# daniestevez/ldpc-toolbox

Hardware: AMD Instinct MI355X
Metric: codewords/s + info-bits/s, DVB-S2 n=64800 r=1/2 min-sum 50 iters (higher is better)
Workload: dtype f32

## Files before the change

### ldpc_toolbox_amd/csrc/c_api.cpp

```cpp
#include "../../include/ldpc_toolbox.h"

#include <algorithm>
#include <cerrno>
#include <cstdio>
#include <cstdlib>
#include <cstring>
#include <fstream>
#include <memory>
#include <sstream>
#include <string>
#include <vector>

#include "codes.h"
#include "demodulator.h"
#include "device_bch.h"
#include "device_decoder.h"
#include "device_encoder.h"
#include "device_nr_rm.h"
#include "encoder.h"
#include "implementation.h"
#include "simulator.h"
#include "sparse.h"

namespace {
// ... 585 lines not shown
  }
  if (!make_device_encoder(h.get(), device)) return nullptr;
  return h.release();
}

int32_t ldpc_toolbox_encoder_encode_batch(void *encoder, uint8_t *output, size_t output_len, const uint8_t *input,
                                          size_t input_len, size_t batch) {
  return encode_batch(encoder, output, output_len, input, input_len, batch, false, nullptr);
}

int32_t ldpc_toolbox_encoder_encode_batch_device(void *encoder, uint8_t *output, size_t output_len, const uint8_t *input,
                                                 size_t input_len, size_t batch, void *hip_stream) {
  return encode_batch(encoder, output, output_len, input, input_len, batch, true, hip_stream);
}

int32_t ldpc_toolbox_encoder_get(void *encoder, const char *key, int64_t *value) {
  auto *h = static_cast<EncoderHandle *>(encoder);
  if (!h || !key || !value) return -1;
  const std::string k = key;
  if (k == "k")
    *value = static_cast<int64_t>(h->enc.k());
  else if (k == "n")
    *value = static_cast<int64_t>(h->enc.n());
  else if (k == "output_len")
    *value = h->out_len == SIZE_MAX ? -1 : static_cast<int64_t>(h->out_len);
  else if (k == "staircase")
    *value = h->enc.staircase() ? 1 : 0;
  else if (k == "staircase_form")
    *value = h->enc.staircase() ? ldpc::staircase_form(h->enc.k()) : -1;
  else if (k == "device")
    *value = h->dev ? h->dev->device() : -1;
  else
    return -1;
  return 0;
}

int32_t ldpc_toolbox_decoder_decode_batch_f32(void *decoder, uint8_t *output, size_t output_len,
                                              const float *llrs, size_t llrs_len, size_t batch,
                                              uint32_t max_iterations, int32_t *iterations, float *posterior) {
  return decode_batch<float>(decoder, output, output_len, llrs, llrs_len, batch, max_iterations, iterations,
                             posterior, false, nullptr);
}

int32_t ldpc_toolbox_decoder_decode_batch_f64(void *decoder, uint8_t *output, size_t output_len,
                                              const double *llrs, size_t llrs_len, size_t batch,
                                              uint32_t max_iterations, int32_t *iterations, double *posterior) {
  return decode_batch<double>(decoder, output, output_len, llrs, llrs_len, batch, max_iterations, iterations,
                              posterior, false, nullptr);
}

int32_t ldpc_toolbox_decoder_decode_batch_f32_device(void *decoder, uint8_t *output, size_t output_len,
                                                     const float *llrs, size_t llrs_len, size_t batch,
                                                     uint32_t max_iterations, int32_t *iterations,
                                                     float *posterior, void *hip_stream) {
  return decode_batch<float>(decoder, output, output_len, llrs, llrs_len, batch, max_iterations, iterations,
                             posterior, true, hip_stream);
}

int32_t ldpc_toolbox_decoder_decode_batch_f64_device(void *decoder, uint8_t *output, size_t output_len,
                                                     const double *llrs, size_t llrs_len, size_t batch,
                                                     uint32_t max_iterations, int32_t *iterations,
                                                     double *posterior, void *hip_stream) {
  return decode_batch<double>(decoder, output, output_len, llrs, llrs_len, batch, max_iterations, iterations,
                              posterior, true, hip_stream);
}

int32_t ldpc_toolbox_decoder_syndrome(void *decoder, const uint8_t *bits, size_t bits_len, size_t batch,
                                      uint8_t *syndrome, uint32_t *weight) {
  g_last_error.clear();
  auto *h = static_cast<DecoderHandle *>(decoder);
  if (!h || !h->dec) {
    set_error("null decoder handle");
    return LDPC_TOOLBOX_ERR_ARGUMENT;
  }
  if (bits_len != h->dec->n() || (!bits && batch)) {
    set_error("hard decisions must cover the whole codeword (bits_len == n)");
    return LDPC_TOOLBOX_ERR_ARGUMENT;
  }
  const int rc = h->dec->syndrome_host(bits, batch, syndrome, weight);
  if (rc == 0) return 0;
  set_error(h->dec->last_error());
  return rc == -1 ? LDPC_TOOLBOX_ERR_ARGUMENT : LDPC_TOOLBOX_ERR_DEVICE;
}

int32_t ldpc_toolbox_decoder_syndrome_device(void *decoder, const uint8_t *bits, size_t bits_len, size_t batch,
                                             uint8_t *syndrome, uint32_t *weight, void *hip_stream) {
  g_last_error.clear();
  auto *h = static_cast<DecoderHandle *>(decoder);
  if (!h || !h->dec) {
    set_error("null decoder handle");
    return LDPC_TOOLBOX_ERR_ARGUMENT;
  }
  if (bits_len != h->dec->n() || (!bits && batch)) {
    set_error("hard decisions must cover the whole codeword (bits_len == n)");
    return LDPC_TOOLBOX_ERR_ARGUMENT;
  }
  const int rc = h->dec->syndrome_device(bits, batch, syndrome, weight, static_cast<hipStream_t>(hip_stream));
  if (rc == 0) return 0;
  set_error(h->dec->last_error());
  return rc == -1 ? LDPC_TOOLBOX_ERR_ARGUMENT : LDPC_TOOLBOX_ERR_DEVICE;
}

int32_t ldpc_toolbox_decoder_get(void *decoder, const char *key, int64_t *value) {
  auto *h = static_cast<DecoderHandle *>(decoder);
  if (!h || !h->dec || !key || !value) return -1;
  const std::string k = key;
  const ldpc::DeviceDecoder &d = *h->dec;
  if (k == "n")
    *value = static_cast<int64_t>(d.n());
  else if (k == "m")
    *value = static_cast<int64_t>(d.m());
  else if (k == "k")
    *value = static_cast<int64_t>(d.n()) - static_cast<int64_t>(d.m());
  else if (k == "edges")
    *value = static_cast<int64_t>(d.edges());
  else if (k == "input_len")
    *value = static_cast<int64_t>(d.input_len());
  else if (k == "device")
    *value = d.device();
  else if (k == "group_size")
    *value = static_cast<int64_t>(d.group_size());
  else if (k == "max_check_degree")
    *value = d.max_check_degree();
  else if (k == "max_variable_degree")
    *value = d.max_variable_degree();
  else if (k == "layers")
    *value = static_cast<int64_t>(d.layers());
  else if (k == "last_lanes")
    *value = d.last_lanes();
  else if (k == "last_pooled")
    *value = static_cast<int64_t>(d.last_pooled());
  else if (k == "last_group")
    *value = static_cast<int64_t>(d.last_group());
  else if (k == "preferred_group")
    *value = static_cast<int64_t>(d.preferred_group(size_t(1) << 20));
  else if (k == "row_records")
    *value = d.row_records();
  else if (k == "record_flag_bits")
    *value = d.record_flag_bits();
  else if (k == "last_vn_records")
    *value = d.last_vn_records();
  else if (k == "last_vn_bundles")
    *value = d.last_vn_bundles();
  else if (k == "vn_bundle_saved_permille")
    *value = d.vn_bundle_saved_permille();
  else if (k == "last_vn_chains")
    *value = d.last_vn_chains();
  else if (k == "vn_chain_saved_permille")
    *value = d.vn_chain_saved_permille();
  else if (k == "flags8")
    *value = d.flags8();
  else if (k == "last_record_flag_bytes")
    *value = d.last_record_flag_bytes();
  else if (k == "minsum_correction")
    *value = static_cast<int64_t>(d.implementation().correction);
  else if (k == "minsum_correction_int")
    *value = d.implementation().correction_int;
  else if (k == "last_persist" || k == "experiments")
    *value = 0;
  else
    return -1;
  return 0;
}

int32_t ldpc_toolbox_decoder_set(void *decoder, const char *key, int64_t value) {
  auto *h = static_cast<DecoderHandle *>(decoder);
  if (!h || !h->dec || !key) return -1;
  const std::string k = key;
  if (k == "group_size" && value >= 0)
    h->dec->set_group_size(static_cast<size_t>(value));
  else if (k == "profiling")
    h->dec->set_profiling(value != 0);
  else if (!h->dec->set_option(k, value))
    return -1;
  return 0;
}

int32_t ldpc_toolbox_decoder_kernel_stats(void *decoder, int32_t kind, uint64_t *launches, double *total_ms,
                                          int32_t reset) {
  auto *h = static_cast<DecoderHandle *>(decoder);
  if (!h || !h->dec || kind < 0 || kind >= ldpc::kKernelKinds) return -1;
  const ldpc::KernelStat s = h->dec->kernel_stat(kind);
  if (launches) *launches = s.launches;
  if (total_ms) *total_ms = s.total_ms;
  if (reset) h->dec->reset_kernel_stats();
  return 0;
}


void *ldpc_toolbox_sim_ctor(const char *alist, const char *implementation, const char *puncturing, int32_t device,
                            uint32_t pool_size, uint64_t pool_seed) {
  g_last_error.clear();
  if (!alist || !implementation) {
    set_error("null argument");
    return nullptr;
  }
  std::string err;
  ldpc::Simulator *s = ldpc::Simulator::create(alist, implementation, puncturing ? puncturing : "", device,
                                               pool_size, pool_seed, &err);
  if (!s) set_error(err);
  return s;
}

void ldpc_toolbox_sim_dtor(void *sim) { delete static_cast<ldpc::Simulator *>(sim); }

int32_t ldpc_toolbox_sim_run(void *sim, double ebn0_db, uint64_t seed, uint64_t first_frame, size_t frames,
                             uint32_t max_iterations, uint64_t *counters) {
  g_last_error.clear();
  auto *s = static_cast<ldpc::Simulator *>(sim);
  if (!s || !counters) {
    set_error("null argument");
    return -1;
  }
  const int rc = s->run(ebn0_db, seed, first_frame, frames, max_iterations, counters);
  if (rc) set_error(s->last_error());
  return rc;
}

int32_t ldpc_toolbox_sim_run_bch(void *sim, double ebn0_db, uint64_t seed, uint64_t first_frame, size_t frames,
                                 uint32_t max_iterations, uint64_t bch_max_errors, uint64_t *counters) {
  g_last_error.clear();
  auto *s = static_cast<ldpc::Simulator *>(sim);
  if (!s || !counters) {
    set_error("null argument");
    return -1;
  }
  const int rc = s->run_bch(ebn0_db, seed, first_frame, frames, max_iterations, bch_max_errors, counters);
  if (rc) set_error(s->last_error());
  return rc;
}

int32_t ldpc_toolbox_sim_generate(void *sim, double ebn0_db, uint64_t seed, uint64_t first_frame, size_t frames,
                                  float *llrs, uint32_t *pool_index) {
  g_last_error.clear();
  auto *s = static_cast<ldpc::Simulator *>(sim);
  if (!s || !llrs) {
    set_error("null argument");
    return -1;
  }
  const int rc = s->generate(ebn0_db, seed, first_frame, frames, llrs, pool_index);
  if (rc) set_error(s->last_error());
  return rc;
}

int32_t ldpc_toolbox_sim_pool(void *sim, uint8_t *messages, uint8_t *tx_bits) {
  auto *s = static_cast<ldpc::Simulator *>(sim);
  if (!s) return -1;
  if (messages) std::memcpy(messages, s->messages().data(), s->messages().size());
  if (tx_bits) std::memcpy(tx_bits, s->tx_bits().data(), s->tx_bits().size());
  return 0;
}

int32_t ldpc_toolbox_sim_get(void *sim, const char *key, int64_t *value) {
  auto *s = static_cast<ldpc::Simulator *>(sim);
  if (!s || !key || !value) return -1;
  const std::string k = key;
  if (k == "k")
    *value = static_cast<int64_t>(s->k());
  else if (k == "n")
    *value = static_cast<int64_t>(s->n());
  else if (k == "n_tx")
    *value = static_cast<int64_t>(s->n_tx());
  else if (k == "pool")
    *value = s->pool();
  else if (k == "modulation")
    *value = s->modulation();
  else if (k == "interleaving")
    *value = s->interleaving();
  else if (k == "constellation")
    *value = s->has_constellation() ? 1 : 0;
  else if (k == "max_log")
    *value = s->max_log() ? 1 : 0;
  else if (k == "bch")
    *value = s->has_bch() ? 1 : 0;
  else if (k == "rate_match")
    *value = s->has_rate_match() ? 1 : 0;
  else if (k == "streamed_frames" || k == "stream_iterations")
    *value = 0;
  else if (k == "pooled_frames")
    *value = static_cast<int64_t>(s->pooled_frames());
  else if (k == "preferred_batch")
    *value = static_cast<int64_t>(s->decoder()->preferred_group(size_t(1) << 20));
  else
    return -1;
  return 0;
}

int32_t ldpc_toolbox_sim_set(void *sim, const char *key, int64_t value) {
  auto *s = static_cast<ldpc::Simulator *>(sim);
  if (!s || !key) return -1;
  const std::string k = key;
  if (k == "group_size" && value >= 0) {
    s->decoder()->set_group_size(static_cast<size_t>(value));
    return 0;
  }
  if (k == "pooling") {
    s->set_pooling(value != 0);
    return 0;
  }
  if (k == "streaming") return 0;
  if (k == "modulation" || k == "interleaving") {
    g_last_error.clear();
    const bool ok = k == "modulation" ? s->set_modulation(static_cast<int>(value)) : s->set_interleaving(value);
    if (!ok) set_error(s->last_error());
    return ok ? 0 : -1;
  }
// ... 329 lines not shown
```

### ldpc_toolbox_amd/csrc/device_decoder.h

```cpp
#pragma once
#include <hip/hip_runtime_api.h>

#include <algorithm>
#include <atomic>
#include <cstddef>
#include <cstdint>
#include <memory>
#include <string>
#include <vector>

#include "hip_owned.h"
#include "implementation.h"
#include "sparse.h"

namespace ldpc {

struct GroupCall;

struct KernelStat {
  uint64_t launches = 0;
  double total_ms = 0.0;
};

enum KernelKind { kKernelCheck = 0, kKernelVar = 1, kKernelLayer = 2, kKernelOther = 3, kKernelKinds = 4 };

class DeviceDecoder {
 public:
  static DeviceDecoder *create(const SparseMatrix &h, const Implementation &impl,
                               const std::vector<uint8_t> &puncturing, int device, std::string *err);
  ~DeviceDecoder();

  size_t n() const { return n_; }
  size_t m() const { return m_; }
  size_t edges() const { return e_; }
  size_t input_len() const { return input_len_; }
  const Implementation &implementation() const { return impl_; }
  int device() const { return device_; }
  uint32_t max_check_degree() const { return max_row_weight_; }
  uint32_t max_variable_degree() const { return max_col_weight_; }
  size_t layers() const { return level_ptr_.empty() ? 0 : level_ptr_.size() - 1; }
  uint32_t last_lanes() const { return last_lanes_; }
  uint64_t last_pooled() const { return last_pooled_; }
  size_t last_group() const { return last_group_; }
  uint32_t row_records() const { return (rec_ready_ && records_wanted() && opt_lfree_ && !opt_staged_minsum_) ? rec_w_ : 0; }
  uint32_t record_flag_bits() const { return row_records() ? rec_flag_bits_ : 0; }
  uint32_t last_vn_records() const { return last_vn_records_.load(std::memory_order_relaxed) ? 1 : 0; }
  uint32_t flags8() const { return opt_flags8_ ? 1 : 0; }
  uint32_t last_record_flag_bytes() const { return last_record_flag_bytes_.load(std::memory_order_relaxed); }
  uint32_t last_vn_bundles() const { return last_vn_bundles_.load(std::memory_order_relaxed) ? 1 : 0; }
  uint32_t vn_bundle_saved_permille() const { return last_vn_bundle_saved_.load(std::memory_order_relaxed); }
  uint32_t last_vn_chains() const { return last_vn_chains_.load(std::memory_order_relaxed) ? 1 : 0; }
  uint32_t vn_chain_saved_permille() const { return last_vn_chain_saved_.load(std::memory_order_relaxed); }

  void set_group_size(size_t g) { group_pref_ = g; }
  size_t group_size() const { return group_pref_; }
  void set_min_group(size_t g) { min_group_ = g; }
  size_t preferred_group(size_t batch) const { return pick_group(batch); }
  bool set_option(const std::string &key, int64_t value);
  void set_profiling(bool on);
  KernelStat kernel_stat(int kind);
  void reset_kernel_stats();

  int decode_device(const void *llrs, bool llrs_f64, size_t batch, uint32_t max_iterations,
                    uint8_t *bits, size_t out_len, int32_t *iterations, void *posterior,
                    hipStream_t stream);

  int decode_host(const void *llrs, bool llrs_f64, size_t batch, uint32_t max_iterations,
                  uint8_t *bits, size_t out_len, int32_t *iterations, void *posterior);

  int syndrome_device(const uint8_t *bits, size_t batch, uint8_t *syndrome, uint32_t *weight, hipStream_t stream);
  int syndrome_host(const uint8_t *bits, size_t batch, uint8_t *syndrome, uint32_t *weight);

  const std::string &last_error() const { return error_; }

 private:
  DeviceDecoder() = default;
  struct Workspace;
  struct GroupFrame;
  int run_group_i8(Workspace &w, const GroupCall &call);
  template <typename T>
  int run_group(Workspace &w, const GroupCall &call);
  int run_any(Workspace &w, const GroupCall &call);
  int ensure_workspace(Workspace &w, size_t group, void *place = nullptr, size_t *need = nullptr);
  int ensure_lanes(uint32_t lanes, size_t group);
  void release_joint();
  int ensure_host_staging(Workspace &w, size_t G, size_t in_elem);
  int ensure_row_scratch(Workspace &w, size_t bytes);
  struct HostPipe;
  int ensure_pipe(size_t group, size_t out_len, size_t in_elem, bool posterior);
  int stage_in(const char *src, char *dst, size_t bytes);
  int drain_out(char *dst, const char *src, size_t bytes);
  struct LatencyPath;
  struct SmallBatchCall;
  struct EdgeLatencyPath;
  size_t edge_latency_limit() const;
  uint32_t opt_latency_edge_ = 256;
  size_t edge_lanes_ = 0;
  int decode_latency_edge(const void *llrs, bool llrs_f64, bool host_pointers, size_t batch, uint32_t max_iterations,
                             uint8_t *bits, size_t out_len, int32_t *iterations, void *posterior, hipStream_t stream);
  uint32_t opt_latency_ = 32;
  static constexpr int kLatencyRetry = -100;
  static constexpr uint32_t opt_serial_levels_default() { return 512; }
  int decode_latency(const void *llrs, bool llrs_f64, bool host_pointers, size_t batch, uint32_t max_iterations,
                     uint8_t *bits, size_t out_len, int32_t *iterations, void *posterior, hipStream_t stream);
  uint32_t lane_count() const;
  bool split_pays(size_t batch) const;
  size_t pick_group(size_t batch) const;
  bool fail(const std::string &msg, hipError_t e = hipSuccess);
  void timed_begin(int kind, hipStream_t s);
  void timed_end(int kind, hipStream_t s);
  void drain_events();

  Implementation impl_;
  int device_ = 0;
  size_t n_ = 0, m_ = 0, e_ = 0, input_len_ = 0;
  uint32_t max_row_weight_ = 0, max_col_weight_ = 0;
  size_t group_pref_ = 0, min_group_ = 0;
  uint32_t opt_tile_ = 0;
  uint32_t opt_waves_ = 0, opt_vec_ = 4;
  bool opt_staged_minsum_ = false;
  static constexpr uint32_t kStreamBlock = 256;
  static constexpr uint32_t kVnWaves = 128 * 1024;
  static constexpr uint32_t kPackWaves = 16 * 1024;
  static constexpr uint32_t kSyndThreads = 512 * 1024, kMoveWaves = 64 * 1024, kRetireBlocks = 256;
  static constexpr uint32_t kCompactHorizon = 8, kCompactCostLive = 9, kCompactCostSlots = 0, kCompactMinFreedQ = 2;
  std::string error_;

  uint32_t n_keep_ = 0, n_free_ = 0;
  uint32_t post_rows_keep_ = 0;
  bool opt_rec_long_ = false;
  bool opt_rec_quiet_ = true;
  bool opt_vn_event_ = true;
  bool opt_vn_records_ = false;
  bool opt_flags8_ = false;
  bool opt_vn_bundles_ = false;
  static constexpr uint32_t kVnBundleW = kStreamBlock / 64;
  uint32_t vn_bundle_saved_[kVnBundleW + 1] = {};
  std::atomic<bool> last_vn_bundles_{false};
  std::atomic<uint32_t> last_vn_bundle_saved_{0};
  bool opt_vn_chains_ = false;
  uint32_t opt_vn_chain_len_ = 8;
  static constexpr uint32_t kVnChainLens[3] = {4, 8, 16};
  struct VnChainAt {
    uint32_t rs_at = 0, var_at = 0, ptr_at = 0, n_blocks = 0;
    uint32_t saved = 0, saved_alone = 0;
  } vn_chain_at_[3];
  std::atomic<bool> last_vn_chains_{false};
  std::atomic<uint32_t> last_vn_chain_saved_{0};
  std::atomic<uint32_t> last_record_flag_bytes_{0};
  std::atomic<bool> last_vn_records_{false};
  uint32_t rec_w_ = 0;
  uint32_t rec_flag_bits_ = 0;
  bool rec_ready_ = false, rec_prefers_ = false;
  uint32_t opt_records_ = 1;
  bool records_wanted() const { return opt_records_ >= 2 || (opt_records_ == 1 && rec_prefers_); }
  uint32_t opt_rec_run_ = 8;
  bool opt_compact_ = true;
  uint32_t opt_compact_first_ = 0, opt_compact_every_ = 0;
  uint32_t opt_serial_levels_ = 512;
  uint32_t opt_cn_reg_ = 1;
  uint32_t opt_hl_reg_ = 1;
  bool opt_lane_threads_ = true, opt_throttle_ = false;
  uint32_t opt_lead_ = 0;
  bool opt_lane_pace_ = true;
  bool opt_hl_records_ = true;
  std::vector<uint32_t> level_maxdeg_;
  std::vector<uint32_t> level_rec_ptr_;
  bool lfree_ready_ = false, opt_lfree_ = true;
  std::vector<uint32_t> level_ptr_;
  uint32_t pattern_len_ = 0;

  size_t joint_stride_ = 0, joint_second_ = 0;
  int order_after_default_stream(hipStream_t s);
  uint32_t last_lanes_ = 0;
  size_t last_group_ = 0;
  bool opt_pooling_ = false;
  uint64_t last_pooled_ = 0;
  uint32_t pool_budget_ = 0, pool_budget_max_it_ = 0;
  struct StragglerPool;
  int ensure_pool(size_t batch, size_t rows, size_t out_len, size_t in_elem, bool posterior, bool own_iterations);
  static uint32_t next_pool_budget(double ok, double sum_its_ok, double stragglers, double straggler_its, double failed_full,
                                   uint32_t max_it);
  int decode_device_plain(const void *llrs, bool llrs_f64, size_t batch, uint32_t max_iterations, uint8_t *bits, size_t out_len,
                          int32_t *iterations, void *posterior, hipStream_t stream);
  int decode_device_pooled(const void *llrs, bool llrs_f64, size_t batch, uint32_t max_iterations, uint8_t *bits, size_t out_len,
                           int32_t *iterations, void *posterior, hipStream_t stream);
  int decode_host_plain(const void *llrs, bool llrs_f64, size_t batch, uint32_t max_iterations, uint8_t *bits, size_t out_len,
                        int32_t *iterations, void *posterior);
  int decode_host_pooled(const void *llrs, bool llrs_f64, size_t batch, uint32_t max_iterations, uint8_t *bits, size_t out_len,
                         int32_t *iterations, void *posterior);
  size_t pool_chunk(size_t batch) const;
  uint32_t opt_lanes_ = 0;
  bool opt_poll_ = true;

  bool profiling_ = false;
  struct PendingEvent {
    int kind;
    Event a, b;
  };
  KernelStat stats_[kKernelKinds];

  Stream stream_, stream2_;
  Event ev_fork_, ev_join_, ev_default_;
  DeviceBuffer d_row_ptr_, d_edge_col_, d_col_ptr_, d_col_edge_;
  DeviceBuffer d_level_rows_;
  DeviceBuffer d_level_recs_;
  DeviceBuffer d_row_recs_;
  DeviceBuffer d_serial_recs_;
  DeviceBuffer d_src_block_;
  DeviceBuffer d_edge_aux_, d_keep_var_, d_keep_ptr_, d_keep_edge_, d_free_var_, d_free_ptr_, d_free_edge_;
  DeviceBuffer d_edge_peer_, d_free_rs_, d_keep_pos_;
  DeviceBuffer d_keep_rs_;
  uint32_t bundle_rs_at_ = 0, bundle_var_at_ = 0, bundle_ptr_at_ = 0;
  DeviceBuffer joint_slab_;
  std::unique_ptr<Workspace> ws_[2];
  std::unique_ptr<StragglerPool> pool_;
  std::unique_ptr<EdgeLatencyPath> lat_edge_;
  std::unique_ptr<LatencyPath> lat_;
  std::unique_ptr<HostPipe> pipe_;
  std::vector<Event> event_pool_;
  std::vector<PendingEvent> pending_;
};

}
```

### ldpc_toolbox_amd/csrc/device_decoder.hip

```cpp
#define LDPC_GROUP_KERNELS_TU 1
#include "codes.h"
#include "device_decoder_internal.h"

namespace ldpc {

static bool is_dvbs2_half_rate_normal(const SparseMatrix::Csr &g) {
  if (g.n_cols != 64800 || g.n_rows != 32400) return false;
  SparseMatrix ref;
  if (!codes::dvbs2("R1_2", &ref)) return false;
  const SparseMatrix::Csr r = ref.csr();
  if (r.n_edges != g.n_edges || r.row_ptr != g.row_ptr) return false;
  std::vector<uint32_t> a, b;
  for (uint32_t row = 0; row < g.n_rows; row++) {
    a.assign(g.edge_col.begin() + g.row_ptr[row], g.edge_col.begin() + g.row_ptr[row + 1]);
    b.assign(r.edge_col.begin() + r.row_ptr[row], r.edge_col.begin() + r.row_ptr[row + 1]);
    std::sort(a.begin(), a.end());
    std::sort(b.begin(), b.end());
    if (a != b) return false;
  }
  return true;
}

bool DeviceDecoder::fail(const std::string &msg, hipError_t e) {
  static std::mutex m;
// ... 73 lines not shown
  };
  g.edge_col.resize(g.edge_col.size() + kTablePad, 0);
  bool ok = up(g.row_ptr, &d->d_row_ptr_) && up(g.edge_col, &d->d_edge_col_) && up(g.col_ptr, &d->d_col_ptr_) &&
            up(g.col_edge, &d->d_col_edge_);
  const bool flooding_minsum = impl.schedule == Schedule::Flooding && impl.rule == Rule::Minsum && !impl.i8;
  if (ok && flooding_minsum) {
    const LfreeTables lf = build_lfree_tables(g);
    if (lf.ready) {
      d->n_keep_ = lf.n_keep;
      d->n_free_ = lf.n_free;
      d->post_rows_keep_ = lf.post_rows_keep;
      ok = up(lf.aux, &d->d_edge_aux_) && up(lf.keep_var, &d->d_keep_var_) && up(lf.keep_ptr, &d->d_keep_ptr_) &&
           up(lf.keep_edge, &d->d_keep_edge_) && up(lf.free_var, &d->d_free_var_) && up(lf.free_ptr, &d->d_free_ptr_) &&
           up(lf.free_edge, &d->d_free_edge_);
      d->lfree_ready_ = ok;
    }
    const RowRecordTables rr = d->lfree_ready_ ? build_row_record_tables(g, lf, impl.f64) : RowRecordTables();
    if (rr.ready) {
      d->rec_prefers_ = rr.rec_prefers;
      d->rec_w_ = rr.rec_w;
      d->rec_flag_bits_ = rr.flag_bits;
      ok = up(rr.keep_pos, &d->d_keep_pos_) && up(rr.peer, &d->d_edge_peer_) && up(rr.free_rs, &d->d_free_rs_);
      d->rec_ready_ = ok;
      const KeepRsTable kr = (ok && rr.flag_bits == 16) ? build_keep_rs(g, lf) : KeepRsTable();
      if (kr.ready) {
        const VnBundleTables vb = build_vn_bundles(lf.n_keep, lf.keep_ptr, lf.keep_var, kr.rs, kVnBundleW);
        std::vector<uint32_t> words = kr.rs;
        auto append = [&](const std::vector<uint32_t> &v) {
          const uint32_t at = static_cast<uint32_t>(words.size());
          words.insert(words.end(), v.begin(), v.end());
          return at;
        };
        d->bundle_rs_at_ = append(vb.keep_rs);
        d->bundle_var_at_ = append(vb.list_var);
        d->bundle_ptr_at_ = append(vb.list_ptr);
        for (uint32_t c = 0; c < 3; c++) {
          const VnChainTables vc = build_vn_chains(lf.n_keep, lf.keep_ptr, lf.keep_var, kr.rs, kVnBundleW, kVnChainLens[c]);
          VnChainAt &at = d->vn_chain_at_[c];
          at.rs_at = append(vc.keep_rs);
          at.var_at = append(vc.list_var);
          at.ptr_at = append(vc.list_ptr);
          at.n_blocks = vc.n_blocks;
          at.saved = vc.fetches ? static_cast<uint32_t>((vc.fetches - vc.issued) * 1000 / vc.fetches) : 0;
          at.saved_alone = vc.fetches ? static_cast<uint32_t>(vc.carried * 1000 / vc.fetches) : 0;
        }
        ok = up(words, &d->d_keep_rs_);
        for (uint32_t w = 2; w <= kVnBundleW; w++) {
          uint64_t fetches = 0, distinct = 0;
          count_vn_bundle_fetches(lf.n_keep, vb.list_ptr, vb.keep_rs, w, &fetches, &distinct);
          d->vn_bundle_saved_[w] = fetches ? static_cast<uint32_t>((fetches - distinct) * 1000 / fetches) : 0;
        }
      }
      d->opt_vn_records_ = kr.ready && ok && !impl.f64 && impl.correction == Correction::None && is_dvbs2_half_rate_normal(g);
      d->opt_flags8_ = d->opt_vn_records_;
      d->opt_vn_bundles_ = d->opt_vn_records_ && d->bundle_rs_at_ != 0;
      d->opt_vn_chains_ = d->opt_vn_bundles_ && d->vn_chain_at_[0].rs_at != 0;
    }
  }
  if (ok && flooding_minsum && !impl.f64) {
    SlicedTables st = build_sliced_tables(g);
    if (st.ready) {
      d->lat_ = std::make_unique<LatencyPath>();
      d->lat_->tables = std::move(st);
    }
  }
  if (ok && impl.schedule == Schedule::Flooding && impl.rule == Rule::Tanh && !impl.i8 && d->max_row_weight_ <= kLevelRecShort) {
    LevelTables all;
    all.level_ptr = {0u, g.n_rows};
    all.rows.resize(g.n_rows);
    for (uint32_t r = 0; r < g.n_rows; r++) all.rows[r] = r;
    all.maxdeg = {d->max_row_weight_};
    ok = up(build_level_recs(all, g.row_ptr, g.edge_col).words, &d->d_row_recs_);
  }
  LevelTables lt;
  if (ok && impl.schedule == Schedule::Layered) {
    lt = build_levels(g.row_ptr, g.edge_col, g.n_rows, g.n_cols);
    d->level_ptr_ = lt.level_ptr;
    d->level_maxdeg_ = lt.maxdeg;
    const LevelRecs lr = build_level_recs(lt, g.row_ptr, g.edge_col);
    d->level_rec_ptr_ = lr.rec_ptr;
    LevelTables all;
    all.level_ptr = {0u, g.n_rows};
    all.rows = lt.rows;
    all.maxdeg = {lt.maxdeg.empty() ? 0u : *std::max_element(lt.maxdeg.begin(), lt.maxdeg.end())};
    ok = up(lt.rows, &d->d_level_rows_) && up(lr.words, &d->d_level_recs_) &&
         up(build_level_recs(all, g.row_ptr, g.edge_col).words, &d->d_serial_recs_);
  }
  if (ok && !impl.fast && !(impl.i8 && impl.rule == Rule::Minsum) && d->lat_ == nullptr &&
      (impl.schedule == Schedule::Flooding || d->level_ptr_.size() <= size_t(opt_serial_levels_default()) + 1)) {
    EdgeLaneTables et = build_edge_lane_tables(g, impl.schedule == Schedule::Layered ? &lt : nullptr);
    if (et.ready) {
      d->edge_lanes_ = et.lane_var.size();
      d->lat_edge_ = std::make_unique<EdgeLatencyPath>();
      d->lat_edge_->tables = std::move(et);
    }
  }
  if (ok && !puncturing.empty()) {
    const DepunctureMap dm = build_depuncture_map(puncturing, g.n_cols);
    if (!dm.ready) return bail("codeword size not divisible by puncturing pattern length");
    d->pattern_len_ = static_cast<uint32_t>(puncturing.size());
    d->input_len_ = dm.input_len;
    ok = up(dm.src_block, &d->d_src_block_);
  }
  ok = ok && d->stream_.create() == hipSuccess && d->stream2_.create() == hipSuccess && d->ev_fork_.create() == hipSuccess &&
       d->ev_join_.create() == hipSuccess && d->ev_default_.create() == hipSuccess;
  if (!ok) return bail("device allocation / upload of the graph tables failed");
  d->ws_[0] = std::make_unique<Workspace>();
  d->ws_[1] = std::make_unique<Workspace>();
  return d.release();
}

DeviceDecoder::~DeviceDecoder() {
  (void)hipSetDevice(device_);
  if (stream_) (void)hipStreamSynchronize(stream_);
  if (stream2_) (void)hipStreamSynchronize(stream2_);
}


void DeviceDecoder::set_profiling(bool on) { profiling_ = on; }

bool DeviceDecoder::set_option(const std::string &key, int64_t value) {
  if (value < 0) return false;
  const uint32_t v = static_cast<uint32_t>(value);
  if (key == "waves")
    opt_waves_ = v;
  else if (key == "vec")
    opt_vec_ = v;
  else if (key == "tile")
    opt_tile_ = v;
  else if (key == "lfree")
    opt_lfree_ = v != 0;
  else if (key == "records")
    opt_records_ = v != 0 ? (v >= 2 ? 2 : 1) : 0;
  else if (key == "rec_run")
    opt_rec_run_ = std::max<uint32_t>(v, 1);
  else if (key == "rec_quiet")
    opt_rec_quiet_ = v != 0;
  else if (key == "vn_event")
    opt_vn_event_ = v != 0;
  else if (key == "vn_records")
    opt_vn_records_ = v != 0;
  else if (key == "flags8")
    opt_flags8_ = v != 0;
  else if (key == "vn_bundles")
    opt_vn_bundles_ = v != 0;
  else if (key == "vn_chains")
    opt_vn_chains_ = v != 0;
  else if (key == "vn_chain_len") {
    if (v != kVnChainLens[0] && v != kVnChainLens[1] && v != kVnChainLens[2]) return false;
    opt_vn_chain_len_ = v;
  }
  else if (key == "rec_long")
    opt_rec_long_ = v != 0;
  else if (key == "compact")
    opt_compact_ = v != 0;
  else if (key == "staged_minsum")
    opt_staged_minsum_ = v != 0;
  else if (key == "hl_reg")
    opt_hl_reg_ = v;
  else if (key == "cn_reg")
    opt_cn_reg_ = v;
  else if (key == "hl_records")
    opt_hl_records_ = v != 0;
  else if (key == "lane_threads")
    opt_lane_threads_ = v != 0;
  else if (key == "throttle")
    opt_throttle_ = v != 0;
  else if (key == "pooling")
    opt_pooling_ = v != 0;
  else if (key == "lead")
    opt_lead_ = v;
  else if (key == "lane_pace")
    opt_lane_pace_ = v != 0;
  else if (key == "lanes")
    opt_lanes_ = std::min<uint32_t>(v, 2);
  else if (key == "poll")
    opt_poll_ = v != 0;
  else if (key == "latency") {
    opt_latency_ = v;
    opt_latency_edge_ = v == 0 ? 0 : std::max<uint32_t>(v, 64);
  } else if (key == "latency_edge")
    opt_latency_edge_ = v;
  else if (key == "compact_first")
    opt_compact_first_ = v;
  else if (key == "serial_levels")
    opt_serial_levels_ = v;
  else if (key == "compact_every")
    opt_compact_every_ = v;
  else
    return false;
  return true;
}

void DeviceDecoder::timed_begin(int kind, hipStream_t s) {
  if (!profiling_) return;
  PendingEvent p;
  p.kind = kind;
  auto get = [&]() {
    Event e;
    if (!event_pool_.empty()) {
      e = std::move(event_pool_.back());
      event_pool_.pop_back();
    } else {
      (void)e.create(hipEventDefault);
    }
    return e;
  };
  p.a = get();
  p.b = get();
  (void)hipEventRecord(p.a, s);
  pending_.push_back(std::move(p));
}

void DeviceDecoder::timed_end(int, hipStream_t s) {
  if (!profiling_) return;
  (void)hipEventRecord(pending_.back().b, s);
}

void DeviceDecoder::drain_events() {
  for (auto &p : pending_) {
    (void)hipEventSynchronize(p.b);
    float ms = 0.f;
    if (hipEventElapsedTime(&ms, p.a, p.b) == hipSuccess) {
      stats_[p.kind].launches++;
      stats_[p.kind].total_ms += ms;
    }
    event_pool_.push_back(std::move(p.a));
    event_pool_.push_back(std::move(p.b));
  }
  pending_.clear();
}

KernelStat DeviceDecoder::kernel_stat(int kind) {
  drain_events();
  return (kind >= 0 && kind < kKernelKinds) ? stats_[kind] : KernelStat();
}

void DeviceDecoder::reset_kernel_stats() {
  drain_events();
  for (auto &s : stats_) s = KernelStat();
}


size_t DeviceDecoder::pick_group(size_t batch) const {
  const bool serial = impl_.schedule == Schedule::Layered && level_ptr_.size() > size_t(opt_serial_levels_) + 1;
  size_t by_size = 4096;
  while (by_size < 65536 && e_ * by_size * 2 <= size_t(226799) * 4096) by_size *= 2;
  size_t g = group_pref_ ? group_pref_ : std::max<size_t>(serial ? 16384 : 4096, by_size);
  g = std::min(g, std::max(round_up(batch, 64), std::min(min_group_, g)));
  g = round_up(g, 64);
  if (impl_.i8) return round_up(g, 256);
  if (g >= 256) g = g / 256 * 256;
  return g;
}

uint32_t DeviceDecoder::lane_count() const {
  if (opt_lanes_) return opt_lanes_;
  if (impl_.schedule == Schedule::Layered) return 2u;
  if (impl_.f64 || impl_.i8) return 1u;
  if (impl_.rule == Rule::Tanh) return 2u;
  if (impl_.rule == Rule::Minsum && max_row_weight_ > 8 && !profiling_) return 2u;
  return 1u;
}

bool DeviceDecoder::split_pays(size_t batch) const {
  return opt_lanes_ == 2 || (batch >= 2048 && n_ * (batch / 2) >= size_t(50) * 1000 * 1000);
}

int DeviceDecoder::ensure_workspace(Workspace &w, size_t G, void *place, size_t *need) {
  const size_t elem = impl_.i8 ? 2 : (impl_.f64 ? 8 : 4);
  const bool records = lfree_ready_ && rec_ready_ && records_wanted() && opt_lfree_;
  if (!need) {
    if (w.G == G && w.elem == elem && w.chan && w.records == records && (!place || w.slab == place))
      return 0;
    w = Workspace();
  }
  const size_t W = G / 64;
  const size_t align = size_t(2) << 20;
  size_t off = 0;
  auto carve = [&](size_t bytes) {
    const size_t at = off;
    off = round_up(off + std::max<size_t>(bytes, 256), align);
    return at;
  };
  const size_t o_msg = carve(std::max<size_t>(e_, 1) * G * elem);
  const size_t o_msg2 = (lfree_ready_ && !records) ? carve(std::max<size_t>(e_, 1) * G * elem) : 0;
  const bool flags16 = records && rec_flag_bits_ == 16;
  const size_t rec_bytes = records ? std::max<size_t>(m_, 1) * (flags16 ? 2 : rec_w_) * G * elem : 0;
  const size_t o_rec0 = records ? carve(rec_bytes) : 0, o_rec1 = records ? carve(rec_bytes) : 0;
  const size_t flag_bytes = flags16 ? std::max<size_t>(m_, 1) * G * sizeof(uint16_t) : 0;
  const size_t o_flag0 = flags16 ? carve(flag_bytes) : 0, o_flag1 = flags16 ? carve(flag_bytes) : 0;
  const size_t o_post = carve(n_ * G * elem);
  const size_t o_chan = carve(n_ * G * elem);
  const size_t o_perm = carve(4 * G * sizeof(uint32_t) + 1024);
  const size_t o_raw = carve(n_ * W * sizeof(uint64_t));
  const size_t o_hard = carve(n_ * W * sizeof(uint64_t));
  const size_t o_flags = carve(9 * G * sizeof(uint32_t) + 1024);
  if (need) {
    *need = off;
    return 0;
  }
  w.records = records;
  if (w.flag.ensure(64, 64, 64, hipHostMallocMapped) == hipSuccess) {
    w.h_flag = w.flag.get<uint64_t>();
    *w.h_flag = 0;
    if (hipHostGetDevicePointer(reinterpret_cast<void **>(&w.d_flag), w.h_flag, 0) != hipSuccess) w.d_flag = nullptr;
  } else {
    w.h_flag = nullptr;
  }
  w.G = G;
  w.elem = elem;
  if (place) {
    w.slab = place;
    w.borrowed = true;
  } else {
    HIP_TRY(w.own_slab.ensure(off));
    w.slab = w.own_slab.get();
  }
  w.slab_bytes = off;
  char *base = static_cast<char *>(w.slab);
  w.msg = base + o_msg;
  w.msg2 = (lfree_ready_ && !records) ? base + o_msg2 : nullptr;
  w.rec[0] = records ? base + o_rec0 : nullptr;
  w.rec[1] = records ? base + o_rec1 : nullptr;
  w.rec_flags[0] = flags16 ? reinterpret_cast<uint16_t *>(base + o_flag0) : nullptr;
  w.rec_flags[1] = flags16 ? reinterpret_cast<uint16_t *>(base + o_flag1) : nullptr;
  w.post = base + o_post;
  w.chan = base + o_chan;
  w.perm = reinterpret_cast<uint32_t *>(base + o_perm);
  w.slot_cw = w.perm + G;
  w.slot_tmp = w.perm + 2 * G;
  w.fill_cw = w.perm + 3 * G;
  w.n_slots = w.perm + 4 * G;
  w.plan = reinterpret_cast<dev::CompactPlan *>(w.perm + 4 * G + 16);
  w.rawbits = reinterpret_cast<uint64_t *>(base + o_raw);
  w.hardbits = reinterpret_cast<uint64_t *>(base + o_hard);
  uint32_t *flags = reinterpret_cast<uint32_t *>(base + o_flags);
  w.done = flags;
  w.unsat0 = flags + G;
  w.unsat1 = flags + 2 * G;
  w.iters = reinterpret_cast<int32_t *>(flags + 3 * G);
  w.n_active = flags + 4 * G;
  w.scratch_flags = flags + 4 * G + 64;
  w.slice_state = flags + 6 * G;
  if (std::getenv("LDPC_TOOLBOX_DEBUG"))
    std::fprintf(stderr, "ldpc_toolbox (hip): workspace G=%zu slab=%p bytes=%zu msg=+%zx post=+%zx chan=+%zx\n", G,
                 w.slab, off, o_msg, o_post, o_chan);
  return 0;
}

int DeviceDecoder::ensure_lanes(uint32_t lanes, size_t G) {
  if (lanes < 2) {
    Workspace &w = *ws_[0];
    if (w.borrowed && w.G != G) release_joint();
    return ensure_workspace(w, G);
  }
  size_t bytes = 0;
  if (int rc = ensure_workspace(*ws_[0], G, nullptr, &bytes)) return rc;
  const size_t lane_align = size_t(2) << 20;
  const size_t stride = round_up(bytes, lane_align);
  const size_t elem = impl_.i8 ? 2 : (impl_.f64 ? 8 : 4);
  const bool records = lfree_ready_ && rec_ready_ && records_wanted() && opt_lfree_;
  auto current = [&](const Workspace &w, const char *at) {
    return w.borrowed && w.slab == at && w.G == G && w.elem == elem && w.records == records;
  };
  char *base = joint_slab_ ? reinterpret_cast<char *>(round_up(reinterpret_cast<size_t>(joint_slab_.get()), lane_align)) : nullptr;
  if (base && joint_stride_ == stride && current(*ws_[0], base) && current(*ws_[1], base + joint_second_)) return 0;
  release_joint();
  HIP_TRY(joint_slab_.ensure(stride + bytes + lane_align));
  base = reinterpret_cast<char *>(round_up(reinterpret_cast<size_t>(joint_slab_.get()), lane_align));
  joint_stride_ = stride;
  joint_second_ = stride;
  if (int rc = ensure_workspace(*ws_[0], G, base)) return rc;
  return ensure_workspace(*ws_[1], G, base + joint_second_);
}

void DeviceDecoder::release_joint() {
  for (auto &w : ws_)
    if (w && w->borrowed) *w = Workspace();
  joint_slab_ = DeviceBuffer();
  joint_stride_ = 0;
  joint_second_ = 0;
}

int DeviceDecoder::run_any(Workspace &w, const GroupCall &call) {
  GroupCall c = call;
  const bool own_thread = c.own_thread;
  const bool may_wait = c.may_block;
  c.may_block = may_wait && opt_poll_ && impl_.schedule == Schedule::Layered && (own_thread || c.nb * n_ <= size_t(8) * 1000 * 1000);
  c.pace_lead = opt_lead_;
  if (own_thread && may_wait && opt_poll_ && impl_.schedule == Schedule::Layered && opt_lane_pace_) {
    c.may_block = true;
    if (!opt_lead_) c.pace_lead = 1;
  }
  if (impl_.schedule == Schedule::Flooding && !impl_.i8 && opt_poll_ && may_wait && !profiling_ && (c.flood_pace || own_thread)) {
    c.may_block = true;
    if (!opt_lead_) c.pace_lead = 2;
  }
  return impl_.i8 ? run_group_i8(w, c) : impl_.f64 ? run_group<double>(w, c) : run_group<float>(w, c);
}

int DeviceDecoder::order_after_default_stream(hipStream_t s) {
  HIP_TRY(hipEventRecord(ev_default_, nullptr));
  HIP_TRY(hipStreamWaitEvent(s, ev_default_, 0));
  return 0;
}


int DeviceDecoder::ensure_pool(size_t batch, size_t rows, size_t out_len, size_t in_elem, bool posterior, bool own_iterations) {
  if (!pool_) pool_ = std::make_unique<StragglerPool>();
  StragglerPool &p = *pool_;
  constexpr size_t kFloor = 256;
  HIP_TRY(p.d_idx.ensure(batch * sizeof(uint32_t), kFloor));
  HIP_TRY(p.d_stats.ensure(64));
  HIP_TRY(p.d_llrs.ensure(rows * input_len_ * in_elem, kFloor));
  HIP_TRY(p.d_bits.ensure(rows * std::max<size_t>(out_len, 1), kFloor));
  HIP_TRY(p.d_its.ensure(rows * sizeof(int32_t), kFloor));
  if (posterior) HIP_TRY(p.d_post.ensure(rows * n_ * in_elem, kFloor));
  if (own_iterations) HIP_TRY(p.d_its_all.ensure(batch * sizeof(int32_t), kFloor));
  return 0;
}

uint32_t DeviceDecoder::next_pool_budget(double ok, double sum_its_ok, double stragglers, double straggler_its,
                                         double failed_full, uint32_t max_it) {
  const double ok_frames = ok + stragglers, ok_its = sum_its_ok + straggler_its;
  const double avg_ok = ok_frames > 0 ? ok_its / ok_frames : static_cast<double>(max_it);
  uint32_t next = static_cast<uint32_t>(std::min<double>(max_it, std::ceil(2.0 * avg_ok) + 8.0));
  next = std::max<uint32_t>(next, 16);
  if (stragglers + failed_full > 0.25 * (ok + stragglers + failed_full) || uint64_t(next) * 10 >= uint64_t(max_it) * 7) next = max_it;
  return next;
}

size_t DeviceDecoder::pool_chunk(size_t batch) const { return pick_group(batch) * std::max<uint32_t>(lane_count(), 1); }

int DeviceDecoder::decode_device(const void *llrs, bool llrs_f64, size_t batch, uint32_t max_iterations, uint8_t *bits,
                                 size_t out_len, int32_t *iterations, void *posterior, hipStream_t stream) {
  last_pooled_ = 0;
  if (opt_pooling_ && max_iterations >= 24 && batch >= 2 * pool_chunk(batch) && (stream == nullptr || opt_throttle_) && out_len <= n_)
    return decode_device_pooled(llrs, llrs_f64, batch, max_iterations, bits, out_len, iterations, posterior, stream);
  return decode_device_plain(llrs, llrs_f64, batch, max_iterations, bits, out_len, iterations, posterior, stream);
}

int DeviceDecoder::decode_device_pooled(const void *llrs, bool llrs_f64, size_t batch, uint32_t max_iterations, uint8_t *bits,
                                        size_t out_len, int32_t *iterations, void *posterior, hipStream_t stream) {
  HIP_TRY(hipSetDevice(device_));
  const size_t in_elem = llrs_f64 ? 8 : 4, G = pick_group(batch), chunk = pool_chunk(batch);
  hipStream_t s = stream ? stream : stream_;
  if (int rc = ensure_pool(batch, chunk, out_len, in_elem, posterior != nullptr, iterations == nullptr)) return rc;
  StragglerPool &p = *pool_;
  uint32_t *const d_idx = p.d_idx.get<uint32_t>(), *const d_stats = p.d_stats.get<uint32_t>();
  int32_t *its = iterations ? iterations : p.d_its_all.get<int32_t>();
  unsigned long long *d_sum = reinterpret_cast<unsigned long long *>(d_stats + 4);
  HIP_TRY(hipMemsetAsync(d_stats, 0, 64, s));
  uint32_t budget = (pool_budget_ && pool_budget_max_it_ == max_iterations) ? std::min(pool_budget_, max_iterations) : max_iterations;
  double straggler_its = 0.0;
  uint32_t seen_stragglers = 0;
  const size_t llr_row = input_len_ * in_elem, post_row = n_ * in_elem;
  for (size_t b0 = 0; b0 < batch; b0 += chunk) {
    const size_t nf = std::min(chunk, batch - b0);
    if (int rc = decode_device_plain(static_cast<const char *>(llrs) + b0 * llr_row, llrs_f64, nf, budget, bits + b0 * out_len, out_len,
                                     its + b0, posterior ? static_cast<char *>(posterior) + b0 * post_row : nullptr, stream))
      return rc;
    dev::pool_select_kernel<<<static_cast<uint32_t>((nf + 255) / 256), 256, 0, s>>>(
        its + b0, static_cast<uint32_t>(nf), static_cast<uint32_t>(b0), budget < max_iterations ? 1 : 0, d_idx, d_stats, d_sum);
    uint32_t h[6];
    HIP_TRY(hipMemcpyAsync(h, d_stats, sizeof(h), hipMemcpyDeviceToHost, s));
    HIP_TRY(hipStreamSynchronize(s));
    unsigned long long sum_ok;
    std::memcpy(&sum_ok, &h[4], sizeof(sum_ok));
    straggler_its += double(h[2] - seen_stragglers) * budget;
    seen_stragglers = h[2];
    budget = next_pool_budget(h[0], static_cast<double>(sum_ok), h[2], straggler_its, h[1], max_iterations);
  }
  pool_budget_ = budget;
  pool_budget_max_it_ = max_iterations;
  const size_t keep_min = min_group_;
  for (size_t p0 = 0; p0 < seen_stragglers; p0 += chunk) {
    const uint32_t np = static_cast<uint32_t>(std::min<size_t>(chunk, seen_stragglers - p0));
    const uint32_t blocks = (np * 64 + 255) / 256;
    dev::pool_gather_kernel<<<blocks, 256, 0, s>>>(d_idx + p0, np, static_cast<const uint32_t *>(llrs), llr_row / 4,
                                                   p.d_llrs.get<uint32_t>());
    min_group_ = G;
    const int rc = decode_device_plain(p.d_llrs.get(), llrs_f64, np, max_iterations, p.d_bits.get<uint8_t>(), out_len, p.d_its.get<int32_t>(),
                                       posterior ? p.d_post.get() : nullptr, stream);
    min_group_ = keep_min;
    if (rc) return rc;
    dev::pool_scatter_kernel<<<blocks, 256, 0, s>>>(d_idx + p0, np, p.d_bits.get<uint8_t>(), static_cast<uint32_t>(out_len), p.d_its.get<int32_t>(),
                                                    p.d_post.get<const uint32_t>(), posterior ? post_row / 4 : 0, bits,
                                                    iterations, static_cast<uint32_t *>(posterior));
  }
  last_pooled_ = seen_stragglers;
  HIP_TRY(hipGetLastError());
  if (stream == nullptr) HIP_TRY(hipStreamSynchronize(s));
  return 0;
}

int DeviceDecoder::decode_device_plain(const void *llrs, bool llrs_f64, size_t batch, uint32_t max_iterations,
                                       uint8_t *bits, size_t out_len, int32_t *iterations, void *posterior,
                                       hipStream_t stream) {
  if (batch == 0) return 0;
  if (out_len > n_) {
    fail("output_len larger than the codeword length");
    return -1;
  }
  HIP_TRY(hipSetDevice(device_));
  const bool own_stream = stream == nullptr;
  hipStream_t s = own_stream ? stream_ : stream;
  if (own_stream)
    if (int rc = order_after_default_stream(s)) return rc;
  if (lat_ && batch <= opt_latency_ && own_stream) {
    const int rc = decode_latency(llrs, llrs_f64, false, batch, max_iterations, bits, out_len, iterations, posterior, s);
    if (rc != kLatencyRetry) return rc;
  }
  if (lat_edge_ && batch <= edge_latency_limit() && own_stream) {
    const int rc = decode_latency_edge(llrs, llrs_f64, false, batch, max_iterations, bits, out_len, iterations, posterior, s);
    if (rc != kLatencyRetry) return rc;
  }
  size_t G = pick_group(batch);
  uint32_t lanes = lane_count();
  if (lanes == 2 && batch <= G && split_pays(batch)) G = round_up((batch + 1) / 2, 256);
  if (batch <= G) lanes = 1;
  last_lanes_ = lanes;
  last_group_ = G;
  if (int rc = ensure_lanes(lanes, G)) return rc;
  if (lanes == 2) {
    HIP_TRY(hipEventRecord(ev_fork_, s));
    HIP_TRY(hipStreamWaitEvent(stream2_, ev_fork_, 0));
  }
  const size_t in_elem = llrs_f64 ? 8 : 4;
  const bool threaded = lanes == 2 && opt_lane_threads_ && !profiling_ && max_iterations > 0 &&
                        (impl_.schedule == Schedule::Layered ||
                         (impl_.schedule == Schedule::Flooding && !impl_.i8 && (opt_throttle_ || own_stream) && opt_poll_));
  const bool may_block = own_stream || opt_throttle_;
  auto run_groups = [&](uint32_t only_lane) -> int {
    uint32_t gi = 0;
    for (size_t b0 = 0; b0 < batch; b0 += G, gi++) {
      const uint32_t lane = lanes == 2 ? (gi & 1u) : 0u;
      if (only_lane != 2 && lane != only_lane) continue;
      const size_t nb = std::min(G, batch - b0);
      const char *src = static_cast<const char *>(llrs) + b0 * input_len_ * in_elem;
      uint8_t *dst_bits = bits + b0 * out_len;
      int32_t *dst_it = iterations ? iterations + b0 : nullptr;
      void *dst_post = posterior ? static_cast<char *>(posterior) + b0 * n_ * in_elem : nullptr;
      if (int rc = run_any(*ws_[lane], GroupCall{src, llrs_f64, nb, max_iterations, dst_bits, out_len, dst_it, dst_post,
                                                 lane ? stream2_ : s, may_block, threaded, lanes == 1}))
        return rc;
    }
    return 0;
  };
  if (threaded) {
    int rc1 = 0;
    std::thread second([&] {
      rc1 = hipSetDevice(device_) == hipSuccess ? run_groups(1) : -2;
    });
    const int rc0 = run_groups(0);
    second.join();
    if (rc0 || rc1) return rc0 ? rc0 : rc1;
  } else if (int rc = run_groups(2)) {
    return rc;
  }
  if (lanes == 2) {
    HIP_TRY(hipEventRecord(ev_join_, stream2_));
    HIP_TRY(hipStreamWaitEvent(s, ev_join_, 0));
  }
  if (own_stream) HIP_TRY(hipStreamSynchronize(s));
  return 0;
}

int DeviceDecoder::ensure_row_scratch(Workspace &w, size_t bytes) {
  HIP_TRY(w.row_scratch.ensure(bytes));
  return 0;
}

int DeviceDecoder::ensure_host_staging(Workspace &w, size_t G, size_t in_elem) {
  HIP_TRY(w.in.ensure(G * input_len_ * in_elem));
  return 0;
}

namespace {

void par_memcpy(char *dst, const char *src, size_t bytes, unsigned threads) {
  if (threads <= 1 || bytes < (size_t(4) << 20)) {
    std::memcpy(dst, src, bytes);
    return;
  }
  const size_t per = round_up((bytes + threads - 1) / threads, 4096);
  std::vector<std::thread> th;
  for (size_t off = per; off < bytes; off += per)
    th.emplace_back([=] { std::memcpy(dst + off, src + off, std::min(per, bytes - off)); });
  std::memcpy(dst, src, std::min(per, bytes));
  for (auto &t : th) t.join();
}

}

int DeviceDecoder::ensure_pipe(size_t group, size_t out_len, size_t in_elem, bool posterior) {
  if (!pipe_) {
    auto p = std::make_unique<HostPipe>();
    const unsigned hw = std::max(1u, std::thread::hardware_concurrency());
    p->copy_threads = std::min(8u, std::max(1u, hw / 2));
    bool ok = p->h2d.create() == hipSuccess && p->d2h.create() == hipSuccess;
    for (int i = 0; ok && i < HostPipe::kSlots; i++) ok = p->in_done[i].create() == hipSuccess && p->out_done[i].create() == hipSuccess;
    for (int l = 0; ok && l < 2; l++) ok = p->in_ready[l].create() == hipSuccess && p->ingested[l].create() == hipSuccess;
    if (!ok) {
      fail("host staging: stream / event creation failed");
      return -2;
    }
    pipe_ = std::move(p);
  }
  HostPipe &p = *pipe_;
  for (int r = 0; r < HostPipe::kOutRing; r++) {
    HIP_TRY(p.d_bits[r].ensure(std::max<size_t>(group * out_len, 1)));
    HIP_TRY(p.d_iters[r].ensure(group * sizeof(int32_t)));
    if (posterior) HIP_TRY(p.d_post[r].ensure(group * n_ * in_elem));
  }
  return 0;
}

int DeviceDecoder::stage_in(const char *src, char *dst, size_t bytes) {
  HostPipe &p = *pipe_;
  for (size_t off = 0; off < bytes; off += HostPipe::kChunk) {
    const size_t len = std::min(HostPipe::kChunk, bytes - off);
    const int slot = p.next_in;
    p.next_in = (p.next_in + 1) % HostPipe::kSlots;
    HIP_TRY(hipEventSynchronize(p.in_done[slot]));
    if (p.in_slot[slot].ensure(len, HostPipe::kGranule, HostPipe::kChunk) != hipSuccess) {
      fail("host staging: pinned input chunk");
      return -2;
    }
    par_memcpy(p.in_slot[slot].get<char>(), src + off, len, p.copy_threads);
    HIP_TRY(hipMemcpyAsync(dst + off, p.in_slot[slot].get(), len, hipMemcpyHostToDevice, p.h2d));
    HIP_TRY(hipEventRecord(p.in_done[slot], p.h2d));
  }
  return 0;
}

int DeviceDecoder::drain_out(char *dst, const char *src, size_t bytes) {
  HostPipe &p = *pipe_;
  const size_t chunks = (bytes + HostPipe::kChunk - 1) / HostPipe::kChunk;
  auto issue = [&](size_t c) -> int {
    const size_t off = c * HostPipe::kChunk, len = std::min(HostPipe::kChunk, bytes - off);
    const int slot = static_cast<int>(c % HostPipe::kSlots);
    if (p.out_slot[slot].ensure(len, HostPipe::kGranule, HostPipe::kChunk) != hipSuccess) {
      fail("host staging: pinned output chunk");
      return -2;
    }
    HIP_TRY(hipMemcpyAsync(p.out_slot[slot].get(), src + off, len, hipMemcpyDeviceToHost, p.d2h));
    HIP_TRY(hipEventRecord(p.out_done[slot], p.d2h));
    return 0;
  };
  for (size_t c = 0; c < std::min<size_t>(chunks, HostPipe::kSlots); c++)
    if (int rc = issue(c)) return rc;
  for (size_t c = 0; c < chunks; c++) {
    const size_t off = c * HostPipe::kChunk, len = std::min(HostPipe::kChunk, bytes - off);
    const int slot = static_cast<int>(c % HostPipe::kSlots);
    HIP_TRY(hipEventSynchronize(p.out_done[slot]));
    par_memcpy(dst + off, p.out_slot[slot].get<char>(), len, p.copy_threads);
    if (c + HostPipe::kSlots < chunks)
      if (int rc = issue(c + HostPipe::kSlots)) return rc;
  }
  return 0;
}

int DeviceDecoder::decode_host(const void *llrs, bool llrs_f64, size_t batch, uint32_t max_iterations, uint8_t *bits,
                               size_t out_len, int32_t *iterations, void *posterior) {
  last_pooled_ = 0;
  if (opt_pooling_ && max_iterations >= 24 && batch >= 2 * 4 * pool_chunk(batch) && out_len <= n_)
    return decode_host_pooled(llrs, llrs_f64, batch, max_iterations, bits, out_len, iterations, posterior);
  return decode_host_plain(llrs, llrs_f64, batch, max_iterations, bits, out_len, iterations, posterior);
}

int DeviceDecoder::decode_host_pooled(const void *llrs, bool llrs_f64, size_t batch, uint32_t max_iterations, uint8_t *bits,
                                      size_t out_len, int32_t *iterations, void *posterior) {
  const size_t in_elem = llrs_f64 ? 8 : 4, chunk = 4 * pool_chunk(batch);
  const size_t llr_row = input_len_ * in_elem, post_row = n_ * in_elem;
  std::vector<int32_t> own_its;
  if (!iterations) own_its.resize(batch);
  int32_t *its = iterations ? iterations : own_its.data();
  std::vector<size_t> stragglers;
  uint32_t budget = (pool_budget_ && pool_budget_max_it_ == max_iterations) ? std::min(pool_budget_, max_iterations) : max_iterations;
  double ok = 0, sum_ok = 0, straggler_its = 0, failed_full = 0;
  for (size_t b0 = 0; b0 < batch; b0 += chunk) {
    const size_t nf = std::min(chunk, batch - b0);
    if (int rc = decode_host_plain(static_cast<const char *>(llrs) + b0 * llr_row, llrs_f64, nf, budget, bits + b0 * out_len, out_len,
                                   its + b0, posterior ? static_cast<char *>(posterior) + b0 * post_row : nullptr))
      return rc;
    const bool reduced = budget < max_iterations;
    for (size_t i = 0; i < nf; i++) {
      const int32_t it = its[b0 + i];
      if (it >= 0) {
        ok += 1;
        sum_ok += it;
      } else if (reduced) {
        stragglers.push_back(b0 + i);
        straggler_its += budget;
      } else {
        failed_full += 1;
      }
    }
    budget = next_pool_budget(ok, sum_ok, static_cast<double>(stragglers.size()), straggler_its, failed_full, max_iterations);
  }
  pool_budget_ = budget;
  pool_budget_max_it_ = max_iterations;
  if (!stragglers.empty()) {
    const size_t np = stragglers.size();
    std::vector<char> rows(np * llr_row), pbits(np * std::max<size_t>(out_len, 1)), ppost(posterior ? np * post_row : 0);
    std::vector<int32_t> pits(np);
    for (size_t i = 0; i < np; i++) std::memcpy(&rows[i * llr_row], static_cast<const char *>(llrs) + stragglers[i] * llr_row, llr_row);
    const size_t keep_min = min_group_;
    min_group_ = pick_group(batch);
    const int rc = decode_host_plain(rows.data(), llrs_f64, np, max_iterations, reinterpret_cast<uint8_t *>(pbits.data()), out_len,
                                     pits.data(), posterior ? ppost.data() : nullptr);
    min_group_ = keep_min;
    if (rc) return rc;
    for (size_t i = 0; i < np; i++) {
      const size_t f = stragglers[i];
      std::memcpy(bits + f * out_len, &pbits[i * out_len], out_len);
      its[f] = pits[i];
      if (posterior) std::memcpy(static_cast<char *>(posterior) + f * post_row, &ppost[i * post_row], post_row);
    }
  }
  last_pooled_ = stragglers.size();
  return 0;
}

int DeviceDecoder::decode_host_plain(const void *llrs, bool llrs_f64, size_t batch, uint32_t max_iterations,
                                     uint8_t *bits, size_t out_len, int32_t *iterations, void *posterior) {
  if (batch == 0) return 0;
  if (out_len > n_) {
    fail("output_len larger than the codeword length");
    return -1;
  }
  HIP_TRY(hipSetDevice(device_));
  if (lat_ && batch <= opt_latency_) {
    const int rc = decode_latency(llrs, llrs_f64, true, batch, max_iterations, bits, out_len, iterations, posterior, stream_);
    if (rc != kLatencyRetry) return rc;
  }
  if (lat_edge_ && batch <= edge_latency_limit()) {
    const int rc = decode_latency_edge(llrs, llrs_f64, true, batch, max_iterations, bits, out_len, iterations, posterior, stream_);
    if (rc != kLatencyRetry) return rc;
  }
  size_t G = pick_group(batch);
  while (!group_pref_ && G > 4096 && G * input_len_ * (llrs_f64 ? 8 : 4) > (size_t(256) << 20)) G /= 2;
  if (lane_count() == 2 && batch <= G && split_pays(batch)) G = round_up((batch + 1) / 2, 256);
  const uint32_t lanes = (batch > G && opt_lanes_ != 1) ? 2u : 1u;
  last_lanes_ = lanes;
  last_group_ = G;
  const size_t in_elem = llrs_f64 ? 8 : 4;
  if (int rc = ensure_lanes(lanes, G)) return rc;
  for (uint32_t l = 0; l < lanes; l++)
    if (int rc = ensure_host_staging(*ws_[l], G, in_elem)) return rc;
  if (int rc = ensure_pipe(std::min(G, batch), out_len, in_elem, posterior != nullptr)) return rc;
  HostPipe &p = *pipe_;
  std::vector<size_t> starts;
  {
    size_t b0 = 0;
    if (batch >= 2 * G && G >= 1024 && (G / 4) % 256 == 0) {
      starts.push_back(0);
      starts.push_back(G / 4);
      b0 = G;
    }
    for (; b0 < batch; b0 += G) starts.push_back(b0);
    const size_t last0 = starts.back(), last_n = batch - last0;
    if (starts.size() >= 3 && last_n >= 1024) {
      const size_t tail = std::max<size_t>(256, last_n / 4 / 256 * 256);
      starts.push_back(batch - tail);
    }
    starts.push_back(batch);
  }
  const size_t n_groups = starts.size() - 1;
  while (p.group_done.size() < n_groups) {
    Event e;
    HIP_TRY(e.create());
    p.group_done.push_back(std::move(e));
  }
  hipStream_t streams[2] = {stream_, stream2_};
  const size_t row_in = input_len_ * in_elem;
  constexpr size_t R = HostPipe::kOutRing;
  int rc = 0;
  auto drain_group = [&](size_t gi) -> int {
    const size_t b0 = starts[gi], nb = starts[gi + 1] - b0, r = gi % R;
    HIP_TRY(hipStreamWaitEvent(p.d2h, p.group_done[gi], 0));
    int drc = 0;
    if (out_len) drc = drain_out(reinterpret_cast<char *>(bits + b0 * out_len), p.d_bits[r].get<const char>(), nb * out_len);
    if (drc == 0 && iterations)
      drc = drain_out(reinterpret_cast<char *>(iterations + b0), p.d_iters[r].get<const char>(), nb * sizeof(int32_t));
    if (drc == 0 && posterior)
      drc = drain_out(static_cast<char *>(posterior) + b0 * n_ * in_elem, p.d_post[r].get<const char>(), nb * n_ * in_elem);
    return drc;
  };
  const bool threaded = lanes == 2 && n_groups >= 2 && impl_.schedule == Schedule::Layered && opt_lane_threads_ && !profiling_ &&
                        max_iterations > 0;
  struct LaneQueue {
    std::thread th;
    std::mutex m;
    std::condition_variable cv;
    std::deque<std::function<int()>> tasks;
    bool closing = false;
    std::atomic<uint32_t> ingest_recorded{0}, enqueued{0};
    std::atomic<int> rc{0};
  };
  LaneQueue lq[2];
  auto wait_for = [&](std::atomic<uint32_t> &counter, uint32_t at_least, LaneQueue &q) {
    while (counter.load(std::memory_order_acquire) < at_least && q.rc.load() == 0) std::this_thread::yield();
  };
  if (threaded) {
    for (uint32_t l = 0; l < 2; l++) {
      lq[l].th = std::thread([this, l, &lq] {
        LaneQueue &q = lq[l];
        if (hipSetDevice(device_) != hipSuccess) q.rc = -2;
        for (;;) {
          std::function<int()> task;
          {
            std::unique_lock<std::mutex> lock(q.m);
            q.cv.wait(lock, [&] { return q.closing || !q.tasks.empty(); });
            if (q.tasks.empty()) return;
            task = std::move(q.tasks.front());
            q.tasks.pop_front();
          }
// ... 161 lines not shown
```

### ldpc_toolbox_amd/csrc/device_decoder_internal.h

```cpp
#pragma once
#include "device_decoder.h"

#include <algorithm>
#include <atomic>
#include <chrono>
#include <condition_variable>
#include <cstdio>
#include <cstdlib>
#include <cstring>
#include <deque>
#include <functional>
#include <mutex>
#include <thread>
#include <type_traits>

#include "graph_tables.h"
#include "hip_owned.h"
#include "kernels.hip.h"
#include "slice_tasks.h"
#include "latency.hip.h"
#include "latency_edge.hip.h"

namespace ldpc {

inline uint32_t env_u32(const char *name, uint32_t dflt) {
  const char *s = std::getenv(name);
  if (!s || !*s) return dflt;
  return static_cast<uint32_t>(std::strtoul(s, nullptr, 10));
}

inline size_t round_up(size_t x, size_t m) { return (x + m - 1) / m * m; }

struct DeviceDecoder::Workspace {
  size_t G = 0;
  size_t elem = 4;
  void *slab = nullptr;
  DeviceBuffer own_slab;
  bool borrowed = false;
  size_t slab_bytes = 0;
  void *chan = nullptr, *post = nullptr, *msg = nullptr, *msg2 = nullptr;
  void *rec[2] = {nullptr, nullptr};
  uint16_t *rec_flags[2] = {nullptr, nullptr};
  bool records = false;
  uint64_t *rawbits = nullptr, *hardbits = nullptr;
  uint32_t *perm = nullptr, *slot_cw = nullptr, *slot_tmp = nullptr, *fill_cw = nullptr, *n_slots = nullptr;
  dev::CompactPlan *plan = nullptr;
  uint32_t *done = nullptr, *unsat0 = nullptr, *unsat1 = nullptr, *n_active = nullptr, *scratch_flags = nullptr,
           *slice_state = nullptr;
  int32_t *iters = nullptr;
  PinnedBuffer flag;
  uint64_t *h_flag = nullptr, *d_flag = nullptr;
  uint32_t epoch = 0;
  DeviceBuffer in;
  hipEvent_t after_ingest = nullptr;
  std::atomic<uint32_t> *ingest_seq = nullptr;
  DeviceBuffer row_scratch;
};

struct DeviceDecoder::HostPipe {
  static constexpr size_t kChunk = size_t(32) << 20;
  static constexpr size_t kGranule = size_t(64) << 10;
  static constexpr int kSlots = 4;
  static constexpr int kOutRing = 4;
  Stream h2d, d2h;
  PinnedBuffer in_slot[kSlots], out_slot[kSlots];
  Event in_done[kSlots], out_done[kSlots];
  int next_in = 0;
  Event in_ready[2], ingested[2];
  std::vector<Event> group_done;
  DeviceBuffer d_bits[kOutRing], d_iters[kOutRing], d_post[kOutRing];
  unsigned copy_threads = 1;
};

struct SmallBatchStaging {
  PinnedBuffer h_in, h_out;
  uint32_t grid = 0;
};

struct DeviceDecoder::LatencyPath {
  SlicedTables tables;
  bool uploaded = false;
  DeviceBuffer d_rslice_ptr, d_rdeg, d_col, d_vslice_ptr, d_vdeg, d_vedge, d_perm, d_inv;
  DeviceBuffer slot_mem, sync;
  dev::LatencyState slots{};
  SmallBatchStaging staging;
  static constexpr size_t kPinnedGranule = size_t(1) << 20;
};

struct DeviceDecoder::EdgeLatencyPath {
  EdgeLaneTables tables;
  bool uploaded = false;
  DeviceBuffer d_level_chunk, d_lane_var, d_lane_info, d_var_ptr, d_var_lane;
  DeviceBuffer slot_mem, flag_mem, sync;
  dev::EdgeLatState slots{};
  SmallBatchStaging staging;
  static constexpr size_t kPinnedGranule = size_t(1) << 16;
};

#define HIP_TRY(expr)                                  \
  do {                                                 \
    hipError_t _e = (expr);                            \
    if (_e != hipSuccess) {                            \
      fail(#expr, _e);                                 \
      return -2;                                       \
    }                                                  \
  } while (0)

struct DeviceDecoder::StragglerPool {
  DeviceBuffer d_idx, d_stats, d_llrs, d_post, d_bits, d_its, d_its_all;
};


struct Tiling {
  uint32_t blocks, threads;
  dev::Sched sched;
};

inline Tiling make_tiling(uint32_t G, uint32_t tile, uint32_t slice, uint32_t nodes, uint32_t threads,
                   uint32_t target_waves) {
  Tiling t;
  t.threads = threads;
  t.sched.tile = tile;
  t.sched.nchunks = G / slice;
  const uint32_t wpb = threads / 64;
  uint32_t wpc = std::max<uint32_t>(1, target_waves / t.sched.nchunks);
  wpc = std::min<uint32_t>(wpc, std::max<uint32_t>(nodes, 1));
  t.sched.slices_per_tile = std::max<uint32_t>(1, tile / slice);
  while ((uint64_t(wpc) * t.sched.slices_per_tile) % wpb != 0) wpc++;
  t.sched.waves_per_chunk = wpc;
  t.sched.reverse = 0;
  t.sched.per_tile_div = dev::fast_div(wpc * t.sched.slices_per_tile);
  t.sched.spt_div = dev::fast_div(t.sched.slices_per_tile);
  t.sched.tile_div = dev::fast_div(tile);
  t.sched.n_tiles = (t.sched.nchunks + t.sched.slices_per_tile - 1) / t.sched.slices_per_tile;
  t.blocks = static_cast<uint32_t>(uint64_t(wpc) * t.sched.nchunks / wpb);
  return t;
}

struct GroupCall {
  const void *llrs;
  bool llrs_f64;
  size_t nb;
  uint32_t max_iterations;
  uint8_t *bits;
  size_t out_len;
  int32_t *iterations;
  void *posterior;
  hipStream_t stream;
  bool may_block;
  bool own_thread;
  bool flood_pace;
  uint32_t pace_lead = 0;
};

template <int V>
using int_c = std::integral_constant<int, V>;
template <typename F>
auto with_bool(bool b, F &&f) {
  if (b) return f(std::true_type{});
  return f(std::false_type{});
}
template <typename T, typename F>
auto with_vec(uint32_t vec, F &&f) {
  if constexpr (sizeof(T) == 4)
    if (vec == 4) return f(int_c<4>{});
  if (vec >= 2) return f(int_c<2>{});
  return f(int_c<1>{});
}

inline bool staged_block(uint32_t arrays, uint32_t dmax, size_t elem, uint32_t *threads, size_t *lds) {
  for (uint32_t t : {256u, 128u, 64u}) {
    const size_t bytes = size_t(arrays) * std::max<uint32_t>(dmax, 1) * t * elem;
    if (bytes <= 64 * 1024 || (t == 64 && bytes <= 160 * 1024)) {
      *threads = t;
      *lds = bytes;
      return true;
    }
  }
  return false;
}


constexpr uint32_t kScratchWaves = 2048, kScratchThreads = 256;
inline size_t scratch_bytes_for(const Tiling &t, uint32_t dmax, size_t elem) {
  return size_t(t.blocks) * (t.threads / 64) * 2 * dmax * 64 * elem;
}


struct ProgressPoll {
  const uint64_t *flag;
  uint32_t epoch;
  bool throttle;
  uint32_t lead;
  hipStream_t stream;
  static constexpr int64_t kStallNs = 200 * 1000 * 1000;
  mutable bool gave_up = false;

  static uint64_t load(const uint64_t *p) { return __atomic_load_n(p, __ATOMIC_ACQUIRE); }
  uint32_t running(uint32_t all) const {
    if (!flag) return all;
    const uint64_t f = load(flag);
    return (f >> 40) == uint64_t(epoch & 0xFFFFFFu) ? static_cast<uint32_t>(f & 0xFFFFFu) : all;
  }
  bool finished(uint32_t it) const {
    if (!flag) return false;
    const uint64_t mine = uint64_t(epoch & 0xFFFFFFu);
    uint64_t f = load(flag);
    if (throttle && !gave_up && it > lead) {
      uint64_t last = f;
      auto since = std::chrono::steady_clock::now();
      for (uint32_t spins = 1;; spins++) {
        if ((f >> 40) == mine && ((f & 0xFFFFFu) == 0 || ((f >> 20) & 0xFFFFFu) + lead >= it)) break;
        if ((spins & 0x3FFu) == 0) {
          if (hipStreamQuery(stream) != hipErrorNotReady) {
            f = load(flag);
            break;
          }
          const auto now = std::chrono::steady_clock::now();
          if (f != last) {
            last = f;
            since = now;
          } else if (std::chrono::duration_cast<std::chrono::nanoseconds>(now - since).count() > kStallNs) {
            gave_up = true;
            break;
          }
        }
        f = load(flag);
      }
    }
    return (f >> 40) == mine && (f & 0xFFFFFu) == 0;
  }
};


inline uint32_t pick_vec_for(uint32_t tile, uint32_t max_vec, uint32_t wanted) {
  uint32_t vec = std::min<uint32_t>(std::min(max_vec, std::max<uint32_t>(wanted, 1)), 4);
  if (vec == 3) vec = 2;
  while (vec > 1 && tile % (64 * vec) != 0) vec /= 2;
  return vec;
}

namespace grp {
void init_group(hipStream_t s, uint32_t *done, int32_t *iters, uint32_t *unsat0, uint32_t *unsat1, uint32_t *n_active,
                uint32_t *n_slots, uint32_t *slot_cw, uint32_t nb, uint32_t G);
void latch(hipStream_t s, uint32_t *done, int32_t *iters, uint32_t *unsat, uint32_t *n_active, int32_t iteration, uint32_t G);
void syndrome_bits(hipStream_t s, uint32_t threads, const uint32_t *row_ptr, const uint32_t *edge_col, uint32_t n_rows,
                   const uint64_t *bits, uint32_t *unsat, const uint32_t *n_active, const uint32_t *n_slots, uint32_t W,
                   uint32_t rows_per_thread);
void compact_plan(hipStream_t s, dev::State st, dev::CompactPlan *plan, uint32_t *movers, uint32_t *holes, uint32_t *fill_cw,
                  uint32_t remaining_iterations, dev::CompactRule rule);
void compact_commit(hipStream_t s, dev::State st, const dev::CompactPlan *plan, uint32_t *unsat0, uint32_t *unsat1,
                    uint32_t *n_slots, const uint32_t *fill_cw, uint32_t G);
}

struct DeviceDecoder::GroupFrame {
  DeviceDecoder &d;
  Workspace &w;
  const GroupCall &c;
  const hipStream_t s;
  const uint32_t G, W, n, m, tile;
  const uint32_t *const row_ptr = d.d_row_ptr_.get<uint32_t>(), *const edge_col = d.d_edge_col_.get<uint32_t>();
  dev::State st;
  const ProgressPoll poll;
  const uint32_t synd_chunks = (W + 63) / 64;
  const uint32_t synd_rows =
      std::max<uint32_t>(1, std::min<uint32_t>(64, uint32_t(uint64_t(m) * synd_chunks * 64 / kSyndThreads)));
  const uint32_t synd_threads = 64 * synd_chunks * ((m + synd_rows - 1) / synd_rows);

  GroupFrame(DeviceDecoder &dec, Workspace &ws, const GroupCall &call, uint32_t tile_)
      : d(dec), w(ws), c(call), s(call.stream), G(static_cast<uint32_t>(ws.G)), W(G / 64), n(static_cast<uint32_t>(dec.n_)),
        m(static_cast<uint32_t>(dec.m_)), tile(tile_),
        st{ws.done, ws.iters, ws.n_active, ws.n_slots, ws.slot_cw, nullptr, 0, 0, nullptr, nullptr, 0},
        poll{(dec.opt_poll_ && ws.d_flag) ? ws.h_flag : nullptr, ws.epoch = (ws.epoch % 0xFFFFFFu) + 1, call.may_block,
             call.pace_lead ? call.pace_lead : (dec.impl_.schedule == Schedule::Layered ? 2u : 8u), call.stream} {}

  dev::Graph graph(const uint32_t *edge_aux, const uint32_t *edge_peer) const {
    return dev::Graph{row_ptr, edge_col, d.d_col_ptr_.get<uint32_t>(), d.d_col_edge_.get<uint32_t>(), m, n, static_cast<uint32_t>(d.e_),
                      nullptr, nullptr,  nullptr,                      0,                              edge_aux, edge_peer};
  }
  dev::State ticked(uint32_t it) const {
    dev::State t = st;
    t.publish = d.opt_poll_ ? w.d_flag : nullptr;
    t.epoch = w.epoch;
    t.tick = it;
    return t;
  }
  void syndrome_of(const uint64_t *hard, uint32_t *unsat) const {
    if (m == 0) return;
    grp::syndrome_bits(s, synd_threads, row_ptr, edge_col, m, hard, unsat, w.n_active, w.n_slots, W, synd_rows);
  }
  void latch(uint32_t *unsat, int32_t it) const { grp::latch(s, w.done, w.iters, unsat, w.n_active, it, G); }
  template <typename K32, typename K64, typename C, typename P>
  int begin(K32 ingest_f32, K64 ingest_f64, C *chan, P *post) const {
    grp::init_group(s, w.done, w.iters, w.unsat0, w.unsat1, w.n_active, w.n_slots, w.slot_cw, static_cast<uint32_t>(c.nb), G);
    const dim3 grid((n + 63) / 64, W);
    const uint32_t block_size = d.pattern_len_ ? n / d.pattern_len_ : 0;
    auto ingest = [&](auto kernel, auto *src) {
      kernel<<<grid, 256, 0, s>>>(src, d.input_len_, static_cast<uint32_t>(c.nb), n, G, tile, chan, post, w.rawbits,
                                  d.d_src_block_.get<int32_t>(), block_size);
    };
    if (c.llrs_f64)
      ingest(ingest_f64, static_cast<const double *>(c.llrs));
    else
      ingest(ingest_f32, static_cast<const float *>(c.llrs));
    if (w.after_ingest) {
      if (const hipError_t e = hipEventRecord(w.after_ingest, s); e != hipSuccess) {
        d.fail("hipEventRecord(w.after_ingest, s)", e);
        return -2;
      }
      if (w.ingest_seq) w.ingest_seq->fetch_add(1, std::memory_order_release);
    }
    syndrome_of(w.rawbits, w.unsat0);
    latch(w.unsat0, 0);
    return 0;
  }
  template <typename P>
  void emit(const P *post, const uint32_t *do_compact, int zero_fill, int retire_only) const {
    const dim3 grid(std::min<uint32_t>((n + 63) / 64, retire_only ? kRetireBlocks : 4096), W);
    auto go = [&](auto kernel, auto *out) {
      kernel<<<grid, 256, 0, s>>>(post, w.rawbits, st, do_compact, n, G, tile, static_cast<uint32_t>(c.out_len), c.bits,
                                  c.iterations, out, zero_fill, retire_only);
    };
    if (c.llrs_f64)
      go(dev::emit_kernel<P, double>, static_cast<double *>(c.posterior));
    else
      go(dev::emit_kernel<P, float>, static_cast<float *>(c.posterior));
  }
};

}
```

### ldpc_toolbox_amd/csrc/kernels_flooding.hip.h

```cpp
#pragma once
namespace ldpc {
namespace dev {



template <typename T>
struct RecWord {
  typedef uint32_t type;
  static constexpr int kArgShift = 26;
};
template <>
struct RecWord<double> {
  typedef uint64_t type;
  static constexpr int kArgShift = 58;
};

typedef uint32_t store_u32x4 __attribute__((ext_vector_type(4)));
__device__ __forceinline__ void store_data_pad(const store_u32x4 &data) { asm volatile("s_nop 0" ::"v"(data)); }

template <typename T, int VEC, bool NT>
__device__ __forceinline__ Pack<T, VEC> buf_load(const RowBuf &b, uint32_t lane_off, uint32_t row_off) {
  constexpr int kBytes = sizeof(T) * VEC;
  static_assert(kBytes == 4 || kBytes == 8 || kBytes == 16, "pack size");
  if constexpr (kBytes == 4)
// ... 116 lines not shown
  template <bool NT>
  __device__ __forceinline__ void store(const RowBuf &b, uint32_t lane_off, uint32_t row_off, uint32_t row_bytes) const {
    buf_store<T, VEC, NT>(b, lane_off, row_off, min1);
    buf_store<T, VEC, NT>(b, lane_off, row_off + row_bytes, min2);
    buf_store<T, VEC, NT>(b, lane_off, row_off + 2 * row_bytes, __builtin_bit_cast(Pack<T, VEC>, flip));
    if constexpr (RECW == 4) buf_store<T, VEC, NT>(b, lane_off, row_off + 3 * row_bytes, __builtin_bit_cast(Pack<T, VEC>, arg));
  }
  __device__ __forceinline__ T value(uint32_t slot, int k) const {
    const W a = RECW == 4 ? arg.v[k] : (flip.v[k] >> RecWord<T>::kArgShift);
    const T mag = (a == W(slot)) ? min2.v[k] : min1.v[k];
    const W sign = (flip.v[k] >> slot) << (8 * sizeof(W) - 1);
    return __builtin_bit_cast(T, __builtin_bit_cast(W, mag) | sign);
  }
};
template <typename T, int VEC>
struct RowRec<T, VEC, 3, uint16_t> {
  typedef typename RecWord<T>::type W;
  static __device__ __forceinline__ uint16_t pack_flags(W fl, uint32_t arg) {
    return uint16_t((uint32_t(fl) & ((1u << kArgShift16) - 1)) | (arg << kArgShift16));
  }
  typedef RowRec New;
  static constexpr uint32_t kRows = 2;
  Pack<T, VEC> min1, min2;
  Pack<uint16_t, VEC> flip;
  __device__ __forceinline__ void load(const RecBuf<true> &b, uint32_t lane_off, uint32_t row_off, uint32_t row_bytes) {
    min1 = buf_load<T, VEC, false>(b.b, lane_off, row_off);
    min2 = buf_load<T, VEC, false>(b.b, lane_off, row_off + row_bytes);
    flip = flags_load<uint16_t, VEC, false>(b.f, lane_off / uint32_t(sizeof(T) / sizeof(uint16_t)), row_off / uint32_t(sizeof(T)));
  }
  template <bool NT>
  __device__ __forceinline__ void store(const RecBuf<true> &b, uint32_t lane_off, uint32_t row_off, uint32_t row_bytes) const {
    buf_store<T, VEC, NT>(b.b, lane_off, row_off, min1);
    buf_store<T, VEC, NT>(b.b, lane_off, row_off + row_bytes, min2);
    flags_store<uint16_t, VEC, NT>(b.f, lane_off / uint32_t(sizeof(T) / sizeof(uint16_t)), row_off / uint32_t(sizeof(T)), flip);
  }
  __device__ __forceinline__ T value(uint32_t slot, int k) const {
    const uint32_t f = flip.v[k];
    const T mag = ((f >> kArgShift16) == slot) ? min2.v[k] : min1.v[k];
    const W sign = W(f >> slot) << (8 * sizeof(W) - 1);
    return __builtin_bit_cast(T, __builtin_bit_cast(W, mag) | sign);
  }
};
template <typename T, int VEC>
struct RowRec8New : RowRec<T, VEC, 3, uint16_t> {
  typedef typename RecWord<T>::type W;
  template <bool NT>
  __device__ __forceinline__ void store(const RecBuf<true> &b, uint32_t lane_off, uint32_t row_off, uint32_t row_bytes) const {
    Pack<T, VEC> m1, m2;
    Pack<uint8_t, VEC> fl;
#pragma unroll
    for (int k = 0; k < VEC; k++) {
      const RecFlags8Stored<W> r = record_flags8_encode<W>(__builtin_bit_cast(W, this->min1.v[k]),
                                                           __builtin_bit_cast(W, this->min2.v[k]), this->flip.v[k]);
      m1.v[k] = __builtin_bit_cast(T, r.min1);
      m2.v[k] = __builtin_bit_cast(T, r.min2);
      fl.v[k] = r.byte;
    }
    buf_store<T, VEC, NT>(b.b, lane_off, row_off, m1);
    buf_store<T, VEC, NT>(b.b, lane_off, row_off + row_bytes, m2);
    flags_store<uint8_t, VEC, NT>(b.f, lane_off / uint32_t(sizeof(T)), row_off / uint32_t(2 * sizeof(T)), fl);
  }
};
template <typename T, int VEC>
struct RowRec<T, VEC, 3, uint8_t> {
  typedef typename RecWord<T>::type W;
  typedef RowRec8New<T, VEC> New;
  static __device__ __forceinline__ uint16_t pack_flags(W fl, uint32_t arg) { return New::pack_flags(fl, arg); }
  static constexpr uint32_t kRows = 2;
  Pack<T, VEC> min1, min2;
  Pack<uint8_t, VEC> fl;
  __device__ __forceinline__ void load(const RecBuf<true> &b, uint32_t lane_off, uint32_t row_off, uint32_t row_bytes) {
    min1 = buf_load<T, VEC, false>(b.b, lane_off, row_off);
    min2 = buf_load<T, VEC, false>(b.b, lane_off, row_off + row_bytes);
    fl = flags_load<uint8_t, VEC, false>(b.f, lane_off / uint32_t(sizeof(T)), row_off / uint32_t(2 * sizeof(T)));
  }
  __device__ __forceinline__ T value(uint32_t slot, int k) const {
    const RecFlags8Loaded<W> r = record_flags8_decode<W>(__builtin_bit_cast(W, min1.v[k]), __builtin_bit_cast(W, min2.v[k]), fl.v[k]);
    const uint32_t f = r.flags;
    const W mag = ((f >> kArgShift16) == slot) ? r.min2 : r.min1;
    const W sign = W(f >> slot) << (8 * sizeof(W) - 1);
    return __builtin_bit_cast(T, mag | sign);
  }
};
template <typename T, int VEC>
struct RowRec8Once {
  typedef typename RecWord<T>::type W;
  typedef RowRec8New<T, VEC> New;
  static constexpr uint32_t kRows = 2;
  Pack<T, VEC> min1, min2;
  uint32_t fl, arg;
  __device__ __forceinline__ void load(const RecBuf<true> &b, uint32_t lane_off, uint32_t row_off, uint32_t row_bytes) {
    min1 = buf_load<T, VEC, false>(b.b, lane_off, row_off);
    min2 = buf_load<T, VEC, false>(b.b, lane_off, row_off + row_bytes);
    const Pack<uint8_t, VEC> bytes = flags_load<uint8_t, VEC, false>(b.f, lane_off / uint32_t(sizeof(T)), row_off / uint32_t(2 * sizeof(T)));
    fl = 0;
#pragma unroll
    for (int k = 0; k < VEC; k++) fl |= uint32_t(bytes.v[k]) << (8 * k);
    uint32_t a = (fl >> 7) & 0x01010101u;
#pragma unroll
    for (int k = 0; k < VEC; k++)
      a |= record_flags8_arg<W>(__builtin_bit_cast(W, min1.v[k]), __builtin_bit_cast(W, min2.v[k]), uint8_t(0)) << (8 * k);
    asm("" : "+v"(fl));
    asm("" : "+v"(a));
    arg = a;
  }
  __device__ __forceinline__ T value(uint32_t slot, int k) const {
    return __builtin_bit_cast(T, record_flags8_value<W>(__builtin_bit_cast(W, min1.v[k]), __builtin_bit_cast(W, min2.v[k]),
                                                        uint8_t(fl >> (8 * k)), (arg >> (8 * k)) & 0xFFu, slot));
  }
};


template <typename T, int VEC, int RECW, bool F16 = false, bool F8 = false>
__global__ __launch_bounds__(256) void vn_free_rec_kernel(Graph g, Sched sc, State st, const uint32_t *__restrict__ free_rs_,
                                                          const T *__restrict__ chan, typename RecRef<T, F16, F8>::in rec,
                                                          T *__restrict__ post, int32_t event_iteration) {
  typedef RowRec<T, VEC, RECW, RecFlagWord<T, F16, F8>> Rec;
  if (event_iteration < 0 && *st.n_active == 0) return;
  const TablePtr free_var = table_ptr(g.list_var), free_rs = table_ptr(free_rs_);
  const uint32_t lane = threadIdx.x & 63u, tile = sc.tile;
  const uint32_t wave = uniform((blockIdx.x * blockDim.x + threadIdx.x) >> 6);
  uint32_t chunk, i0;
  wave_slot(sc, wave, &chunk, &i0);
  if (chunk >= sc.nchunks) return;
  const uint32_t b0 = chunk * (64 * VEC);
  if (b0 >= *st.n_slots) return;
  if (event_iteration >= 0 && st.slice_state[chunk] != 1) return;
  const size_t off = size_t(b0) + lane * VEC;
  const size_t G = tile;
  chan += tile_base(b0, g.n_cols, sc) + lane * VEC;
  post += tile_base(b0, g.n_cols, sc) + lane * VEC;
  const uint32_t row_bytes = tile * uint32_t(sizeof(T)), lane_off = lane * uint32_t(VEC * sizeof(T));
  const RecBuf<F16> b_rec = rec_buf<T, RECW>(rec, b0, g.n_rows, sc, row_bytes);
  bool live[VEC];
  bool any_live = false;
#pragma unroll
  for (int k = 0; k < VEC; k++) {
    live[k] = event_iteration < 0 ? st.done[off + k] == 0 : (st.done[off + k] != 0 && st.iters[off + k] == event_iteration);
    any_live = any_live || live[k];
  }
  if (__builtin_amdgcn_ballot_w64(any_live) == 0) return;
  for (uint32_t i = i0; i < g.n_list; i += sc.waves_per_chunk) {
    const uint32_t v = free_var[i], a = free_rs[2 * i], b = free_rs[2 * i + 1];
    const Pack<T, VEC> ch = load_pack<T, VEC>(chan + size_t(v) * G);
    Rec ra, rb;
    if (a != kAuxNone) ra.load(b_rec, lane_off, (a >> 6) * Rec::kRows * row_bytes, row_bytes);
    if (b != kAuxNone) rb.load(b_rec, lane_off, (b >> 6) * Rec::kRows * row_bytes, row_bytes);
#pragma unroll
    for (int k = 0; k < VEC; k++) {
      T sum = -T(0.0);
      if (a != kAuxNone) sum = sum + ra.value(a & 63u, k);
      if (b != kAuxNone) sum = sum + rb.value(b & 63u, k);
      if (live[k]) post[size_t(v) * G + k] = ch.v[k] + sum;
    }
  }
}


template <typename RecIn>
struct VnEvent {
  const uint32_t *free_var, *free_rs;
  RecIn rec;
  uint32_t n_free;
};
template <typename T, bool EVF16, bool EVF8 = false>
using VnEventOf = VnEvent<typename RecRef<T, EVF16, EVF8>::in>;
__device__ __forceinline__ bool has_records(const void *rec) { return rec != nullptr; }
template <typename T, typename FW>
__device__ __forceinline__ bool has_records(const RecPair<T, FW> &rec) { return rec.mag != nullptr; }
template <typename... SRC>
struct VnSource;
template <typename M>
struct VnSource<M> {
  M msg;
};
template <typename R, typename K>
struct VnSource<R, K> {
  R rec;
  K keep_rs;
};
struct VnChain {
  uint32_t len, width, mates, n_blocks, n_groups;
};
template <typename R, typename K, typename C>
struct VnSource<R, K, C> {
  R rec;
  K keep_rs;
  C chain;
};
template <typename Rec, typename T, int VEC, typename FW>
struct VnCarry {
  static_assert(VEC * sizeof(FW) <= 8, "the flag words of a lane fit two registers");
  Pack<T, VEC> min1, min2;
  uint32_t fl[2];
  static __device__ __forceinline__ Pack<FW, VEC> &flags_of(RowRec<T, VEC, 3, uint16_t> &r) { return r.flip; }
  static __device__ __forceinline__ Pack<FW, VEC> &flags_of(RowRec<T, VEC, 3, uint8_t> &r) { return r.fl; }
  __device__ __forceinline__ void keep(Rec r) {
    min1 = r.min1;
    min2 = r.min2;
    uint64_t bits = 0;
#pragma unroll
    for (int k = 0; k < VEC; k++) bits |= uint64_t(flags_of(r).v[k]) << (8 * sizeof(FW) * k);
    fl[0] = uint32_t(bits);
    fl[1] = uint32_t(bits >> 32);
    asm("" : "+v"(fl[0]));
    if constexpr (VEC * sizeof(FW) > 4) asm("" : "+v"(fl[1]));
  }
  __device__ __forceinline__ T value(uint32_t slot, int k) const {
    Rec r;
    r.min1 = min1;
    r.min2 = min2;
    const uint64_t bits = uint64_t(fl[0]) | (uint64_t(fl[1]) << 32);
    flags_of(r).v[k] = FW(bits >> (8 * sizeof(FW) * k));
    return r.value(slot, k);
  }
};
struct VnChainWalk {
  uint32_t blk, w, t, mate;
  __device__ __forceinline__ uint32_t settle(const VnChain &c, uint32_t n_list) {
    while (blk < c.n_blocks) {
      const uint32_t i = (blk * c.len + t) * c.width + w;
      if (t < c.len && i < n_list) return i;
      t = 0;
      w += c.mates;
      if (w >= c.width) {
        w = mate;
        blk += c.n_groups;
      }
    }
    return n_list;
  }
};
template <typename T, int VEC, int U, bool NT, bool LIST, int EVW = 0, bool EVF16 = false, bool EVF8 = false, typename... SRC>
__global__ __launch_bounds__(256) void vn_kernel(
    Graph g, Sched sc, State st, const T *__restrict__ chan, SRC... src,
    T *__restrict__ post, const uint32_t *__restrict__ unsat_in, uint32_t *__restrict__ unsat_clear,
    int32_t latch_iteration, VnEventOf<T, EVF16, EVF8> ev = {}) {
  constexpr bool REC = sizeof...(SRC) >= 2, CHAIN = sizeof...(SRC) == 3;
  const VnSource<const SRC &...> from{src...};
  static_assert(!REC || (LIST && EVF16 && (EVW == 0 || EVW == 3)), "from records: the kept list, the 16-bit family's records");
  uint32_t *__restrict__ n_active = st.n_active;
  const bool idle = *n_active == 0;
  if (EVW == 0 && idle) return;
  const TablePtr col_ptr = table_ptr(LIST ? g.list_ptr : g.col_ptr);
  TablePtr col_edge = nullptr;
  if constexpr (!REC) col_edge = table_ptr(LIST ? g.list_edge : g.col_edge);
  uint32_t *__restrict__ done = st.done;
  int32_t *__restrict__ iters = st.iters;
  const uint32_t n_cols = LIST ? g.n_list : g.n_cols;
  const uint32_t waves_per_chunk = sc.waves_per_chunk, tile = sc.tile;
  const uint32_t lane = threadIdx.x & 63u;
  const uint32_t wave = uniform((blockIdx.x * blockDim.x + threadIdx.x) >> 6);
  uint32_t chunk, v_first;
  wave_slot(sc, wave, &chunk, &v_first);
  if (chunk >= sc.nchunks) return;
  const uint32_t b0 = chunk * (64 * VEC);
  if (b0 >= *st.n_slots) return;
  if constexpr (EVW != 0) {
    if (idle && (!has_records(ev.rec) || unsat_in == nullptr || st.slice_state == nullptr || st.slice_state[chunk] == 2u)) return;
  }
  const size_t off = size_t(b0) + lane * VEC;
  const size_t G = tile;
  chan += tile_base(b0, g.n_cols, sc) + lane * VEC;
  post += tile_base(b0, g.n_cols, sc) + lane * VEC;
  const T *__restrict__ msg = nullptr;
  if constexpr (!REC) msg = from.msg + tile_base(b0, g.n_edges, sc) + lane * VEC;
  uint32_t row_bytes = 0, lane_off = 0;
  if constexpr (REC) {
    row_bytes = tile * uint32_t(sizeof(T));
    lane_off = lane * uint32_t(VEC * sizeof(T));
  }
  bool skip[VEC];
  bool any_live = false, any_new = false;
#pragma unroll
  for (int k = 0; k < VEC; k++) {
    const bool was_done = done[off + k] != 0;
    const bool converged = !was_done && unsat_in != nullptr && unsat_in[off + k] == 0;
    int32_t own_iterations = latch_iteration;
    bool expired = false;
    if (st.it0 != nullptr) {
      own_iterations = latch_iteration - static_cast<int32_t>(st.it0[off + k]);
      expired = !was_done && !converged && own_iterations >= static_cast<int32_t>(st.max_it);
    }
    skip[k] = was_done || converged || expired;
    any_live = any_live || !skip[k];
    if (v_first == 0 && !idle) {
      if (converged || expired) {
        done[off + k] = 1u;
        iters[off + k] = converged ? own_iterations : -1;
        atomicSub(n_active, 1u);
        any_new = true;
      }
      unsat_clear[off + k] = 0u;
    }
  }
  if constexpr (EVW != 0) {
    if (has_records(ev.rec) && unsat_in != nullptr && st.slice_state != nullptr && st.slice_state[chunk] != 2u) {
      bool fresh[VEC];
      bool any_fresh = false;
#pragma unroll
      for (int k = 0; k < VEC; k++) {
        const int32_t was = iters[off + k];
        fresh[k] = unsat_in[off + k] == 0 && st.slot_cw[off + k] != kNoCodeword && (was < 0 || was == latch_iteration);
        any_fresh = any_fresh || fresh[k];
      }
      if (__builtin_amdgcn_ballot_w64(any_fresh) != 0) {
// ... 848 lines not shown
```

### ldpc_toolbox_amd/csrc/kernels_group.hip.h

```cpp
#pragma once
namespace ldpc {
namespace dev {

#ifdef LDPC_GROUP_KERNELS_TU
__global__ void init_group_kernel(uint32_t *done, int32_t *iters, uint32_t *unsat0, uint32_t *unsat1,
                                  uint32_t *n_active, uint32_t *n_slots, uint32_t *slot_cw, uint32_t nb,
                                  uint32_t G) {
  const uint32_t b = blockIdx.x * blockDim.x + threadIdx.x;
  if (b < G) {
    done[b] = b >= nb ? 1u : 0u;
    iters[b] = -1;
    unsat0[b] = 0;
    unsat1[b] = 0;
    slot_cw[b] = b < nb ? b : kNoCodeword;
  }
  if (b == 0) {
    *n_active = nb;
    *n_slots = min(G, (nb + 255u) / 256u * 256u);
  }
}
#endif

#ifdef LDPC_GROUP_KERNELS_TU
__global__ void latch_kernel(uint32_t *done, int32_t *iters, uint32_t *unsat, uint32_t *n_active,
                             int32_t iteration, uint32_t G) {
  const uint32_t b = blockIdx.x * blockDim.x + threadIdx.x;
  if (b >= G) return;
  if (!done[b] && unsat[b] == 0) {
    done[b] = 1u;
    iters[b] = iteration;
    atomicSub(n_active, 1u);
  }
  unsat[b] = 0;
}
#endif

template <typename T>
__global__ void pack_hard_kernel(const T *__restrict__ soft, uint64_t *__restrict__ bits,
                                 const uint32_t *__restrict__ n_active, const uint32_t *__restrict__ n_slots,
                                 uint32_t n_cols, uint32_t tile, uint32_t W, uint32_t waves_per_word) {
  if (*n_active == 0) return;
  const uint32_t lane = threadIdx.x & 63u;
  const uint32_t wave = uniform((blockIdx.x * blockDim.x + threadIdx.x) >> 6);
  const uint32_t w = wave / waves_per_word;
  if (w >= W || w * 64 >= *n_slots) return;
  soft += tile_base(w * 64, n_cols, tile) + lane;
  constexpr int U = 8;
  for (uint32_t v0 = wave % waves_per_word; v0 < n_cols; v0 += U * waves_per_word) {
    T x[U];
#pragma unroll
    for (int u = 0; u < U; u++) {
      const uint32_t v = v0 + u * waves_per_word;
      if (v < n_cols) x[u] = soft[size_t(v) * tile];
    }
#pragma unroll
    for (int u = 0; u < U; u++) {
      const uint32_t v = v0 + u * waves_per_word;
      if (v < n_cols) {
        const uint64_t b = __builtin_amdgcn_ballot_w64(x[u] <= T(0.0));
        if (lane == 0) bits[size_t(v) * W + w] = b;
      }
    }
  }
}

template <typename T>
__global__ void pack_hard_pair_kernel(const T *__restrict__ soft, uint64_t *__restrict__ bits,
                                      const uint32_t *__restrict__ n_active, const uint32_t *__restrict__ n_slots,
                                      uint32_t n_cols, uint32_t tile, uint32_t W, uint32_t waves_per_pair) {
  if (*n_active == 0) return;
  struct alignas(2 * sizeof(T)) Two {
    T a, b;
  };
  const uint32_t lane = threadIdx.x & 63u;
  const uint32_t wave = uniform((blockIdx.x * blockDim.x + threadIdx.x) >> 6);
  const uint32_t w = (wave / waves_per_pair) * 2;
  if (w >= W || w * 64 >= *n_slots) return;
  const Two *__restrict__ src = reinterpret_cast<const Two *>(soft + tile_base(w * 64, n_cols, tile)) + lane;
  const uint32_t row_pairs = tile / 2;
  const int from0 = static_cast<int>((lane >> 1) * 4), from1 = static_cast<int>((32 + (lane >> 1)) * 4);
  const uint32_t which = lane & 1u;
  constexpr int U = 8;
  for (uint32_t v0 = wave % waves_per_pair; v0 < n_cols; v0 += U * waves_per_pair) {
    Two x[U];
#pragma unroll
    for (int u = 0; u < U; u++) {
      const uint32_t v = v0 + u * waves_per_pair;
      if (v < n_cols) x[u] = src[size_t(v) * row_pairs];
    }
#pragma unroll
    for (int u = 0; u < U; u++) {
      const uint32_t v = v0 + u * waves_per_pair;
      if (v < n_cols) {
        const int two = (x[u].a <= T(0) ? 1 : 0) | (x[u].b <= T(0) ? 2 : 0);
        const uint32_t lo = static_cast<uint32_t>(__builtin_amdgcn_ds_bpermute(from0, two));
        const uint32_t hi = static_cast<uint32_t>(__builtin_amdgcn_ds_bpermute(from1, two));
        const uint64_t b0 = __builtin_amdgcn_ballot_w64(((lo >> which) & 1u) != 0);
        const uint64_t b1 = __builtin_amdgcn_ballot_w64(((hi >> which) & 1u) != 0);
        if (lane == 0) {
          bits[size_t(v) * W + w] = b0;
          if (w + 1 < W) bits[size_t(v) * W + w + 1] = b1;
        }
      }
    }
  }
}

#ifdef LDPC_GROUP_KERNELS_TU
__global__ __launch_bounds__(256) void syndrome_bits_kernel(const uint32_t *__restrict__ row_ptr_,
                                                            const uint32_t *__restrict__ edge_col_, uint32_t n_rows,
                                                            const uint64_t *__restrict__ bits,
                                                            uint32_t *__restrict__ unsat,
                                                            const uint32_t *__restrict__ n_active,
                                                            const uint32_t *__restrict__ n_slots, uint32_t W,
                                                            uint32_t rows_per_wave) {
  if (*n_active == 0) return;
  constexpr int U = 8;
  const TablePtr row_ptr = table_ptr(row_ptr_), edge_col = table_ptr(edge_col_);
  const uint32_t lane = threadIdx.x & 63u;
  const uint32_t wave = uniform((blockIdx.x * blockDim.x + threadIdx.x) >> 6);
  const uint32_t word_chunks = (W + 63) / 64;
  const uint32_t w = (wave % word_chunks) * 64 + lane;
  const uint32_t c0 = (wave / word_chunks) * rows_per_wave;
  if (c0 >= n_rows) return;
  const bool live = w < W && w * 64 < *n_slots;
  if (__builtin_amdgcn_ballot_w64(live) == 0) return;
  const uint32_t c1 = min(c0 + rows_per_wave, n_rows);
  bits += live ? w : 0;
  uint64_t acc = 0;
  for (uint32_t c = c0; c < c1; c++) {
    const uint32_t e0 = row_ptr[c], e1 = row_ptr[c + 1];
    uint64_t x = 0;
    for (uint32_t e = e0; e < e1; e += U) {
      uint64_t y[U];
#pragma unroll
      for (int u = 0; u < U; u++) {
        const uint32_t v = edge_col[min(e + u, e1 - 1)];
        y[u] = bits[size_t(v) * W];
      }
#pragma unroll
      for (int u = 0; u < U; u++) x ^= (e + u < e1) ? y[u] : 0;
    }
    acc |= x;
  }
  if (!live) acc = 0;
  const uint32_t w0 = (wave % word_chunks) * 64;
  for (uint32_t j = 0; j < 64; j++) {
    const uint64_t bitsj = (uint64_t(uint32_t(__builtin_amdgcn_readlane(static_cast<int>(acc >> 32), j))) << 32) |
                           uint64_t(uint32_t(__builtin_amdgcn_readlane(static_cast<int>(acc), j)));
    if (bitsj == 0) continue;
    if ((bitsj >> lane) & 1ull) unsat[size_t(w0 + j) * 64 + lane] = 1u;
  }
}
#endif


template <typename SrcT, typename T>
__global__ __launch_bounds__(256) void ingest_kernel(const SrcT *__restrict__ src, size_t src_stride,
                                                     uint32_t nb, uint32_t n, uint32_t G, uint32_t tile,
                                                     T *__restrict__ chan, T *__restrict__ post,
                                                     uint64_t *__restrict__ rawbits,
                                                     const int32_t *__restrict__ src_block,
                                                     uint32_t block_size) {
  __shared__ SrcT lds[64][65];
  const uint32_t tx = threadIdx.x & 63u, ty = threadIdx.x >> 6;
  const uint32_t v0 = blockIdx.x * 64, b0 = blockIdx.y * 64;
  for (uint32_t r = ty; r < 64; r += 4) {
    const uint32_t b = b0 + r, v = v0 + tx;
    SrcT val = SrcT(1.0);
    if (b < nb && v < n) {
      if (src_block) {
        const int32_t sb = src_block[v / block_size];
        val = sb < 0 ? SrcT(0.0) : src[size_t(b) * src_stride + size_t(sb) * block_size + v % block_size];
      } else {
        val = src[size_t(b) * src_stride + v];
      }
    }
    lds[r][tx] = val;
  }
  __syncthreads();
  const uint32_t W = G / 64;
  const size_t base = tile_base(b0, n, tile) + tx;
  for (uint32_t r = ty; r < 64; r += 4) {
    const uint32_t v = v0 + r;
    if (v < n) {
      const SrcT val = lds[tx][r];
      const T q = static_cast<T>(val);
      chan[base + size_t(v) * tile] = q;
      post[base + size_t(v) * tile] = q;
      const uint64_t bal = __builtin_amdgcn_ballot_w64(val <= SrcT(0.0));
      if (tx == 0) rawbits[size_t(v) * W + blockIdx.y] = bal;
    }
  }
}

template <typename T, typename OutT>
__global__ __launch_bounds__(256) void emit_kernel(const T *__restrict__ post,
                                                   const uint64_t *__restrict__ rawbits, State st,
                                                   const uint32_t *__restrict__ do_compact, uint32_t n,
                                                   uint32_t G, uint32_t tile, uint32_t out_len,
                                                   uint8_t *__restrict__ bits, int32_t *__restrict__ iterations,
                                                   OutT *__restrict__ posterior, int zero_fill,
                                                   int retire_only) {
  __shared__ T lds[64][65];
  const uint32_t tx = threadIdx.x & 63u, ty = threadIdx.x >> 6;
  const uint32_t b0 = blockIdx.y * 64;
  if (b0 >= *st.n_slots) return;
  if (retire_only && *do_compact == 0) return;
  if (retire_only) {
    const uint32_t slot = b0 + tx;
    if (__builtin_amdgcn_ballot_w64(st.done[slot] != 0 && st.slot_cw[slot] != kNoCodeword) == 0) return;
  }
  const size_t base = tile_base(b0, n, tile) + tx;
  const uint32_t W = G / 64;
  const uint32_t n_emit = posterior ? n : min(n, out_len);
  for (uint32_t v0 = blockIdx.x * 64; v0 < max(n_emit, 1u); v0 += gridDim.x * 64) {
  __syncthreads();
  for (uint32_t r = ty; r < 64; r += 4) {
    const uint32_t v = v0 + r;
    lds[r][tx] = (v < n) ? post[base + size_t(v) * tile] : T(0.0);
  }
  __syncthreads();
  for (uint32_t r = ty; r < 64; r += 4) {
    const uint32_t slot = b0 + r, v = v0 + tx;
    const uint32_t cw = st.slot_cw[slot];
    if (cw == kNoCodeword) continue;
    if (retire_only && st.done[slot] == 0) continue;
    const int32_t it = st.iters[slot];
    if (v < n) {
      T val = lds[tx][r];
      uint8_t bit;
      if (it == 0 && rawbits != nullptr)
        bit = uint8_t((rawbits[size_t(v) * W + (cw >> 6)] >> (cw & 63u)) & 1u);
      else if (zero_fill && it < 0) {
        bit = 1;
        val = T(0.0);
      } else
        bit = uint8_t(val <= T(0.0));
      if (v < out_len) bits[size_t(cw) * out_len + v] = bit;
      if constexpr (sizeof(T) == 2) {
        const int c = val >= 127 ? 127 : (val <= -127 ? -127 : int(val));
        if (posterior) posterior[size_t(cw) * n + v] = static_cast<OutT>(c);
      } else {
        if (posterior) posterior[size_t(cw) * n + v] = static_cast<OutT>(val);
      }
    }
    if (iterations && v0 == 0 && tx == 0) iterations[cw] = it;
  }
  }
}

#ifdef LDPC_GROUP_KERNELS_TU
__global__ __launch_bounds__(256) void syndrome_of_bits_kernel(const uint32_t *__restrict__ row_ptr,
                                                               const uint32_t *__restrict__ edge_col,
                                                               uint32_t m, uint32_t n, uint32_t batch,
                                                               const uint8_t *__restrict__ bits,
                                                               uint8_t *__restrict__ syndrome,
                                                               uint32_t *__restrict__ weight) {
  const uint32_t c = blockIdx.x * blockDim.x + threadIdx.x;
  const uint32_t b = blockIdx.y;
  if (b >= batch) return;
  uint32_t parity = 0;
  if (c < m) {
    const uint8_t *row = bits + size_t(b) * n;
    for (uint32_t e = row_ptr[c]; e < row_ptr[c + 1]; e++) parity ^= row[edge_col[e]] & 1u;
    if (syndrome) syndrome[size_t(b) * m + c] = static_cast<uint8_t>(parity);
  }
  if (weight) {
    const uint64_t odd = __builtin_amdgcn_ballot_w64(parity != 0);
    if ((threadIdx.x & 63u) == 0 && odd != 0) atomicAdd(weight + b, static_cast<uint32_t>(__popcll(odd)));
  }
}
#endif

struct CompactPlan {
  uint32_t do_compact;
  uint32_t n_live;
  uint32_t new_slots;
  uint32_t n_move;
};

struct CompactRule {
  uint32_t horizon;
  uint32_t cost_live;
  uint32_t cost_slots;
  uint32_t min_freed_q;
};

#ifdef LDPC_GROUP_KERNELS_TU
__global__ __launch_bounds__(1024) void compact_plan_kernel(State st, CompactPlan *plan, uint32_t *movers,
                                                           uint32_t *holes, uint32_t *fill_cw,
                                                           uint32_t remaining_iterations, CompactRule rule) {
  __shared__ uint32_t wave_tot[2][16];
  __shared__ uint32_t base[2];
  __shared__ uint32_t s_new_slots, s_go;
  if (threadIdx.x == 0 && st.publish != nullptr)
    __hip_atomic_store(st.publish, progress_word(st.epoch, st.tick, min(*st.n_active, 0xFFFFFu)), __ATOMIC_RELAXED,
                       __HIP_MEMORY_SCOPE_SYSTEM);
  const uint32_t n_slots = *st.n_slots;
  const uint32_t lane = threadIdx.x & 63u, wid = threadIdx.x >> 6;
  if (threadIdx.x == 0) base[0] = base[1] = 0;
  __syncthreads();
  uint32_t mine = 0;
  for (uint32_t s = threadIdx.x; s < n_slots; s += 1024) mine += st.done[s] == 0 ? 1u : 0u;
  for (int o = 32; o > 0; o >>= 1) mine += __shfl_down(mine, o, 64);
  if (lane == 0) wave_tot[0][wid] = mine;
  __syncthreads();
  if (threadIdx.x == 0) {
    uint32_t n_live = 0;
    for (uint32_t i = 0; i < 16; i++) n_live += wave_tot[0][i];
    const uint32_t new_slots = (n_live + 255u) / 256u * 256u;
    plan->n_live = n_live;
    plan->new_slots = new_slots;
    plan->n_move = 0;
    const uint32_t freed = n_slots - min(new_slots, n_slots);
    const uint64_t gain = uint64_t(freed) * min(remaining_iterations, rule.horizon) * 4;
    const uint64_t cost = uint64_t(n_live) * rule.cost_live + uint64_t(n_slots) * rule.cost_slots;
    const uint32_t go =
        (n_live > 0 && uint64_t(freed) * 4 >= uint64_t(n_slots) * rule.min_freed_q && freed > 0 && gain > cost) ? 1u : 0u;
    plan->do_compact = go;
    s_go = go;
    s_new_slots = new_slots;
  }
  __syncthreads();
  if (!s_go) return;
  const uint32_t new_slots = s_new_slots;
  for (uint32_t s0 = 0; s0 < n_slots; s0 += 1024) {
    const uint32_t s = s0 + threadIdx.x;
    const bool in = s < n_slots;
    const bool live = in && st.done[s] == 0;
    const bool cls[2] = {live && s >= new_slots, in && !live && s < new_slots};
    uint32_t before[2];
#pragma unroll
    for (int q = 0; q < 2; q++) {
      const uint64_t m = __builtin_amdgcn_ballot_w64(cls[q]);
      before[q] = __popcll(m & ((1ull << lane) - 1ull));
      if (lane == 0) wave_tot[q][wid] = __popcll(m);
    }
    if (in) fill_cw[s] = kNoCodeword;
    __syncthreads();
#pragma unroll
    for (int q = 0; q < 2; q++) {
      uint32_t off = base[q];
      for (uint32_t i = 0; i < wid; i++) off += wave_tot[q][i];
      if (cls[q]) (q == 0 ? movers : holes)[off + before[q]] = s;
    }
    __syncthreads();
    if (threadIdx.x < 2) {
      uint32_t t = 0;
      for (uint32_t i = 0; i < 16; i++) t += wave_tot[threadIdx.x][i];
      base[threadIdx.x] += t;
    }
    __syncthreads();
  }
  const uint32_t n_move = base[0];
  for (uint32_t i = threadIdx.x; i < n_move; i += 1024) fill_cw[holes[i]] = st.slot_cw[movers[i]];
  if (threadIdx.x == 0) plan->n_move = n_move;
}
#endif

template <typename T>
struct MoveList {
  T *arr[3];
  uint32_t rows[3];
  uint32_t moved[3];
  uint32_t count;
};

template <typename T>
__global__ __launch_bounds__(256) void compact_move_kernel(const CompactPlan *plan,
                                                           const uint32_t *__restrict__ movers,
                                                           const uint32_t *__restrict__ holes, MoveList<T> ml,
                                                           uint32_t tile, uint32_t nchunks, uint32_t waves_per_chunk) {
  if (plan->do_compact == 0) return;
  constexpr int U = 8;
  const uint32_t lane = threadIdx.x & 63u;
  const uint32_t wave = uniform((blockIdx.x * blockDim.x + threadIdx.x) >> 6);
  const uint32_t chunk = wave / waves_per_chunk;
  if (chunk >= nchunks || chunk * 64 >= plan->n_move) return;
  const uint32_t i = chunk * 64 + lane;
  const bool valid = i < plan->n_move;
  const uint32_t from = valid ? movers[i] : 0, to = valid ? holes[i] : 0;
  const uint32_t r0 = wave % waves_per_chunk;
  for (uint32_t a = 0; a < ml.count; a++) {
    const uint32_t rows = ml.rows[a];
    const T *__restrict__ src = ml.arr[a] + tile_base(from, rows, tile);
    T *__restrict__ dst = ml.arr[a] + tile_base(to, rows, tile);
    const uint32_t moved = ml.moved[a];
    for (uint32_t r = r0; r < moved; r += U * waves_per_chunk) {
      T x[U];
#pragma unroll
      for (int u = 0; u < U; u++) {
        const uint32_t ru = r + u * waves_per_chunk;
        if (valid && ru < moved) x[u] = src[size_t(ru) * tile];
      }
#pragma unroll
      for (int u = 0; u < U; u++) {
        const uint32_t ru = r + u * waves_per_chunk;
        if (valid && ru < moved) dst[size_t(ru) * tile] = x[u];
      }
    }
  }
}

#ifdef LDPC_GROUP_KERNELS_TU
__global__ void compact_commit_kernel(State st, const CompactPlan *plan, uint32_t *unsat0, uint32_t *unsat1,
                                      uint32_t *n_slots_w, const uint32_t *__restrict__ fill_cw, uint32_t G) {
  if (plan->do_compact == 0) return;
  const uint32_t b = blockIdx.x * blockDim.x + threadIdx.x;
  if (b >= G) return;
  if (st.slice_state != nullptr && b < G / 64) st.slice_state[b] = 2;
  if (b >= plan->new_slots) {
    st.slot_cw[b] = kNoCodeword;
    st.done[b] = 1u;
  } else if (st.done[b] != 0) {
    const uint32_t cw = fill_cw[b];
    st.slot_cw[b] = cw;
    st.done[b] = cw == kNoCodeword ? 1u : 0u;
  }
  st.iters[b] = -1;
  unsat0[b] = 0;
  unsat1[b] = 0;
  if (b == 0) *n_slots_w = plan->new_slots;
}
#endif

#ifdef LDPC_GROUP_KERNELS_TU
__global__ __launch_bounds__(256) void pool_select_kernel(const int32_t *__restrict__ its, uint32_t nf, uint32_t first, int reduced,
                                                          uint32_t *__restrict__ idx, uint32_t *__restrict__ stats,
                                                          unsigned long long *__restrict__ sum_its) {
  const uint32_t i = blockIdx.x * blockDim.x + threadIdx.x;
  const int32_t it = i < nf ? its[i] : 0;
  const bool ok = i < nf && it >= 0, miss = i < nf && it < 0;
  const uint64_t ok_mask = __builtin_amdgcn_ballot_w64(ok), miss_mask = __builtin_amdgcn_ballot_w64(miss);
  const uint32_t lane = threadIdx.x & 63u;
  unsigned long long s = ok ? static_cast<unsigned long long>(it) : 0ull;
  for (int off = 32; off > 0; off >>= 1) s += __shfl_xor(s, off, 64);
  uint32_t base = 0;
  if (lane == 0) {
    if (ok_mask) {
      atomicAdd(&stats[0], static_cast<uint32_t>(__builtin_popcountll(ok_mask)));
      atomicAdd(sum_its, s);
    }
    if (miss_mask) base = atomicAdd(&stats[reduced ? 2 : 1], static_cast<uint32_t>(__builtin_popcountll(miss_mask)));
  }
  base = __shfl(base, 0, 64);
  if (miss && reduced) idx[base + __builtin_popcountll(miss_mask & ((1ull << lane) - 1ull))] = first + i;
}
__global__ __launch_bounds__(256) void pool_gather_kernel(const uint32_t *__restrict__ idx, uint32_t count,
                                                          const uint32_t *__restrict__ src, size_t row_words,
                                                          uint32_t *__restrict__ dst) {
  const uint32_t i = (blockIdx.x * blockDim.x + threadIdx.x) >> 6, lane = threadIdx.x & 63u;
  if (i >= count) return;
  const uint32_t *s = src + size_t(idx[i]) * row_words;
  uint32_t *d = dst + size_t(i) * row_words;
  for (size_t w = lane; w < row_words; w += 64) d[w] = s[w];
}
__global__ __launch_bounds__(256) void pool_scatter_kernel(const uint32_t *__restrict__ idx, uint32_t count,
                                                           const uint8_t *__restrict__ pbits, uint32_t out_len,
                                                           const int32_t *__restrict__ pits, const uint32_t *__restrict__ ppost,
                                                           size_t post_words, uint8_t *__restrict__ bits,
                                                           int32_t *__restrict__ its, uint32_t *__restrict__ post) {
  const uint32_t i = (blockIdx.x * blockDim.x + threadIdx.x) >> 6, lane = threadIdx.x & 63u;
  if (i >= count) return;
  const size_t f = idx[i];
  for (uint32_t b = lane; b < out_len; b += 64) bits[f * out_len + b] = pbits[size_t(i) * out_len + b];
  if (lane == 0 && its != nullptr) its[f] = pits[i];
  if (post != nullptr)
    for (size_t w = lane; w < post_words; w += 64) post[f * post_words + w] = ppost[size_t(i) * post_words + w];
}
#endif

}
}
```

### ldpc_toolbox_amd/csrc/launch.hip.h

```cpp
#pragma once
#include "device_decoder_internal.h"

namespace ldpc {

template <typename T>
struct Launch {
  hipStream_t s;
  bool rec_long;
  bool fast;
  bool corr;
  dev::MinsumCorr<T> minsum_corr;

  template <typename F>
  auto with_corr(F &&launch) const {
    if (corr) return launch(minsum_corr);
    return launch();
  }
  template <typename F>
  auto minsum(uint32_t vec, bool first, F &&f) const {
    return with_vec<T>(vec, [&](auto V) {
      return with_bool(first, [&](auto FIRST) { return with_corr([&](auto... mc) { return f(V, FIRST, mc...); }); });
    });
  }
  template <typename F>
  void with_rule(Rule rule, F &&f) const {
    auto fast_or = [&](auto fast_rule, auto exact_rule) {
      if constexpr (sizeof(T) == 4)
        if (fast) return f(fast_rule);
      f(exact_rule);
    };
    switch (rule) {
      case Rule::Phi: return fast_or(int_c<dev::kRulePhiFast>{}, int_c<dev::kRulePhi>{});
      case Rule::Tanh: return fast_or(int_c<dev::kRuleTanhFast>{}, int_c<dev::kRuleTanh>{});
      case Rule::Minstarapprox: return f(int_c<dev::kRuleMinstarapprox>{});
      case Rule::Aminstar: return f(int_c<dev::kRuleAminstar>{});
      case Rule::Minsum:
        return with_corr([&](auto... mc) { f(int_c<sizeof...(mc) ? dev::kRuleMinsumCorr : dev::kRuleMinsum>{}, mc...); });
    }
  }
  template <typename K, typename... A>
  void go(K kernel, const Tiling &t, size_t lds, const A &...args) const {
    if (lds > 48 * 1024)
      (void)hipFuncSetAttribute(reinterpret_cast<const void *>(kernel), hipFuncAttributeMaxDynamicSharedMemorySize,
                                static_cast<int>(lds));
    kernel<<<t.blocks, t.threads, lds, s>>>(args...);
  }

  void cn_minsum(bool first, uint32_t vec, bool wide_mask, const Tiling &t, const dev::Graph &g, const dev::State &st,
                 const T *L, T *msg, uint32_t *unsat) const {
    minsum(vec, first, [&](auto V, auto FIRST, auto... mc) {
      with_bool(wide_mask, [&](auto wide) {
        using MASK = std::conditional_t<decltype(wide)::value, uint64_t, uint32_t>;
        dev::cn_minsum_kernel<T, decltype(V)::value, MASK, 8, decltype(FIRST)::value, true, decltype(mc)...>
            <<<t.blocks, t.threads, 0, s>>>(g, t.sched, st, L, msg, unsat, mc...);
      });
    });
  }
  void cn_lfree(bool first, uint32_t vec, bool wide_mask, const Tiling &t, const dev::Graph &g, const dev::State &st,
                const T *chan, T *post, const T *msg_in, T *msg_out, uint32_t *unsat) const {
    minsum(vec, first, [&](auto V, auto FIRST, auto... mc) {
      with_bool(wide_mask, [&](auto wide) {
        using MASK = std::conditional_t<decltype(wide)::value, uint64_t, uint32_t>;
        dev::cn_minsum_lfree_kernel<T, decltype(V)::value, MASK, 4, decltype(FIRST)::value, true, false, decltype(mc)...>
            <<<t.blocks, t.threads, 0, s>>>(g, t.sched, st, chan, post, msg_in, msg_out, unsat, mc...);
      });
    });
  }
  struct Records {
    T *mag;
    void *flags;
    uint32_t recw;
    bool flags8 = false;
  };
  template <typename F>
  static void with_rec_form(const Records &r, F &&f) {
    if (r.recw == 3 && r.flags != nullptr && r.flags8) return f(int_c<3>{}, std::true_type{}, std::true_type{});
    if (r.recw == 3 && r.flags != nullptr) return f(int_c<3>{}, std::true_type{}, std::false_type{});
    if (r.recw == 3) return f(int_c<3>{}, std::false_type{}, std::false_type{});
    f(int_c<4>{}, std::false_type{}, std::false_type{});
  }
  template <bool CONST, bool F16, bool F8 = false>
  static auto rec_ref(const Records &r) {
    using TT = std::conditional_t<CONST, const T, T>;
    using FW = dev::RecFlagWord<T, F16, F8>;
    if constexpr (F16)
      return dev::RecPair<TT, FW>{r.mag, static_cast<FW *>(r.flags)};
    else
      return static_cast<TT *>(r.mag);
  }
  void cn_rec(bool first, uint32_t vec, const Tiling &t, const dev::Graph &g, const dev::State &st, const T *chan, T *post,
              const Records &in, const Records &out, T *msg, uint32_t *unsat, uint32_t run, bool send = true) const {
    minsum(vec, first, [&](auto V, auto FIRST, auto... mc) {
      with_rec_form(in, [&](auto W, auto F16, auto F8) {
        with_bool(rec_long, [&](auto long_rows) {
          constexpr bool kF8 = decltype(F8)::value && !decltype(long_rows)::value;
          constexpr int kU = kF8 ? int(kRecFlags8MaxRow) : 8;
          auto go_rec = [&](auto SEND) {
            dev::cn_minsum_rec_kernel<T, decltype(V)::value, decltype(W)::value, decltype(F16)::value, kU, decltype(FIRST)::value,
                                      true, false, decltype(long_rows)::value, decltype(SEND)::value, kF8, decltype(mc)...>
                <<<t.blocks, t.threads, 0, s>>>(g, t.sched, st, chan, post, rec_ref<true, decltype(F16)::value, kF8>(in),
                                                rec_ref<false, decltype(F16)::value, kF8>(out), msg, unsat, run, mc...);
          };
          if constexpr (decltype(F16)::value) {
            if (!send) return go_rec(std::false_type{});
          }
          go_rec(std::true_type{});
        });
      });
    });
  }
  void vn_free_rec(uint32_t vec, const Tiling &t, const dev::Graph &g, const dev::State &st, const uint32_t *free_rs,
                   const T *chan, const Records &rec, T *post, int32_t event_iteration) const {
    with_vec<T>(vec, [&](auto V) {
      with_rec_form(rec, [&](auto W, auto F16, auto F8) {
        dev::vn_free_rec_kernel<T, decltype(V)::value, decltype(W)::value, decltype(F16)::value, decltype(F8)::value>
            <<<t.blocks, t.threads, 0, s>>>(g, t.sched, st, free_rs, chan, rec_ref<true, decltype(F16)::value, decltype(F8)::value>(rec),
                                            post, event_iteration);
      });
    });
  }

  void cn_staged(bool first, Rule rule, uint32_t reg_dmax, const uint32_t *recs, const Tiling &t, size_t lds, T *row_scratch,
                 const dev::Graph &g, const dev::State &st, const T *L, T *msg, uint32_t *unsat, uint32_t dmax) const {
    with_rule(rule, [&](auto rule_c, auto... mc) {
      with_bool(first, [&](auto FIRST) {
        constexpr int RULE = decltype(rule_c)::value;
        if constexpr (RULE == dev::kRuleTanh) {
          if (reg_dmax != 0)
            return with_bool(reg_dmax == 10, [&](auto ten) {
              go(dev::cn_reg_kernel<RULE, T, decltype(ten)::value ? 10 : 12, decltype(FIRST)::value>, t, lds, g, t.sched, st,
                 recs, L, msg, unsat, dmax);
            });
        }
        if (row_scratch)
          go(dev::cn_staged_kernel<RULE, T, decltype(FIRST)::value, true, decltype(mc)...>, t, 0, g, t.sched, st, L, msg,
             unsat, dmax, row_scratch, mc...);
        else
          go(dev::cn_staged_kernel<RULE, T, decltype(FIRST)::value, false, decltype(mc)...>, t, lds, g, t.sched, st, L, msg,
             unsat, dmax, nullptr, mc...);
      });
    });
  }

  template <int VEC, bool NT, bool LIST, int EVW, bool EVF16, bool EVF8, typename... SRC>
  void vn_go(const Tiling &t, const dev::Graph &g, const dev::State &st, const T *chan, T *post, const uint32_t *unsat_in,
             uint32_t *unsat_clear, int32_t latch_it, const uint32_t *free_var, const uint32_t *free_rs, const Records *ev_rec,
             uint32_t n_free, SRC... src) const {
    dev::VnEventOf<T, EVF16, EVF8> ev{};
    if (ev_rec) ev = dev::VnEventOf<T, EVF16, EVF8>{free_var, free_rs, rec_ref<true, EVF16, EVF8>(*ev_rec), n_free};
    dev::vn_kernel<T, VEC, 8, NT, LIST, EVW, EVF16, EVF8, SRC...>
        <<<t.blocks, t.threads, 0, s>>>(g, t.sched, st, chan, src..., post, unsat_in, unsat_clear, latch_it, ev);
  }
  typedef const T *__restrict__ MsgIn;
  typedef const uint32_t *__restrict__ TableIn;
  void vn(bool list, uint32_t vec, const Tiling &t, const dev::Graph &g, const dev::State &st, const T *chan, const T *msg,
          T *post, const uint32_t *unsat_in, uint32_t *unsat_clear, int32_t latch_it) const {
    with_vec<T>(vec, [&](auto V) {
      with_bool(list, [&](auto LIST) {
        vn_go<decltype(V)::value, true, decltype(LIST)::value, 0, false, false, MsgIn>(
            t, g, st, chan, post, unsat_in, unsat_clear, latch_it, nullptr, nullptr, nullptr, 0, msg);
      });
    });
  }
  void vn_event(uint32_t vec, const Tiling &t, const dev::Graph &g, const dev::State &st, const T *chan, const T *msg, T *post,
                const uint32_t *unsat_in, uint32_t *unsat_clear, int32_t latch_it, const uint32_t *free_var,
                const uint32_t *free_rs, const Records &rec, uint32_t n_free) const {
    with_vec<T>(vec, [&](auto V) {
      with_rec_form(rec, [&](auto W, auto F16, auto F8) {
        vn_go<decltype(V)::value, true, true, decltype(W)::value, decltype(F16)::value, decltype(F8)::value, MsgIn>(
            t, g, st, chan, post, unsat_in, unsat_clear, latch_it, free_var, free_rs, &rec, n_free, msg);
      });
    });
  }

  void vn_rec(uint32_t vec, const Tiling &t, const dev::Graph &g, const dev::State &st, const T *chan,
              const Records &rec, const uint32_t *keep_rs, T *post, const uint32_t *unsat_in, uint32_t *unsat_clear,
              int32_t latch_it, const uint32_t *free_var, const uint32_t *free_rs, const Records *ev_rec, uint32_t n_free,
              const dev::VnChain *chain = nullptr) const {
    with_vec<T>(vec, [&](auto V) {
      with_bool(ev_rec != nullptr, [&](auto EV) {
        with_bool(rec.flags8, [&](auto F8) {
          constexpr bool kF8 = decltype(F8)::value;
          using RecIn = typename dev::RecRef<T, true, kF8>::in;
          if (chain)
            return vn_go<decltype(V)::value, true, true, decltype(EV)::value ? 3 : 0, true, kF8, RecIn, TableIn, dev::VnChain>(
                t, g, st, chan, post, unsat_in, unsat_clear, latch_it, free_var, free_rs, ev_rec, n_free,
                rec_ref<true, true, kF8>(rec), keep_rs, *chain);
          vn_go<decltype(V)::value, true, true, decltype(EV)::value ? 3 : 0, true, kF8, RecIn, TableIn>(
              t, g, st, chan, post, unsat_in, unsat_clear, latch_it, free_var, free_rs, ev_rec, n_free,
              rec_ref<true, true, kF8>(rec), keep_rs);
        });
      });
    });
  }
  static Tiling chain_tiling(uint32_t G, uint32_t tile, uint32_t slice, uint32_t threads, uint32_t target_waves,
                             dev::VnChain *chain) {
    const uint32_t wpb = threads / 64, spt = std::max<uint32_t>(1, tile / slice);
    uint32_t mates = (spt <= wpb && wpb % spt == 0) ? wpb / spt : 1;
    mates = std::min(mates, chain->width);
    if (chain->width % mates != 0) mates = 1;
    Tiling t = make_tiling(G, tile, slice, std::max<uint32_t>(chain->n_blocks, 1) * mates, threads, target_waves);
    if (t.sched.waves_per_chunk % mates != 0) mates = 1;
    chain->mates = mates;
    chain->n_groups = t.sched.waves_per_chunk / mates;
    return t;
  }

  void hl(bool first, Rule rule, uint32_t reg_dmax, const Tiling &t, size_t lds, T *row_scratch, const dev::Graph &g,
          const dev::State &st, const uint32_t *level_rows, uint32_t n_level, T *Q, T *R, uint32_t dmax) const {
    with_rule(rule, [&](auto rule_c, auto... mc) {
      with_bool(first, [&](auto FIRST) {
        constexpr int RULE = decltype(rule_c)::value;
        auto reg = [&](auto DMAX) {
          go(dev::hl_level_reg_kernel<RULE, T, decltype(DMAX)::value, decltype(FIRST)::value, decltype(mc)...>, t, lds, g,
             t.sched, st, level_rows, n_level, Q, R, dmax, mc...);
        };
        if (reg_dmax == 10)
          reg(int_c<10>{});
        else if (reg_dmax == 12)
          reg(int_c<12>{});
        else if (reg_dmax == 24)
          reg(int_c<24>{});
        else if (row_scratch)
          go(dev::hl_level_kernel<RULE, T, decltype(FIRST)::value, true, decltype(mc)...>, t, 0, g, t.sched, st, level_rows,
             n_level, Q, R, dmax, row_scratch, mc...);
        else
          go(dev::hl_level_kernel<RULE, T, decltype(FIRST)::value, false, decltype(mc)...>, t, lds, g, t.sched, st,
             level_rows, n_level, Q, R, dmax, nullptr, mc...);
      });
    });
  }

  void hl_minsum(bool first, uint32_t vec, const Tiling &t, const dev::Graph &g, const dev::State &st,
                 const uint32_t *level_rows, uint32_t n_level, T *Q, T *R) const {
    minsum(vec, first, [&](auto V, auto FIRST, auto... mc) {
      dev::hl_minsum_kernel<T, decltype(V)::value, 8, decltype(FIRST)::value, decltype(mc)...>
          <<<t.blocks, t.threads, 0, s>>>(g, t.sched, st, level_rows, n_level, Q, R, mc...);
    });
  }
  static uint32_t hl_reg_bucket(uint32_t maxdeg) {
    const uint32_t dmax = maxdeg <= 8 ? 8 : (maxdeg <= 12 ? 12 : (maxdeg <= 20 ? 20 : (maxdeg <= 32 ? 32 : 0)));
    return 2 * dmax * (sizeof(T) / 4) <= 96 ? dmax : 0;
  }
  static uint32_t hl_reg_vec(uint32_t vec, uint32_t dmax) {
    const uint32_t words = sizeof(T) / 4;
    while (vec > 1 && 2 * dmax * vec * words > 96) vec /= 2;
    return vec;
  }
  template <typename F>
  static bool with_bucket(uint32_t dmax, F &&f) {
    switch (dmax) {
      case 8: return f(int_c<8>{});
      case 12: return f(int_c<12>{});
      case 20: return f(int_c<20>{});
      case 32: return f(int_c<32>{});
      default: return false;
    }
  }
  bool hl_minsum_reg(bool first, uint32_t vec, uint32_t dmax, const Tiling &t, const dev::Graph &g, const dev::State &st,
                     const uint32_t *level_rows, uint32_t n_level, T *Q, T *R) const {
    return minsum(vec, first, [&](auto V, auto FIRST, auto... mc) {
      return with_bucket(dmax, [&](auto D) {
        constexpr int VEC = decltype(V)::value, DMAX = decltype(D)::value;
        if constexpr (DMAX <= 12 || VEC * sizeof(T) <= (DMAX == 20 ? 8u : 4u)) {
          dev::hl_minsum_reg_kernel<T, VEC, DMAX, decltype(FIRST)::value, decltype(mc)...>
              <<<t.blocks, t.threads, 0, s>>>(g, t.sched, st, level_rows, n_level, Q, R, mc...);
          return true;
        } else {
          return false;
        }
// ... 28 lines not shown
```

### ldpc_toolbox_amd/csrc/run_group.hip.h

```cpp
#pragma once
#include "launch.hip.h"

namespace ldpc {


template <typename T>
int DeviceDecoder::run_group(Workspace &w, const GroupCall &call) {
  const uint32_t max_iterations = call.max_iterations;
  const size_t nb = call.nb;
  uint32_t tile = opt_tile_ ? opt_tile_ : (sizeof(T) == 4 ? 256 : 128);
  tile = std::max<uint32_t>(64, tile / 64 * 64);
  while (w.G % tile != 0) tile -= 64;
  GroupFrame f(*this, w, call, tile);
  const uint32_t G = f.G, W = f.W, n = f.n, m = f.m;
  const hipStream_t s = f.s;
  const ProgressPoll &poll = f.poll;
  dev::State &st = f.st;
  auto ticked = [&](uint32_t it) { return f.ticked(it); };
  T *chan = static_cast<T *>(w.chan), *post = static_cast<T *>(w.post), *msg = static_cast<T *>(w.msg);
  const uint32_t target_waves = opt_waves_ ? opt_waves_ : 256 * 1024;
  const uint32_t lds_columns = impl_.rule == Rule::Tanh ? 1u : 2u;
  const Launch<T> launch{s, max_row_weight_ > 8 || opt_rec_long_, impl_.fast, impl_.correction != Correction::None,
                         dev::MinsumCorr<T>{static_cast<T>(impl_.alpha()), static_cast<T>(impl_.beta())}};
  const dev::Graph g = f.graph(d_edge_aux_.get<uint32_t>(), d_edge_peer_.get<uint32_t>());

  if (int rc = f.begin(dev::ingest_kernel<float, T>, dev::ingest_kernel<double, T>, chan, post)) return rc;
  const Tiling pack_t = make_tiling(G, tile, 64, n, 256, std::min<uint32_t>(target_waves, kPackWaves));
  auto pack = [&](const T *soft) {
    dev::pack_hard_kernel<T><<<pack_t.blocks, pack_t.threads, 0, s>>>(soft, w.hardbits, w.n_active, w.n_slots, n, tile,
                                                                      W, pack_t.sched.waves_per_chunk);
  };

  auto emit = [&](int zero_fill, int retire_only) { f.emit(post, &w.plan->do_compact, zero_fill, retire_only); };
  const Tiling mv_t = make_tiling(G, tile, 64, n, 256, kMoveWaves);
  uint32_t post_move_rows = 0;
  auto compact = [&](uint32_t remaining, T *msg_cur, bool with_chan, uint32_t msg_rows, uint16_t *flags = nullptr,
                     uint32_t flag_rows = 0, bool flags8 = false) {
    grp::compact_plan(s, ticked(max_iterations - remaining), w.plan, w.perm, w.slot_tmp, w.fill_cw, remaining,
        dev::CompactRule{kCompactHorizon, kCompactCostLive, kCompactCostSlots, kCompactMinFreedQ});
    emit(0, 1);
    dev::MoveList<T> ml{};
    auto add = [&](T *arr, uint32_t rows, uint32_t moved) {
      ml.arr[ml.count] = arr;
      ml.rows[ml.count] = rows;
      ml.moved[ml.count++] = moved;
    };
    if (with_chan) add(chan, n, n);
    add(post, n, post_move_rows ? post_move_rows : n);
    if (msg_rows) add(msg_cur, msg_rows, msg_rows);
    dev::compact_move_kernel<T><<<mv_t.blocks, mv_t.threads, 0, s>>>(w.plan, w.perm, w.slot_tmp, ml, tile,
                                                                     mv_t.sched.nchunks, mv_t.sched.waves_per_chunk);
    if (flags && flags8) {
      const dev::MoveList<uint8_t> fl{{reinterpret_cast<uint8_t *>(flags)}, {flag_rows}, {flag_rows}, 1};
      dev::compact_move_kernel<uint8_t><<<mv_t.blocks, mv_t.threads, 0, s>>>(w.plan, w.perm, w.slot_tmp, fl, tile,
                                                                           mv_t.sched.nchunks, mv_t.sched.waves_per_chunk);
    } else if (flags) {
      const dev::MoveList<uint16_t> fl{{flags}, {flag_rows}, {flag_rows}, 1};
      dev::compact_move_kernel<uint16_t><<<mv_t.blocks, mv_t.threads, 0, s>>>(w.plan, w.perm, w.slot_tmp, fl, tile,
                                                                            mv_t.sched.nchunks, mv_t.sched.waves_per_chunk);
    }
    grp::compact_commit(s, st, w.plan, w.unsat0, w.unsat1, w.n_slots, w.fill_cw, G);
  };
  auto checkpoint_due = [&](uint32_t it) {
    if (!opt_compact_ || max_iterations < 12 || it + 4 > max_iterations) return false;
    const bool layered = impl_.schedule == Schedule::Layered;
    const uint32_t first = opt_compact_first_ ? opt_compact_first_ : (layered ? 3u : 6u);
    const uint32_t every = opt_compact_every_ ? opt_compact_every_ : (layered ? 1u : 2u);
    if (it < first) return false;
    return it <= 26 ? (it - first) % every == 0 : it % 4 == 0;
  };

  uint32_t *unsat[2] = {w.unsat0, w.unsat1};
  int zero_fill = 0;
  last_record_flag_bytes_.store(0, std::memory_order_relaxed);

  if (impl_.schedule == Schedule::Flooding) {
    const bool streaming = impl_.rule == Rule::Minsum && !opt_staged_minsum_ && max_row_weight_ <= 64;
    const uint32_t vec = pick_vec_for(tile, sizeof(T) == 4 ? 4 : 2, opt_vec_);
    const uint32_t stream_block = kStreamBlock;
    const Tiling vn_t = make_tiling(G, tile, 64 * vec, n, stream_block, opt_waves_ ? opt_waves_ : kVnWaves);
    Tiling cn_t = make_tiling(G, tile, 64 * vec, m, stream_block, target_waves);
    uint32_t st_threads = 256;
    size_t st_lds = 0;
    T *cn_scratch = nullptr;
    if (!streaming) {
      if (staged_block(lds_columns, max_row_weight_, sizeof(T), &st_threads, &st_lds)) {
        cn_t = make_tiling(G, tile, 64, m, st_threads, target_waves);
      } else {
        st_threads = kScratchThreads;
        st_lds = 0;
        cn_t = make_tiling(G, tile, 64, m, st_threads, std::min(target_waves, kScratchWaves));
        if (int rc = ensure_row_scratch(w, scratch_bytes_for(cn_t, max_row_weight_, sizeof(T)))) return rc;
        cn_scratch = w.row_scratch.get<T>();
      }
    }
    const uint32_t cn_reg = (streaming || !opt_cn_reg_ || !d_row_recs_ || impl_.rule != Rule::Tanh || impl_.fast ||
                             uint64_t(std::max(e_, n_)) * tile * sizeof(T) >= (1ull << 32))
                                ? 0u
                                : (max_row_weight_ <= 10 ? 10u : (max_row_weight_ <= 12 ? 12u : 0u));
    const bool wide_mask = max_row_weight_ > 32;
    const bool records = streaming && w.records && w.rec[0] != nullptr &&
                         uint64_t(std::max<size_t>(std::max(e_, n_), m_ * rec_w_)) * tile * sizeof(T) < (1ull << 32);
    const bool lfree = streaming && lfree_ready_ && opt_lfree_ && (w.msg2 != nullptr || records);
    T *mbuf[2] = {msg, (lfree && !records) ? static_cast<T *>(w.msg2) : msg};
    const bool flags8 = records && w.rec_flags[0] != nullptr && opt_flags8_ && !launch.rec_long &&
                        record_flag_bytes(max_row_weight_, sizeof(T) == 8) == 1;
    if (records) last_record_flag_bytes_.store((flags8 ? 1u : (w.rec_flags[0] ? 2u : uint32_t(sizeof(T)))),
                                  std::memory_order_relaxed);
    const typename Launch<T>::Records rbuf[2] = {{static_cast<T *>(w.rec[0]), w.rec_flags[0], rec_w_, flags8},
                                                 {static_cast<T *>(w.rec[1]), w.rec_flags[1], rec_w_, flags8}};
    const uint32_t rec_rows = w.rec_flags[0] ? 2 * m : m * rec_w_;
    if (lfree && post_rows_keep_ > 0 && post_rows_keep_ <= n) post_move_rows = post_rows_keep_;
    const bool vn_records = records && w.rec_flags[0] != nullptr && d_keep_rs_ && opt_vn_records_;
    last_vn_records_.store(vn_records, std::memory_order_relaxed);
    bool vn_bundles = false;
    const bool quiet = records && opt_rec_quiet_;
    if (quiet) {
      st.slice_state = w.slice_state;
      HIP_TRY(hipMemsetAsync(w.slice_state, 0, size_t(G / 64) * sizeof(uint32_t), s));
    }
    const uint32_t rec_run = std::max<uint32_t>(1, std::min<uint32_t>(opt_rec_run_, m));
    const Tiling rec_t = make_tiling(G, tile, 64 * vec, (m + rec_run - 1) / rec_run, stream_block, target_waves);
    dev::Graph g_keep = g, g_free = g;
    Tiling vn_keep_t = vn_t, vn_free_t = vn_t, vn_event_t = vn_t;
    if (lfree) {
      g_keep.list_var = d_keep_var_.get<uint32_t>();
      g_keep.list_ptr = d_keep_ptr_.get<uint32_t>();
      g_keep.list_edge = records ? d_keep_pos_.get<uint32_t>() : d_keep_edge_.get<uint32_t>();
      g_keep.n_list = n_keep_;
      g_free.list_var = d_free_var_.get<uint32_t>();
      g_free.list_ptr = d_free_ptr_.get<uint32_t>();
      g_free.list_edge = d_free_edge_.get<uint32_t>();
      g_free.n_list = n_free_;
      const uint32_t wv = opt_waves_ ? opt_waves_ : kVnWaves;
      vn_keep_t = make_tiling(G, tile, 64 * vec, n_keep_, stream_block, wv);
      vn_keep_t.sched.reverse = 1u;
      vn_free_t = make_tiling(G, tile, 64 * vec, n_free_, stream_block, wv);
      vn_event_t = make_tiling(G, tile, 64 * vec, n_free_, stream_block, 16 * 1024);
    }
    dev::Graph g_bundle = g_keep;
    uint32_t bundle_saved = 0, chain_rs_at = 0;
    if (vn_records && opt_vn_bundles_ && bundle_rs_at_ != 0) {
      vn_bundles = true;
      g_bundle.list_var = d_keep_rs_.get<uint32_t>() + bundle_var_at_;
      g_bundle.list_ptr = d_keep_rs_.get<uint32_t>() + bundle_ptr_at_;
      const uint32_t bundle_w = std::max<uint32_t>(1, (stream_block / 64) / vn_keep_t.sched.slices_per_tile);
      bundle_saved = vn_bundle_saved_[std::min(bundle_w, kVnBundleW)];
    }
    last_vn_bundles_.store(vn_bundles, std::memory_order_relaxed);
    last_vn_bundle_saved_.store(bundle_saved, std::memory_order_relaxed);
    dev::VnChain chain{};
    Tiling vn_chain_t = vn_keep_t;
    uint32_t chain_saved = 0;
    bool vn_chains = false;
    if (vn_bundles && opt_vn_chains_) {
      const VnChainAt &at = vn_chain_at_[opt_vn_chain_len_ == kVnChainLens[0] ? 0 : (opt_vn_chain_len_ == kVnChainLens[1] ? 1 : 2)];
      if (at.rs_at != 0) {
        vn_chains = true;
        chain.len = opt_vn_chain_len_;
        chain.width = kVnBundleW;
        chain.n_blocks = at.n_blocks;
        vn_chain_t = Launch<T>::chain_tiling(G, tile, 64 * vec, stream_block, opt_waves_ ? opt_waves_ : kVnWaves, &chain);
        vn_chain_t.sched.reverse = 1u;
        g_bundle.list_var = d_keep_rs_.get<uint32_t>() + at.var_at;
        g_bundle.list_ptr = d_keep_rs_.get<uint32_t>() + at.ptr_at;
        chain_rs_at = at.rs_at;
        chain_saved = chain.mates == kVnBundleW ? at.saved : at.saved_alone;
      }
    }
    last_vn_chains_.store(vn_chains, std::memory_order_relaxed);
    last_vn_chain_saved_.store(chain_saved, std::memory_order_relaxed);
    const bool adaptive = opt_compact_ && poll.flag != nullptr && poll.throttle && !opt_compact_every_;
    bool seen_drop = false;
    auto tail_checkpoint = [&](uint32_t it) {
      const uint32_t first_ck = opt_compact_first_ ? opt_compact_first_ : 6u;
      return seen_drop && max_iterations >= 12 && it + 4 <= max_iterations && it >= first_ck;
    };
    for (uint32_t it = 1; it <= max_iterations; it++) {
      if (it > 1 && poll.finished(it)) break;
      if (adaptive && !seen_drop && poll.running(static_cast<uint32_t>(nb)) < nb) seen_drop = true;
      const bool first = it == 1;
      uint32_t *unsat_out = unsat[it & 1];
      T *m_out = mbuf[it & 1];
      const T *m_in = mbuf[(it + 1) & 1];
      const dev::State stp = ticked(it);
      timed_begin(kKernelCheck, s);
      if (records)
        launch.cn_rec(first, vec, rec_t, g, stp, chan, post, rbuf[(it + 1) & 1], rbuf[it & 1], msg, unsat_out, rec_run,
                      !vn_records);
      else if (lfree)
        launch.cn_lfree(first, vec, wide_mask, cn_t, g, stp, chan, post, m_in, m_out, unsat_out);
      else if (streaming)
        launch.cn_minsum(first, vec, wide_mask, cn_t, g, stp, first ? chan : post, msg, unsat_out);
      else
        launch.cn_staged(first, impl_.rule, cn_reg, d_row_recs_.get<uint32_t>(), cn_t, st_lds, cn_scratch, g, stp, first ? chan : post, msg,
                         unsat_out, max_row_weight_);
      timed_end(kKernelCheck, s);
      timed_begin(kKernelVar, s);
      if (vn_records) {
        const bool event = quiet && it > 1 && opt_vn_event_;
        launch.vn_rec(vec, vn_chains ? vn_chain_t : vn_keep_t, vn_bundles ? g_bundle : g_keep, st, chan, rbuf[it & 1],
                      d_keep_rs_.get<uint32_t>() + (vn_chains ? chain_rs_at : (vn_bundles ? bundle_rs_at_ : 0u)), post,
                      first ? nullptr : unsat_out, unsat[(it + 1) & 1], static_cast<int32_t>(it) - 1, d_free_var_.get<uint32_t>(),
                      d_free_rs_.get<uint32_t>(), event ? &rbuf[(it - 1) & 1] : nullptr, n_free_, vn_chains ? &chain : nullptr);
        if (quiet && it > 1 && !event)
          launch.vn_free_rec(vec, vn_event_t, g_free, st, d_free_rs_.get<uint32_t>(), chan, rbuf[(it - 1) & 1], post,
                             static_cast<int32_t>(it) - 1);
      } else if (quiet && it > 1 && opt_vn_event_) {
        launch.vn_event(vec, vn_keep_t, g_keep, st, chan, m_out, post, unsat_out, unsat[(it + 1) & 1],
                        static_cast<int32_t>(it) - 1, d_free_var_.get<uint32_t>(), d_free_rs_.get<uint32_t>(), rbuf[(it - 1) & 1],
                        n_free_);
      } else {
        launch.vn(lfree, vec, lfree ? vn_keep_t : vn_t, lfree ? g_keep : g, st, chan, m_out, post,
                  first ? nullptr : unsat_out, unsat[(it + 1) & 1], static_cast<int32_t>(it) - 1);
        if (quiet && it > 1)
          launch.vn_free_rec(vec, vn_event_t, g_free, st, d_free_rs_.get<uint32_t>(), chan, rbuf[(it - 1) & 1], post,
                             static_cast<int32_t>(it) - 1);
      }
      timed_end(kKernelVar, s);
      if (checkpoint_due(it) || tail_checkpoint(it)) {
        if (records)
          compact(max_iterations - it, rbuf[it & 1].mag, true, rec_rows, w.rec_flags[it & 1], m, flags8);
        else
          compact(max_iterations - it, m_out, true, static_cast<uint32_t>(e_));
      }
    }
    if (records && max_iterations > 0) {
      launch.vn_free_rec(vec, vn_free_t, g_free, st, d_free_rs_.get<uint32_t>(), chan, rbuf[max_iterations & 1], post, -1);
    } else if (lfree && max_iterations > 0) {
      dev::State st_nolatch = st;
      launch.vn(true, vec, vn_free_t, g_free, st_nolatch, chan, mbuf[max_iterations & 1], post, nullptr, w.scratch_flags, -1);
    }
    if (max_iterations > 0) {
      pack(post);
      uint32_t *u = unsat[(max_iterations + 1) & 1];
      f.syndrome_of(w.hardbits, u);
      f.latch(u, static_cast<int32_t>(max_iterations));
    } else {
      zero_fill = 1;
    }
  } else {
    uint32_t threads = 64;
    size_t lds = 0;
    const bool streaming = impl_.rule == Rule::Minsum && !opt_staged_minsum_;
    if (!staged_block(lds_columns, max_row_weight_, sizeof(T), &threads, &lds) && !streaming) {
      const size_t waves_bound = size_t(kScratchWaves) + size_t(G / 64) * (kScratchThreads / 64);
      if (int rc = ensure_row_scratch(w, waves_bound * 2 * max_row_weight_ * 64 * sizeof(T))) return rc;
    }
    const uint32_t n_levels = level_ptr_.empty() ? 0 : static_cast<uint32_t>(level_ptr_.size() - 1);
    const dev::State st0 = st;
    const uint32_t vec = pick_vec_for(tile, sizeof(T) == 4 ? 4 : 2, opt_vec_);
    const bool serial = n_levels > opt_serial_levels_;
    const uint32_t n_launch = serial ? std::min<uint32_t>(n_levels, 1) : n_levels;
    const bool hl_rec = streaming && opt_hl_records_ && opt_hl_reg_ && max_row_weight_ <= (sizeof(T) == 4 ? 26u : 58u) &&
                        Launch<T>::hl_reg_bucket(max_row_weight_) != 0 && m_ * 3 <= e_ &&
                        uint64_t(std::max(n_, m_ * 3)) * tile * sizeof(T) < (1ull << 32);
    for (uint32_t it = 1; it <= max_iterations; it++) {
      if (it > 1 && poll.finished(it)) break;
      const dev::State stp = ticked(it);
      for (uint32_t l = 0; l < n_launch; l++) {
        const dev::State &st = l == 0 ? stp : st0;
        const uint32_t r0 = serial ? 0 : level_ptr_[l], cnt = serial ? m : level_ptr_[l + 1] - level_ptr_[l];
        const uint32_t lmaxdeg = serial ? max_row_weight_ : level_maxdeg_[l];
        const uint32_t tnodes = serial ? 1 : cnt;
        const uint32_t sblock = serial ? 64 : 256;
        const uint32_t reg_dmax = opt_hl_reg_ ? Launch<T>::hl_reg_bucket(lmaxdeg) : 0;
        if (hl_rec) {
          const uint32_t rvec = Launch<T>::hl_rec_vec(vec, reg_dmax);
          const Tiling t = make_tiling(G, tile, 64 * rvec, tnodes, sblock, target_waves);
          timed_begin(kKernelLayer, s);
          const bool launched = launch.hl_minsum_rec(it == 1, rvec, reg_dmax, t, g, st, d_level_rows_.get<uint32_t>() + r0, cnt, post, msg);
          timed_end(kKernelLayer, s);
          if (!launched) {
            fail("internal error: no row-record layered kernel for this level");
            return -3;
          }
          continue;
        }
        if (streaming && reg_dmax) {
          const uint32_t rvec = Launch<T>::hl_reg_vec(vec, reg_dmax);
          const Tiling t = make_tiling(G, tile, 64 * rvec, tnodes, sblock, target_waves);
          timed_begin(kKernelLayer, s);
          const bool launched = launch.hl_minsum_reg(it == 1, rvec, reg_dmax, t, g, st, d_level_rows_.get<uint32_t>() + r0, cnt, post, msg);
          timed_end(kKernelLayer, s);
          if (!launched) {
            fail("internal error: no register-resident layered kernel for this level");
            return -3;
          }
          continue;
        }
        if (streaming) {
          const Tiling t = make_tiling(G, tile, 64 * vec, tnodes, sblock, target_waves);
          timed_begin(kKernelLayer, s);
          launch.hl_minsum(it == 1, vec, t, g, st, d_level_rows_.get<uint32_t>() + r0, cnt, post, msg);
          timed_end(kKernelLayer, s);
          continue;
        }
        const uint32_t ldmax = std::max<uint32_t>(lmaxdeg, 1);
        uint32_t lthreads = threads;
        size_t llds = lds;
        const bool lfits = staged_block(lds_columns, ldmax, sizeof(T), &lthreads, &llds);
        if (serial) {
          lthreads = 64;
          llds = size_t(lds_columns) * ldmax * 64 * sizeof(T);
        }
        if (!lfits) {
          lthreads = serial ? 64 : kScratchThreads;
          llds = 0;
        }
        const bool fits32 = uint64_t(std::max(e_, n_)) * tile * sizeof(T) < (1ull << 32);
        const uint32_t lreg = (!opt_hl_reg_ || !fits32) ? 0 : (ldmax <= 10 ? 10 : (ldmax <= 12 ? 12 : (ldmax <= 24 ? 24 : 0)));
        const uint32_t *ltab = !lreg ? d_level_rows_.get<uint32_t>() + r0 : (serial ? d_serial_recs_.get<uint32_t>() : d_level_recs_.get<uint32_t>() + level_rec_ptr_[l]);
        const Tiling t = make_tiling(G, tile, 64, tnodes, lthreads, lfits ? target_waves : std::min(target_waves, kScratchWaves));
        if (!lfits && scratch_bytes_for(t, ldmax, sizeof(T)) > w.row_scratch.capacity()) {
          fail("internal error: row scratch smaller than a level's launch");
          return -3;
        }
        timed_begin(kKernelLayer, s);
        launch.hl(it == 1, impl_.rule, lreg, t, llds, lfits ? nullptr : w.row_scratch.get<T>(), g, st, ltab, cnt, post,
                  msg, ldmax);
        timed_end(kKernelLayer, s);
      }
      pack(post);
      f.syndrome_of(w.hardbits, w.unsat0);
      f.latch(w.unsat0, static_cast<int32_t>(it));
      if (checkpoint_due(it)) compact(max_iterations - it, msg, false, hl_rec ? m * 3 : static_cast<uint32_t>(e_));
    }
  }

  emit(zero_fill, 0);
  HIP_TRY(hipGetLastError());
  return 0;
}

}
```

Before: 50960.

## Trim per-call edge work: skip post at ingest, fuse checkpoint retire/move, emit from hard bits

When posteriors are not requested and the record-based flooding path is used, ingest no longer writes the posterior array, and the first check-node pass reads the channel values in its place. At checkpoints, the separate retire-emit and row-move launches are fused into combined retire+move and post-commit kernels. The final pass now uses a variable-node kernel that writes hard-decision bits directly with ballots, and emit builds output bytes from those packed bits instead of transposing float posteriors. The aim is to cut memory traffic and launch count at call boundaries, at the cost of more code paths and new correctness edge cases such as the partial pack rows and the hard_ok gating.

```diff
diff --git a/ldpc_toolbox_amd/csrc/c_api.cpp b/ldpc_toolbox_amd/csrc/c_api.cpp
--- a/ldpc_toolbox_amd/csrc/c_api.cpp
+++ b/ldpc_toolbox_amd/csrc/c_api.cpp
@@ -761,6 +761,10 @@
     *value = d.flags8();
   else if (k == "last_record_flag_bytes")
     *value = d.last_record_flag_bytes();
+  else if (k == "call_edges")
+    *value = d.call_edges();
+  else if (k == "last_call_edges")
+    *value = d.last_call_edges();
   else if (k == "minsum_correction")
     *value = static_cast<int64_t>(d.implementation().correction);
   else if (k == "minsum_correction_int")
diff --git a/ldpc_toolbox_amd/csrc/device_decoder.h b/ldpc_toolbox_amd/csrc/device_decoder.h
--- a/ldpc_toolbox_amd/csrc/device_decoder.h
+++ b/ldpc_toolbox_amd/csrc/device_decoder.h
@@ -51,6 +51,12 @@
   uint32_t vn_bundle_saved_permille() const { return last_vn_bundle_saved_.load(std::memory_order_relaxed); }
   uint32_t last_vn_chains() const { return last_vn_chains_.load(std::memory_order_relaxed) ? 1 : 0; }
   uint32_t vn_chain_saved_permille() const { return last_vn_chain_saved_.load(std::memory_order_relaxed); }
+  uint32_t call_edges() const { return opt_call_edges_ ? 1 : 0; }
+  uint32_t last_call_edges() const { return last_call_edges_.load(std::memory_order_relaxed); }
+  static constexpr uint32_t kCallEdgeIngest = 1;
+  static constexpr uint32_t kCallEdgeClose = 2;
+  static constexpr uint32_t kCallEdgeEmit = 4;
+  static constexpr uint32_t kCallEdgeCheckpoint = 8;
 
   void set_group_size(size_t g) { group_pref_ = g; }
   size_t group_size() const { return group_pref_; }
@@ -123,6 +129,7 @@
   static constexpr uint32_t kVnWaves = 128 * 1024;
   static constexpr uint32_t kPackWaves = 16 * 1024;
   static constexpr uint32_t kSyndThreads = 512 * 1024, kMoveWaves = 64 * 1024, kRetireBlocks = 256;
+  static constexpr uint32_t kEdgeRetireBlocks = 1024, kEdgeMoveBlocks = 2048;
   static constexpr uint32_t kCompactHorizon = 8, kCompactCostLive = 9, kCompactCostSlots = 0, kCompactMinFreedQ = 2;
   std::string error_;
 
@@ -147,6 +154,8 @@
   } vn_chain_at_[3];
   std::atomic<bool> last_vn_chains_{false};
   std::atomic<uint32_t> last_vn_chain_saved_{0};
+  bool opt_call_edges_ = true;
+  std::atomic<uint32_t> last_call_edges_{0};
   std::atomic<uint32_t> last_record_flag_bytes_{0};
   std::atomic<bool> last_vn_records_{false};
   uint32_t rec_w_ = 0;
diff --git a/ldpc_toolbox_amd/csrc/device_decoder.hip b/ldpc_toolbox_amd/csrc/device_decoder.hip
--- a/ldpc_toolbox_amd/csrc/device_decoder.hip
+++ b/ldpc_toolbox_amd/csrc/device_decoder.hip
@@ -249,6 +249,8 @@
   }
   else if (key == "rec_long")
     opt_rec_long_ = v != 0;
+  else if (key == "call_edges")
+    opt_call_edges_ = v != 0;
   else if (key == "compact")
     opt_compact_ = v != 0;
   else if (key == "staged_minsum")
@@ -430,6 +432,7 @@
   w.fill_cw = w.perm + 3 * G;
   w.n_slots = w.perm + 4 * G;
   w.plan = reinterpret_cast<dev::CompactPlan *>(w.perm + 4 * G + 16);
+  w.hard_ok = w.perm + 4 * G + 32;
   w.rawbits = reinterpret_cast<uint64_t *>(base + o_raw);
   w.hardbits = reinterpret_cast<uint64_t *>(base + o_hard);
   uint32_t *flags = reinterpret_cast<uint32_t *>(base + o_flags);
@@ -533,6 +536,7 @@
 int DeviceDecoder::decode_device(const void *llrs, bool llrs_f64, size_t batch, uint32_t max_iterations, uint8_t *bits,
                                  size_t out_len, int32_t *iterations, void *posterior, hipStream_t stream) {
   last_pooled_ = 0;
+  last_call_edges_.store(0, std::memory_order_relaxed);
   if (opt_pooling_ && max_iterations >= 24 && batch >= 2 * pool_chunk(batch) && (stream == nullptr || opt_throttle_) && out_len <= n_)
     return decode_device_pooled(llrs, llrs_f64, batch, max_iterations, bits, out_len, iterations, posterior, stream);
   return decode_device_plain(llrs, llrs_f64, batch, max_iterations, bits, out_len, iterations, posterior, stream);
@@ -762,6 +766,7 @@
 int DeviceDecoder::decode_host(const void *llrs, bool llrs_f64, size_t batch, uint32_t max_iterations, uint8_t *bits,
                                size_t out_len, int32_t *iterations, void *posterior) {
   last_pooled_ = 0;
+  last_call_edges_.store(0, std::memory_order_relaxed);
   if (opt_pooling_ && max_iterations >= 24 && batch >= 2 * 4 * pool_chunk(batch) && out_len <= n_)
     return decode_host_pooled(llrs, llrs_f64, batch, max_iterations, bits, out_len, iterations, posterior);
   return decode_host_plain(llrs, llrs_f64, batch, max_iterations, bits, out_len, iterations, posterior);
diff --git a/ldpc_toolbox_amd/csrc/device_decoder_internal.h b/ldpc_toolbox_amd/csrc/device_decoder_internal.h
--- a/ldpc_toolbox_amd/csrc/device_decoder_internal.h
+++ b/ldpc_toolbox_amd/csrc/device_decoder_internal.h
@@ -45,6 +45,7 @@
   uint64_t *rawbits = nullptr, *hardbits = nullptr;
   uint32_t *perm = nullptr, *slot_cw = nullptr, *slot_tmp = nullptr, *fill_cw = nullptr, *n_slots = nullptr;
   dev::CompactPlan *plan = nullptr;
+  uint32_t *hard_ok = nullptr;
   uint32_t *done = nullptr, *unsat0 = nullptr, *unsat1 = nullptr, *n_active = nullptr, *scratch_flags = nullptr,
            *slice_state = nullptr;
   int32_t *iters = nullptr;
@@ -315,11 +316,14 @@
     return 0;
   }
   template <typename P>
-  void emit(const P *post, const uint32_t *do_compact, int zero_fill, int retire_only) const {
-    const dim3 grid(std::min<uint32_t>((n + 63) / 64, retire_only ? kRetireBlocks : 4096), W);
+  void emit(const P *post, const uint32_t *do_compact, int zero_fill, int retire_only, const uint64_t *hard = nullptr,
+            const uint32_t *hard_ok = nullptr) const {
+    const bool from_hard = hard != nullptr && c.posterior == nullptr && !zero_fill && !retire_only;
+    const uint32_t blocks_x = from_hard ? (std::min<uint32_t>(n, static_cast<uint32_t>(c.out_len)) + 3) / 4 / 64 + 1 : (n + 63) / 64;
+    const dim3 grid(std::min<uint32_t>(blocks_x, retire_only ? kRetireBlocks : 4096), W);
     auto go = [&](auto kernel, auto *out) {
       kernel<<<grid, 256, 0, s>>>(post, w.rawbits, st, do_compact, n, G, tile, static_cast<uint32_t>(c.out_len), c.bits,
-                                  c.iterations, out, zero_fill, retire_only);
+                                  c.iterations, out, zero_fill, retire_only, from_hard ? hard : nullptr, hard_ok);
     };
     if (c.llrs_f64)
       go(dev::emit_kernel<P, double>, static_cast<double *>(c.posterior));
diff --git a/ldpc_toolbox_amd/csrc/kernels_flooding.hip.h b/ldpc_toolbox_amd/csrc/kernels_flooding.hip.h
--- a/ldpc_toolbox_amd/csrc/kernels_flooding.hip.h
+++ b/ldpc_toolbox_amd/csrc/kernels_flooding.hip.h
@@ -292,6 +292,73 @@
       if (a != kAuxNone) sum = sum + ra.value(a & 63u, k);
       if (b != kAuxNone) sum = sum + rb.value(b & 63u, k);
       if (live[k]) post[size_t(v) * G + k] = ch.v[k] + sum;
+    }
+  }
+}
+
+template <typename T, int VEC, int RECW, bool F16 = false, bool F8 = false>
+__global__ __launch_bounds__(256) void vn_free_hard_kernel(Graph g, Sched sc, State st, const uint32_t *__restrict__ free_rs_,
+                                                           const T *__restrict__ chan, typename RecRef<T, F16, F8>::in rec,
+                                                           const T *__restrict__ post, uint64_t *__restrict__ bits, uint32_t W) {
+  typedef RowRec<T, VEC, RECW, RecFlagWord<T, F16, F8>> Rec;
+  if (*st.n_active == 0) return;
+  const TablePtr free_var = table_ptr(g.list_var), free_rs = table_ptr(free_rs_);
+  const uint32_t lane = threadIdx.x & 63u, tile = sc.tile;
+  const uint32_t wave = uniform((blockIdx.x * blockDim.x + threadIdx.x) >> 6);
+  uint32_t chunk, i0;
+  wave_slot(sc, wave, &chunk, &i0);
+  if (chunk >= sc.nchunks) return;
+  const uint32_t b0 = chunk * (64 * VEC);
+  if (b0 >= *st.n_slots) return;
+  const size_t off = size_t(b0) + lane * VEC;
+  const size_t G = tile;
+  chan += tile_base(b0, g.n_cols, sc) + lane * VEC;
+  post += tile_base(b0, g.n_cols, sc) + lane * VEC;
+  bits += chunk * VEC;
+  const uint32_t row_bytes = tile * uint32_t(sizeof(T)), lane_off = lane * uint32_t(VEC * sizeof(T));
+  const RecBuf<F16> b_rec = rec_buf<T, RECW>(rec, b0, g.n_rows, sc, row_bytes);
+  bool live[VEC];
+  bool any_live = false, all_live = true;
+#pragma unroll
+  for (int k = 0; k < VEC; k++) {
+    live[k] = st.done[off + k] == 0;
+    any_live = any_live || live[k];
+    all_live = all_live && live[k];
+  }
+  any_live = __builtin_amdgcn_ballot_w64(any_live) != 0;
+  all_live = __builtin_amdgcn_ballot_w64(!all_live) == 0;
+  const uint32_t mine = lane % VEC, at = lane / VEC;
+  for (uint32_t i = i0; i < g.n_list; i += sc.waves_per_chunk) {
+    const uint32_t v = free_var[i], a = free_rs[2 * i], b = free_rs[2 * i + 1];
+    Pack<T, VEC> x;
+    if (any_live) {
+      const Pack<T, VEC> ch = load_pack<T, VEC>(chan + size_t(v) * G);
+      Rec ra, rb;
+      if (a != kAuxNone) ra.load(b_rec, lane_off, (a >> 6) * Rec::kRows * row_bytes, row_bytes);
+      if (b != kAuxNone) rb.load(b_rec, lane_off, (b >> 6) * Rec::kRows * row_bytes, row_bytes);
+#pragma unroll
+      for (int k = 0; k < VEC; k++) {
+        T sum = -T(0.0);
+        if (a != kAuxNone) sum = sum + ra.value(a & 63u, k);
+        if (b != kAuxNone) sum = sum + rb.value(b & 63u, k);
+        x.v[k] = ch.v[k] + sum;
+      }
+    }
+    if (!all_live) {
+      const Pack<T, VEC> old = load_pack<T, VEC>(post + size_t(v) * G);
+#pragma unroll
+      for (int k = 0; k < VEC; k++) x.v[k] = (any_live && live[k]) ? x.v[k] : old.v[k];
+    }
+    uint64_t picked = 0;
+#pragma unroll
+    for (int k = 0; k < VEC; k++) {
+      const uint64_t bal = __builtin_amdgcn_ballot_w64(x.v[k] <= T(0.0));
+      picked = (mine == uint32_t(k)) ? bal : picked;
+    }
+#pragma unroll
+    for (int j = 0; j < VEC; j++) {
+      const uint64_t word = __builtin_amdgcn_ballot_w64(((picked >> (uint32_t(j) * (64 / VEC) + at)) & 1ull) != 0);
+      if (lane == 0) bits[size_t(v) * W + j] = word;
     }
   }
 }
diff --git a/ldpc_toolbox_amd/csrc/kernels_group.hip.h b/ldpc_toolbox_amd/csrc/kernels_group.hip.h
--- a/ldpc_toolbox_amd/csrc/kernels_group.hip.h
+++ b/ldpc_toolbox_amd/csrc/kernels_group.hip.h
@@ -38,7 +38,9 @@
 template <typename T>
 __global__ void pack_hard_kernel(const T *__restrict__ soft, uint64_t *__restrict__ bits,
                                  const uint32_t *__restrict__ n_active, const uint32_t *__restrict__ n_slots,
-                                 uint32_t n_cols, uint32_t tile, uint32_t W, uint32_t waves_per_word) {
+                                 uint32_t n_cols, uint32_t tile, uint32_t W, uint32_t waves_per_word, uint32_t n_pack,
+                                 uint32_t *__restrict__ ran) {
+  if (ran != nullptr && blockIdx.x == 0 && threadIdx.x == 0) *ran = *n_active != 0 ? 1u : 0u;
   if (*n_active == 0) return;
   const uint32_t lane = threadIdx.x & 63u;
   const uint32_t wave = uniform((blockIdx.x * blockDim.x + threadIdx.x) >> 6);
@@ -46,17 +48,17 @@
   if (w >= W || w * 64 >= *n_slots) return;
   soft += tile_base(w * 64, n_cols, tile) + lane;
   constexpr int U = 8;
-  for (uint32_t v0 = wave % waves_per_word; v0 < n_cols; v0 += U * waves_per_word) {
+  for (uint32_t v0 = wave % waves_per_word; v0 < n_pack; v0 += U * waves_per_word) {
     T x[U];
 #pragma unroll
     for (int u = 0; u < U; u++) {
       const uint32_t v = v0 + u * waves_per_word;
-      if (v < n_cols) x[u] = soft[size_t(v) * tile];
+      if (v < n_pack) x[u] = soft[size_t(v) * tile];
     }
 #pragma unroll
     for (int u = 0; u < U; u++) {
       const uint32_t v = v0 + u * waves_per_word;
-      if (v < n_cols) {
+      if (v < n_pack) {
         const uint64_t b = __builtin_amdgcn_ballot_w64(x[u] <= T(0.0));
         if (lane == 0) bits[size_t(v) * W + w] = b;
       }
@@ -187,12 +189,19 @@
       const SrcT val = lds[tx][r];
       const T q = static_cast<T>(val);
       chan[base + size_t(v) * tile] = q;
-      post[base + size_t(v) * tile] = q;
+      if (post != nullptr) post[base + size_t(v) * tile] = q;
       const uint64_t bal = __builtin_amdgcn_ballot_w64(val <= SrcT(0.0));
       if (tx == 0) rawbits[size_t(v) * W + blockIdx.y] = bal;
     }
   }
 }
+
+template <typename T, typename OutT>
+__device__ __forceinline__ void emit_rows(T (*lds)[65], uint32_t bx, uint32_t nbx, uint32_t by, const T *__restrict__ post,
+                                          const uint64_t *__restrict__ rawbits, const State &st, uint32_t n, uint32_t G,
+                                          uint32_t tile, uint32_t out_len, uint8_t *__restrict__ bits,
+                                          int32_t *__restrict__ iterations, OutT *__restrict__ posterior, int zero_fill,
+                                          int retire_only);
 
 template <typename T, typename OutT>
 __global__ __launch_bounds__(256) void emit_kernel(const T *__restrict__ post,
@@ -201,20 +210,80 @@
                                                    uint32_t G, uint32_t tile, uint32_t out_len,
                                                    uint8_t *__restrict__ bits, int32_t *__restrict__ iterations,
                                                    OutT *__restrict__ posterior, int zero_fill,
-                                                   int retire_only) {
+                                                   int retire_only, const uint64_t *__restrict__ hard = nullptr,
+                                                   const uint32_t *__restrict__ hard_ok = nullptr) {
   __shared__ T lds[64][65];
+  if (retire_only && *do_compact == 0) return;
+  const uint32_t W = G / 64;
+  if (hard != nullptr && posterior == nullptr && !zero_fill && !retire_only && (hard_ok == nullptr || *hard_ok != 0)) {
+    const uint32_t tx = threadIdx.x & 63u, ty = threadIdx.x >> 6;
+    const uint32_t b0 = blockIdx.y * 64;
+    if (b0 >= *st.n_slots) return;
+    __shared__ uint64_t words[260];
+    const uint32_t n_bits = min(n, out_len);
+    const uint32_t n_groups = (n_bits + 3) / 4 + 1;
+    for (uint32_t g0 = blockIdx.x * 64; g0 < n_groups; g0 += gridDim.x * 64) {
+      __syncthreads();
+      for (uint32_t t = threadIdx.x; t < 260; t += 256) {
+        const int32_t v = int32_t(4 * g0 + t) - 3;
+        words[t] = (v >= 0 && uint32_t(v) < n_bits) ? hard[size_t(v) * W + blockIdx.y] : 0ull;
+      }
+      __syncthreads();
+      for (uint32_t r = ty; r < 64; r += 4) {
+        const uint32_t slot = b0 + r;
+        const uint32_t cw = st.slot_cw[slot];
+        if (cw == kNoCodeword) continue;
+        const int32_t it = st.iters[slot];
+        uint8_t *row = bits + size_t(cw) * out_len;
+        const uint32_t a = uint32_t(reinterpret_cast<uintptr_t>(row)) & 3u;
+        const int32_t vs = int32_t(4 * (g0 + tx)) - int32_t(a);
+        uint32_t four = 0;
+        if (it == 0 && rawbits != nullptr) {
+#pragma unroll
+          for (int j = 0; j < 4; j++) {
+            const int32_t v = vs + j;
+            if (v >= 0 && uint32_t(v) < n_bits)
+              four |= uint32_t((rawbits[size_t(v) * W + (cw >> 6)] >> (cw & 63u)) & 1u) << (8 * j);
+          }
+        } else {
+#pragma unroll
+          for (int j = 0; j < 4; j++) four |= uint32_t((words[4 * tx + 3 - a + j] >> r) & 1u) << (8 * j);
+        }
+        if (vs >= 0 && uint32_t(vs) + 4 <= n_bits) {
+          *reinterpret_cast<uint32_t *>(row + vs) = four;
+        } else {
+#pragma unroll
+          for (int j = 0; j < 4; j++) {
+            const int32_t v = vs + j;
+            if (v >= 0 && uint32_t(v) < n_bits) row[v] = uint8_t(four >> (8 * j));
+          }
+        }
+        if (iterations && g0 == 0 && tx == 0) iterations[cw] = it;
+      }
+    }
+    return;
+  }
+  emit_rows<T, OutT>(lds, blockIdx.x, gridDim.x, blockIdx.y, post, rawbits, st, n, G, tile, out_len, bits, iterations, posterior,
+                     zero_fill, retire_only);
+}
+
+template <typename T, typename OutT>
+__device__ __forceinline__ void emit_rows(T (*lds)[65], uint32_t bx, uint32_t nbx, uint32_t by, const T *__restrict__ post,
+                                          const uint64_t *__restrict__ rawbits, const State &st, uint32_t n, uint32_t G,
+                                          uint32_t tile, uint32_t out_len, uint8_t *__restrict__ bits,
+                                          int32_t *__restrict__ iterations, OutT *__restrict__ posterior, int zero_fill,
+                                          int retire_only) {
   const uint32_t tx = threadIdx.x & 63u, ty = threadIdx.x >> 6;
-  const uint32_t b0 = blockIdx.y * 64;
+  const uint32_t b0 = by * 64;
   if (b0 >= *st.n_slots) return;
-  if (retire_only && *do_compact == 0) return;
   if (retire_only) {
     const uint32_t slot = b0 + tx;
     if (__builtin_amdgcn_ballot_w64(st.done[slot] != 0 && st.slot_cw[slot] != kNoCodeword) == 0) return;
   }
+  const uint32_t W = G / 64;
   const size_t base = tile_base(b0, n, tile) + tx;
-  const uint32_t W = G / 64;
   const uint32_t n_emit = posterior ? n : min(n, out_len);
-  for (uint32_t v0 = blockIdx.x * 64; v0 < max(n_emit, 1u); v0 += gridDim.x * 64) {
+  for (uint32_t v0 = bx * 64; v0 < max(n_emit, 1u); v0 += nbx * 64) {
   __syncthreads();
   for (uint32_t r = ty; r < 64; r += 4) {
     const uint32_t v = v0 + r;
@@ -368,14 +437,23 @@
 };
 
 template <typename T>
+__device__ __forceinline__ void move_rows(const CompactPlan *plan, const uint32_t *__restrict__ movers,
+                                          const uint32_t *__restrict__ holes, const MoveList<T> &ml, uint32_t tile,
+                                          uint32_t nchunks, uint32_t waves_per_chunk, uint32_t wave);
+template <typename T>
 __global__ __launch_bounds__(256) void compact_move_kernel(const CompactPlan *plan,
                                                            const uint32_t *__restrict__ movers,
                                                            const uint32_t *__restrict__ holes, MoveList<T> ml,
                                                            uint32_t tile, uint32_t nchunks, uint32_t waves_per_chunk) {
   if (plan->do_compact == 0) return;
+  move_rows<T>(plan, movers, holes, ml, tile, nchunks, waves_per_chunk, uniform((blockIdx.x * blockDim.x + threadIdx.x) >> 6));
+}
+template <typename T>
+__device__ __forceinline__ void move_rows(const CompactPlan *plan, const uint32_t *__restrict__ movers,
+                                          const uint32_t *__restrict__ holes, const MoveList<T> &ml, uint32_t tile,
+                                          uint32_t nchunks, uint32_t waves_per_chunk, uint32_t wave) {
   constexpr int U = 8;
   const uint32_t lane = threadIdx.x & 63u;
-  const uint32_t wave = uniform((blockIdx.x * blockDim.x + threadIdx.x) >> 6);
   const uint32_t chunk = wave / waves_per_chunk;
   if (chunk >= nchunks || chunk * 64 >= plan->n_move) return;
   const uint32_t i = chunk * 64 + lane;
@@ -403,11 +481,8 @@
   }
 }
 
-#ifdef LDPC_GROUP_KERNELS_TU
-__global__ void compact_commit_kernel(State st, const CompactPlan *plan, uint32_t *unsat0, uint32_t *unsat1,
-                                      uint32_t *n_slots_w, const uint32_t *__restrict__ fill_cw, uint32_t G) {
-  if (plan->do_compact == 0) return;
-  const uint32_t b = blockIdx.x * blockDim.x + threadIdx.x;
+__device__ __forceinline__ void commit_slot(const State &st, const CompactPlan *plan, uint32_t *unsat0, uint32_t *unsat1,
+                                            uint32_t *n_slots_w, const uint32_t *__restrict__ fill_cw, uint32_t G, uint32_t b) {
   if (b >= G) return;
   if (st.slice_state != nullptr && b < G / 64) st.slice_state[b] = 2;
   if (b >= plan->new_slots) {
@@ -423,7 +498,55 @@
   unsat1[b] = 0;
   if (b == 0) *n_slots_w = plan->new_slots;
 }
-#endif
+#ifdef LDPC_GROUP_KERNELS_TU
+__global__ void compact_commit_kernel(State st, const CompactPlan *plan, uint32_t *unsat0, uint32_t *unsat1,
+                                      uint32_t *n_slots_w, const uint32_t *__restrict__ fill_cw, uint32_t G) {
+  if (plan->do_compact == 0) return;
+  commit_slot(st, plan, unsat0, unsat1, n_slots_w, fill_cw, G, blockIdx.x * blockDim.x + threadIdx.x);
+}
+#endif
+
+template <typename T, typename OutT, typename FW>
+__global__ __launch_bounds__(256) void compact_retire_move_kernel(
+    const CompactPlan *plan, const T *__restrict__ post, const uint64_t *__restrict__ rawbits, State st, uint32_t n, uint32_t G,
+    uint32_t tile, uint32_t out_len, uint8_t *__restrict__ bits, int32_t *__restrict__ iterations, OutT *__restrict__ posterior,
+    uint32_t emit_blocks, uint32_t emit_nbx, const uint32_t *__restrict__ movers, const uint32_t *__restrict__ holes,
+    MoveList<T> ml, MoveList<FW> fl, uint32_t nchunks, uint32_t waves_per_chunk) {
+  __shared__ T lds[64][65];
+  if (plan->do_compact == 0) return;
+  if (blockIdx.x < emit_blocks) {
+    const uint32_t W = G / 64;
+    for (uint32_t b = blockIdx.x; b < emit_nbx * W; b += emit_blocks)
+      emit_rows<T, OutT>(lds, b % emit_nbx, emit_nbx, b / emit_nbx, post, rawbits, st, n, G, tile, out_len, bits, iterations,
+                         posterior, 0, 1);
+    return;
+  }
+  const uint32_t n_waves = (gridDim.x - emit_blocks) * (blockDim.x >> 6);
+  const uint32_t wave0 = uniform(((blockIdx.x - emit_blocks) * blockDim.x + threadIdx.x) >> 6);
+  const uint32_t todo = min(nchunks, (plan->n_move + 63u) / 64u) * waves_per_chunk;
+  for (uint32_t wave = wave0; wave < todo; wave += n_waves) {
+    move_rows<T>(plan, movers, holes, ml, tile, nchunks, waves_per_chunk, wave);
+    if (fl.count != 0) move_rows<FW>(plan, movers, holes, fl, tile, nchunks, waves_per_chunk, wave);
+  }
+}
+template <typename T>
+__global__ __launch_bounds__(256) void compact_post_commit_kernel(State st, const CompactPlan *plan, uint32_t *unsat0,
+                                                                  uint32_t *unsat1, uint32_t *n_slots_w,
+                                                                  const uint32_t *__restrict__ fill_cw, uint32_t G,
+                                                                  uint32_t commit_blocks, const uint32_t *__restrict__ movers,
+                                                                  const uint32_t *__restrict__ holes, MoveList<T> ml,
+                                                                  uint32_t tile, uint32_t nchunks, uint32_t waves_per_chunk) {
+  if (plan->do_compact == 0) return;
+  if (blockIdx.x < commit_blocks) {
+    commit_slot(st, plan, unsat0, unsat1, n_slots_w, fill_cw, G, blockIdx.x * blockDim.x + threadIdx.x);
+    return;
+  }
+  const uint32_t n_waves = (gridDim.x - commit_blocks) * (blockDim.x >> 6);
+  const uint32_t wave0 = uniform(((blockIdx.x - commit_blocks) * blockDim.x + threadIdx.x) >> 6);
+  const uint32_t todo = min(nchunks, (plan->n_move + 63u) / 64u) * waves_per_chunk;
+  for (uint32_t wave = wave0; wave < todo; wave += n_waves)
+    move_rows<T>(plan, movers, holes, ml, tile, nchunks, waves_per_chunk, wave);
+}
 
 #ifdef LDPC_GROUP_KERNELS_TU
 __global__ __launch_bounds__(256) void pool_select_kernel(const int32_t *__restrict__ its, uint32_t nf, uint32_t first, int reduced,
diff --git a/ldpc_toolbox_amd/csrc/launch.hip.h b/ldpc_toolbox_amd/csrc/launch.hip.h
--- a/ldpc_toolbox_amd/csrc/launch.hip.h
+++ b/ldpc_toolbox_amd/csrc/launch.hip.h
@@ -116,6 +116,16 @@
         dev::vn_free_rec_kernel<T, decltype(V)::value, decltype(W)::value, decltype(F16)::value, decltype(F8)::value>
             <<<t.blocks, t.threads, 0, s>>>(g, t.sched, st, free_rs, chan, rec_ref<true, decltype(F16)::value, decltype(F8)::value>(rec),
                                             post, event_iteration);
+      });
+    });
+  }
+  void vn_free_hard(uint32_t vec, const Tiling &t, const dev::Graph &g, const dev::State &st, const uint32_t *free_rs,
+                    const T *chan, const Records &rec, const T *post, uint64_t *bits, uint32_t W) const {
+    with_vec<T>(vec, [&](auto V) {
+      with_rec_form(rec, [&](auto RW, auto F16, auto F8) {
+        dev::vn_free_hard_kernel<T, decltype(V)::value, decltype(RW)::value, decltype(F16)::value, decltype(F8)::value>
+            <<<t.blocks, t.threads, 0, s>>>(g, t.sched, st, free_rs, chan, rec_ref<true, decltype(F16)::value, decltype(F8)::value>(rec),
+                                            post, bits, W);
       });
     });
   }
diff --git a/ldpc_toolbox_amd/csrc/run_group.hip.h b/ldpc_toolbox_amd/csrc/run_group.hip.h
--- a/ldpc_toolbox_amd/csrc/run_group.hip.h
+++ b/ldpc_toolbox_amd/csrc/run_group.hip.h
@@ -24,20 +24,70 @@
                          dev::MinsumCorr<T>{static_cast<T>(impl_.alpha()), static_cast<T>(impl_.beta())}};
   const dev::Graph g = f.graph(d_edge_aux_.get<uint32_t>(), d_edge_peer_.get<uint32_t>());
 
-  if (int rc = f.begin(dev::ingest_kernel<float, T>, dev::ingest_kernel<double, T>, chan, post)) return rc;
+  const bool fl_streaming = impl_.schedule == Schedule::Flooding && impl_.rule == Rule::Minsum && !opt_staged_minsum_ &&
+                            max_row_weight_ <= 64;
+  const bool fl_records = fl_streaming && w.records && w.rec[0] != nullptr &&
+                          uint64_t(std::max<size_t>(std::max(e_, n_), m_ * rec_w_)) * tile * sizeof(T) < (1ull << 32);
+  const bool edges = opt_call_edges_, edges_no_post = edges && fl_records && call.posterior == nullptr;
+  uint32_t edges_ran = 0;
+  const bool ingest_no_post = edges_no_post;
+  if (ingest_no_post) edges_ran |= kCallEdgeIngest;
+  if (int rc = f.begin(dev::ingest_kernel<float, T>, dev::ingest_kernel<double, T>, chan, ingest_no_post ? static_cast<T *>(nullptr) : post))
+    return rc;
   const Tiling pack_t = make_tiling(G, tile, 64, n, 256, std::min<uint32_t>(target_waves, kPackWaves));
-  auto pack = [&](const T *soft) {
+  auto pack = [&](const T *soft, uint32_t rows, uint32_t *ran) {
     dev::pack_hard_kernel<T><<<pack_t.blocks, pack_t.threads, 0, s>>>(soft, w.hardbits, w.n_active, w.n_slots, n, tile,
-                                                                      W, pack_t.sched.waves_per_chunk);
+                                                                      W, pack_t.sched.waves_per_chunk, rows, ran);
   };
 
-  auto emit = [&](int zero_fill, int retire_only) { f.emit(post, &w.plan->do_compact, zero_fill, retire_only); };
+  const uint64_t *emit_hard = nullptr;
+  auto emit = [&](int zero_fill, int retire_only) {
+    f.emit(post, &w.plan->do_compact, zero_fill, retire_only, retire_only ? nullptr : emit_hard, w.hard_ok);
+  };
   const Tiling mv_t = make_tiling(G, tile, 64, n, 256, kMoveWaves);
   uint32_t post_move_rows = 0;
   auto compact = [&](uint32_t remaining, T *msg_cur, bool with_chan, uint32_t msg_rows, uint16_t *flags = nullptr,
                      uint32_t flag_rows = 0, bool flags8 = false) {
     grp::compact_plan(s, ticked(max_iterations - remaining), w.plan, w.perm, w.slot_tmp, w.fill_cw, remaining,
         dev::CompactRule{kCompactHorizon, kCompactCostLive, kCompactCostSlots, kCompactMinFreedQ});
+    if (edges) {
+      edges_ran |= kCallEdgeCheckpoint;
+      dev::MoveList<T> rest{}, pm{};
+      auto add_to = [](dev::MoveList<T> &l, T *arr, uint32_t rows, uint32_t moved) {
+        l.arr[l.count] = arr;
+        l.rows[l.count] = rows;
+        l.moved[l.count++] = moved;
+      };
+      if (with_chan) add_to(rest, chan, n, n);
+      if (msg_rows) add_to(rest, msg_cur, msg_rows, msg_rows);
+      add_to(pm, post, n, post_move_rows ? post_move_rows : n);
+      const uint32_t emit_nbx = std::min<uint32_t>((n + 63) / 64, kRetireBlocks);
+      const uint32_t emit_blocks = std::min<uint32_t>(emit_nbx * W, kEdgeRetireBlocks);
+      const uint32_t commit_blocks = (G + 255) / 256;
+      auto retire_move = [&](auto fw, auto *out) {
+        using FW = decltype(fw);
+        dev::MoveList<FW> fl{};
+        if (flags) fl = dev::MoveList<FW>{{reinterpret_cast<FW *>(flags)}, {flag_rows}, {flag_rows}, 1};
+        using OutT = std::remove_pointer_t<decltype(out)>;
+        dev::compact_retire_move_kernel<T, OutT, FW><<<emit_blocks + kEdgeMoveBlocks, 256, 0, s>>>(
+            w.plan, post, w.rawbits, st, n, G, tile, static_cast<uint32_t>(call.out_len), call.bits, call.iterations, out,
+            emit_blocks, emit_nbx, w.perm, w.slot_tmp, rest, fl, mv_t.sched.nchunks, mv_t.sched.waves_per_chunk);
+      };
+      auto with_out = [&](auto fw) {
+        if (call.llrs_f64)
+          retire_move(fw, static_cast<double *>(call.posterior));
+        else
+          retire_move(fw, static_cast<float *>(call.posterior));
+      };
+      if (flags && flags8)
+        with_out(uint8_t{});
+      else
+        with_out(uint16_t{});
+      dev::compact_post_commit_kernel<T><<<commit_blocks + kEdgeMoveBlocks, 256, 0, s>>>(
+          st, w.plan, w.unsat0, w.unsat1, w.n_slots, w.fill_cw, G, commit_blocks, w.perm, w.slot_tmp, pm, tile,
+          mv_t.sched.nchunks, mv_t.sched.waves_per_chunk);
+      return;
+    }
     emit(0, 1);
     dev::MoveList<T> ml{};
     auto add = [&](T *arr, uint32_t rows, uint32_t moved) {
@@ -75,7 +125,7 @@
   last_record_flag_bytes_.store(0, std::memory_order_relaxed);
 
   if (impl_.schedule == Schedule::Flooding) {
-    const bool streaming = impl_.rule == Rule::Minsum && !opt_staged_minsum_ && max_row_weight_ <= 64;
+    const bool streaming = fl_streaming;
     const uint32_t vec = pick_vec_for(tile, sizeof(T) == 4 ? 4 : 2, opt_vec_);
     const uint32_t stream_block = kStreamBlock;
     const Tiling vn_t = make_tiling(G, tile, 64 * vec, n, stream_block, opt_waves_ ? opt_waves_ : kVnWaves);
@@ -99,8 +149,7 @@
                                 ? 0u
                                 : (max_row_weight_ <= 10 ? 10u : (max_row_weight_ <= 12 ? 12u : 0u));
     const bool wide_mask = max_row_weight_ > 32;
-    const bool records = streaming && w.records && w.rec[0] != nullptr &&
-                         uint64_t(std::max<size_t>(std::max(e_, n_), m_ * rec_w_)) * tile * sizeof(T) < (1ull << 32);
+    const bool records = fl_records;
     const bool lfree = streaming && lfree_ready_ && opt_lfree_ && (w.msg2 != nullptr || records);
     T *mbuf[2] = {msg, (lfree && !records) ? static_cast<T *>(w.msg2) : msg};
     const bool flags8 = records && w.rec_flags[0] != nullptr && opt_flags8_ && !launch.rec_long &&
@@ -186,8 +235,8 @@
       const dev::State stp = ticked(it);
       timed_begin(kKernelCheck, s);
       if (records)
-        launch.cn_rec(first, vec, rec_t, g, stp, chan, post, rbuf[(it + 1) & 1], rbuf[it & 1], msg, unsat_out, rec_run,
-                      !vn_records);
+        launch.cn_rec(first, vec, rec_t, g, stp, chan, (first && ingest_no_post) ? chan : post, rbuf[(it + 1) & 1], rbuf[it & 1],
+                      msg, unsat_out, rec_run, !vn_records);
       else if (lfree)
         launch.cn_lfree(first, vec, wide_mask, cn_t, g, stp, chan, post, m_in, m_out, unsat_out);
       else if (streaming)
@@ -225,14 +274,20 @@
           compact(max_iterations - it, m_out, true, static_cast<uint32_t>(e_));
       }
     }
-    if (records && max_iterations > 0) {
+    const bool close_hard = edges_no_post && records && lfree && max_iterations > 0;
+    if (close_hard) {
+      edges_ran |= kCallEdgeClose | kCallEdgeEmit;
+      pack(post, post_move_rows ? post_move_rows : n, w.hard_ok);
+      launch.vn_free_hard(vec, vn_free_t, g_free, st, d_free_rs_.get<uint32_t>(), chan, rbuf[max_iterations & 1], post, w.hardbits, W);
+      emit_hard = w.hardbits;
+    } else if (records && max_iterations > 0) {
       launch.vn_free_rec(vec, vn_free_t, g_free, st, d_free_rs_.get<uint32_t>(), chan, rbuf[max_iterations & 1], post, -1);
     } else if (lfree && max_iterations > 0) {
       dev::State st_nolatch = st;
       launch.vn(true, vec, vn_free_t, g_free, st_nolatch, chan, mbuf[max_iterations & 1], post, nullptr, w.scratch_flags, -1);
     }
     if (max_iterations > 0) {
-      pack(post);
+      if (!close_hard) pack(post, n, nullptr);
       uint32_t *u = unsat[(max_iterations + 1) & 1];
       f.syndrome_of(w.hardbits, u);
       f.latch(u, static_cast<int32_t>(max_iterations));
@@ -321,7 +376,7 @@
                   msg, ldmax);
         timed_end(kKernelLayer, s);
       }
-      pack(post);
+      pack(post, n, nullptr);
       f.syndrome_of(w.hardbits, w.unsat0);
       f.latch(w.unsat0, static_cast<int32_t>(it));
       if (checkpoint_due(it)) compact(max_iterations - it, msg, false, hl_rec ? m * 3 : static_cast<uint32_t>(e_));
@@ -329,6 +384,7 @@
   }
 
   emit(zero_fill, 0);
+  last_call_edges_.fetch_or(edges_ran, std::memory_order_relaxed);
   HIP_TRY(hipGetLastError());
   return 0;
 }
```

Result: faster. 51500 (median of 6 runs) (+1.1%).
